# laitalaj/cvpce

Hardware: AMD Instinct MI355X
Metric: shelf images/sec end-to-end (detect+embed+match) (higher is better)
Workload: dtype bf16; 1 GPU; full production path: 8 shelf images/GPU of 3x2048x2048 (SKU-110K shape) -> GLN detect (800x800 internal, detections_per_img=200, conf>0.5) -> RoI crop 256x256 -> MAC-VGG16 embed -> cosine NN match, gallery=3200x1024 (BASELINE configs[2]/[4] per-GPU shape); images_per_gpu=8, global_images=8, gallery=3200, match_dtype=bf16, detector_precision=fp16, parallelism=dp1

## Files before the change

cvpce_amd/_lib.py:

```python
import ctypes
import os
from ctypes import c_int, c_float, c_void_p, c_size_t, c_longlong, POINTER

_HERE = os.path.dirname(os.path.abspath(__file__))
LIB_PATH = os.environ.get('CVPCE_LIB') or os.path.join(_HERE, 'libcvpce_hip.so')


class HipLibraryMissing(ImportError):
    pass


if not os.path.exists(LIB_PATH):
    raise HipLibraryMissing(
        f'{LIB_PATH} not found: the cvpce_amd hot path has no CPU fallback. '
        'Build the HIP library first (python -c "import __graft_entry__ as g; g.build()").')

lib = ctypes.CDLL(LIB_PATH)

_vp = c_void_p
_fp = c_void_p
_ip = c_void_p

SIGNATURES = {
    'cvpce_conv2d_nhwc_bf16': (c_int, [_vp, _vp, _fp, _vp, _vp] + [c_int] * 21 + [_vp]),
    'cvpce_conv2d_splitk_bf16': (c_int, [_vp, _vp, _fp, _vp, _vp] + [c_int] * 20 + [_vp, c_size_t, _vp]),
    'cvpce_conv2d_splitk_workspace_bytes': (c_size_t, [c_longlong, c_int, c_int]),
    'cvpce_set_persistent_workgroups': (c_int, [c_int]),
    'cvpce_conv1x1_nhwc_bf16': (c_int, [_vp, _vp, _fp, _vp, _vp] + [c_int] * 14 + [_vp]),
    'cvpce_vgg_stem_fused': (c_int, [_vp, c_int, _vp, _fp, _vp, _fp, _vp, c_int, c_int, c_int, _vp]),
    'cvpce_gln_stem_fused': (c_int, [_vp, _vp, _fp, _vp, c_int, c_int, c_int, _vp]),
    'cvpce_atlas_copy': (c_int, [POINTER(_vp), POINTER(c_int), POINTER(c_int), POINTER(c_int), POINTER(c_int), c_int, c_int, _vp, c_int, c_int, c_int, c_int, _vp]),
    'cvpce_conv3x3_halo': (c_int, [_vp, _vp, _fp, _vp] + [c_int] * 9 + [_vp]),
    'cvpce_conv3x3_halo_mac': (c_int, [_vp, _vp, _fp, _vp, _fp, c_int, c_int] + [c_int] * 8 + [_vp]),
    'cvpce_conv3x3_halo_wide': (c_int, [_vp, _vp, _fp, _vp] + [c_int] * 9 + [_vp]),
    'cvpce_conv3x3_halo_masked': (c_int, [_vp, _vp, _fp, _vp, _vp, c_int, _vp] + [c_int] * 8 + [_vp]),
    'cvpce_maxpool2d_nhwc_bf16': (c_int, [_vp, _vp] + [c_int] * 9 + [_vp]),
    'cvpce_relu_bf16': (c_int, [_vp, _vp, c_longlong, _vp]),
    'cvpce_pack_halo_weights': (c_int, [_vp, _vp, c_int, c_int]),
    'cvpce_conv3x3_thin_bf16': (c_int, [_vp, _vp, _fp, _vp] + [c_int] * 9 + [_vp]),
    'cvpce_gauss_tail_bf16': (c_int, [_vp, _vp, _fp, _vp, _fp, _fp, c_longlong, c_int, c_int, _vp]),
    'cvpce_gauss_subnet_bf16': (c_int, [_vp, _vp, _fp, _vp, _fp, _vp, _fp, _vp, _fp, c_int, _vp, _fp, c_int, _fp, c_int, c_int, c_int, c_int, _vp]),
    'cvpce_global_max_nhwc_bf16': (c_int, [_vp, _fp, c_int, c_int, c_int, c_int, c_int, _vp]),
    'cvpce_l2_normalize_f32': (c_int, [_fp, _fp, _vp, c_int, c_int, c_float, _vp]),
    'cvpce_gln_transform': (c_int, [_fp, _vp] + [c_int] * 6 + [POINTER(c_float), POINTER(c_float), _vp]),
    'cvpce_gln_transform_batch': (c_int, [POINTER(c_void_p), POINTER(c_int), POINTER(c_int), POINTER(c_int), POINTER(c_int), c_int, _vp, c_int, c_int,
                                          POINTER(c_float), POINTER(c_float), _vp]),
    'cvpce_crop_resize': (c_int, [_fp, _fp, _ip, c_int, _vp, c_int, c_int, c_int, c_int,
                                  POINTER(c_float), POINTER(c_float), _vp]),
    'cvpce_crop_resize_content': (c_int, [_fp, _fp, _ip, c_int, _vp, c_int, c_int, c_int, c_int,
                                          POINTER(c_float), POINTER(c_float), _ip, _vp]),
    'cvpce_pack_embed_input': (c_int, [_fp, _vp, c_int, c_int, c_int, POINTER(c_float), POINTER(c_float), _vp]),
    'cvpce_crop_extents': (c_int, [_fp, _ip, c_int, c_int, c_int, c_int, c_int, _ip, _vp]),
    'cvpce_pad_extents': (c_int, [_fp, c_int, c_int, c_float, _ip, _vp]),
    'cvpce_embed_worklists': (c_int, [_ip, c_int, c_int, ctypes.c_uint, _vp, c_int, _vp, c_longlong, _ip, _ip, _vp]),
    'cvpce_mac_init': (c_int, [_fp, c_int, c_int, c_int, c_int, _fp, _fp, c_int, c_int, _ip, _vp]),
    'cvpce_vgg_stem_fused_list': (c_int, [_vp, c_int, _vp, _vp, _fp, _vp, _fp, _vp, c_int, c_int, c_int, _vp, _ip, _vp]),
    'cvpce_bottleneck_fused_fm': (c_int, [_vp, _vp, _vp, _fp, _vp, _fp, _vp, _fp, _vp] + [c_int] * 5 + [_vp]),
    'cvpce_conv3x3_halo_thin_out': (c_int, [_vp, _vp, _fp, _fp] + [c_int] * 7 + [_vp]),
    'cvpce_conv3x3_halo_list': (c_int, [_vp, _vp, _fp, _vp, _fp, c_int, c_int] + [c_int] * 9 + [_vp, _ip, _vp]),
    'cvpce_conv3x3_halo_strips': (c_int, [_vp, _vp, _fp, _vp, _fp, c_int, c_int] + [c_int] * 9 + [_vp, _ip, _vp]),
    'cvpce_detect_workspace_bytes': (c_size_t, [c_int, c_int, c_int]),
    'cvpce_detect_postprocess': (c_int, [POINTER(c_void_p), POINTER(c_void_p), POINTER(c_int), POINTER(c_int),
                                         POINTER(c_int), POINTER(c_int), _fp, _ip, _fp,
                                         c_int, c_int, c_int, c_int, c_int, c_float, c_float, c_float, c_int, c_float,
                                         _vp, c_size_t, _fp, _fp, _vp, _ip, _ip, _vp]),
    'cvpce_row_norms': (c_int, [_vp, _fp, c_int, c_int, c_int, c_float, _vp]),
    'cvpce_match_workspace_bytes': (c_size_t, [c_int, c_int, c_int]),
    'cvpce_match_set_core': (c_int, [c_int, c_int, c_int]),
    'cvpce_probe_l2_stream': (c_int, [_vp, c_longlong, c_int, _fp, c_int, _vp]),
    'cvpce_probe_mfma_bf16': (c_int, [c_int, c_int, _vp, _fp, c_int, _vp]),
    'cvpce_match_topk': (c_int, [_vp, _vp, _fp, _fp, c_int, c_int, c_int, c_int, c_int, _vp, c_size_t, _vp, _fp, _vp]),
}
for _base, _twin in (('cvpce_conv2d_nhwc_bf16', 'cvpce_conv2d_nhwc_f16'), ('cvpce_conv2d_splitk_bf16', 'cvpce_conv2d_splitk_f16'), ('cvpce_conv1x1_nhwc_bf16', 'cvpce_conv1x1_nhwc_f16'),
                     ('cvpce_gln_stem_fused', 'cvpce_gln_stem_fused_f16'), ('cvpce_conv3x3_halo', 'cvpce_conv3x3_halo_f16'),
                     ('cvpce_conv3x3_halo_wide', 'cvpce_conv3x3_halo_wide_f16'), ('cvpce_conv3x3_halo_thin_out', 'cvpce_conv3x3_halo_thin_out_f16'), ('cvpce_conv3x3_halo_masked', 'cvpce_conv3x3_halo_masked_f16'),
                     ('cvpce_bottleneck_fused_fm', 'cvpce_bottleneck_fused_fm_f16'),
                     ('cvpce_maxpool2d_nhwc_bf16', 'cvpce_maxpool2d_nhwc_f16'), ('cvpce_relu_bf16', 'cvpce_relu_f16'), ('cvpce_gauss_tail_bf16', 'cvpce_gauss_tail_f16'), ('cvpce_gauss_subnet_bf16', 'cvpce_gauss_subnet_f16'), ('cvpce_conv3x3_thin_bf16', 'cvpce_conv3x3_thin_f16'),
                     ('cvpce_gln_transform', 'cvpce_gln_transform_f16'), ('cvpce_gln_transform_batch', 'cvpce_gln_transform_batch_f16')):
    SIGNATURES[_twin] = SIGNATURES[_base]

EVAL_SIGNATURES = {
    'cvpce_eval_match_detections': (c_int, [_fp, _ip, _ip, _ip, _fp, _ip, _ip, _fp] + [c_int] * 5 + [_ip, _vp, _vp]),
}

INPUT_SIGNATURES = {
    'cvpce_gln_transform_batch_u8': (c_int, [POINTER(c_void_p), POINTER(ctypes.c_ubyte), POINTER(c_int), POINTER(c_int), POINTER(c_int), POINTER(c_int), c_int,
                                             _vp, c_int, c_int, POINTER(c_float), POINTER(c_float), _fp, _vp]),
    'cvpce_crop_resize_u8': (c_int, [_vp, _fp, _fp, _ip, c_int, _vp, c_int, c_int, c_int, c_int, POINTER(c_float), POINTER(c_float), _vp]),
    'cvpce_crop_resize_content_u8': (c_int, [_vp, _fp, _fp, _ip, c_int, _vp, c_int, c_int, c_int, c_int, POINTER(c_float), POINTER(c_float), _ip, _vp]),
}
INPUT_SIGNATURES['cvpce_gln_transform_batch_u8_f16'] = INPUT_SIGNATURES['cvpce_gln_transform_batch_u8']

PLANOGRAM_SIGNATURES = {
    'cvpce_planogram_graphs': (c_int, [_fp, _ip, _fp] + [c_int] * 4 + [_ip, _fp, _ip, _vp]),
    'cvpce_planogram_match_workspace_bytes': (c_size_t, [c_longlong]),
    'cvpce_planogram_match': (c_int, [_ip] * 11 + [c_int] * 6 + [c_longlong, _vp, c_size_t, _ip, _ip, _vp]),
}

for _table in (SIGNATURES, EVAL_SIGNATURES, INPUT_SIGNATURES, PLANOGRAM_SIGNATURES):
    for _name, (_res, _args) in _table.items():
        _fn = getattr(lib, _name)
        _fn.restype = _res
        _fn.argtypes = _args

_ERR = {1: 'bad argument', 2: 'kernel launch failure'}


def check(rc, what):
    if rc != 0:
        raise RuntimeError(f'{what} failed: {_ERR.get(rc, rc)}')


class SkipLayer(ctypes.Structure):
    _fields_ = [(k, c_int) for k in ('H', 'W', 'tile_h', 'tile_w', 'out_ops', 'in_H', 'in_W', 'in_ops', 'skip')]


def float3(vals):
    return (c_float * 3)(*[float(v) for v in vals])
```

cvpce_amd/csrc/conv3x3_halo2.hip:

```cpp
#include "halo_common.h"
#include "../../include/cvpce_amd.h"

typedef __attribute__((address_space(3))) void lds_void;
typedef __attribute__((address_space(3))) char lds_char;

#ifndef CVPCE_DBG
#define CVPCE_DBG 0
#endif

#define G2_T 16
#define G2_P 18
#define G2_NPIX 324
#define G2_A_BYTES (328 * 128)
#define G2_NPIECE 41
#define G2_MAX_SEQ 512
#define G2_LTILE_OFF (3 * G2_A_BYTES)
#define G2_LROW_OFF (G2_LTILE_OFF + G2_MAX_SEQ * 4)
#define G2_SMEM_MASKED (G2_LROW_OFF + G2_MAX_SEQ * 32)
#define G2_LLIST_OFF (3 * G2_A_BYTES)
#define G2_SMEM_LIST (G2_LLIST_OFF + G2_MAX_SEQ * 8)

__device__ __forceinline__ int g2_swz0(int u) { return ((u & 3) << 1) | ((u >> 2) & 1); }
__device__ __forceinline__ int g2_swz(int py, int px) { return g2_swz0(px >> 1) ^ (py & 1); }

struct Halo2Args {
    const bf16_t* in;
    const bf16_t* wgt;
    const float* bias;
    const unsigned char* mask;
    bf16_t* out;
    const int* tile_map;
    int tiles_per_image;
    float* gmax;
    int gmax_stride, gmax_off;
    int N, H, W, Cin, Cout, K_pad, relu;
    int cgroups;
    int tiles_x, tiles_y, ptiles, ctiles, ntiles;
    unsigned in_bytes, wgt_bytes;
    const unsigned long long* list;
    const int* list_count;
};

#if CVPCE_DBG & 512
__device__ unsigned long long cvpce_halo2_clock[1024][2];
extern "C" int cvpce_debug_halo2_clock(unsigned long long* host_out) {
    return hipMemcpyFromSymbol(host_out, HIP_SYMBOL(cvpce_halo2_clock), sizeof(cvpce_halo2_clock)) == hipSuccess ? 0 : 2;
}
#endif

template <typename E, bool POOL, bool GMAX, bool LIST, bool STRIP = false, int NW = 8>
__global__ __launch_bounds__(64 * NW, NW == 8 ? 2 : 1) void conv3x3_halo2_kernel(Halo2Args a) {
    static_assert(!STRIP || LIST, "strips come from a work list");
    static_assert(NW == 8 || NW == 4, "cout waves");
    constexpr int TC = 32 * NW, NB = 16, NS = STRIP ? 3 : 1;

    extern __shared__ __attribute__((aligned(16))) unsigned char smem[];
    unsigned char* Ap = smem;

    const int tid = threadIdx.x, lane = tid & 63;
    const int wc = __builtin_amdgcn_readfirstlane(tid >> 6);
    const int l16 = lane & 15, lq = lane >> 4;

    const __amdgpu_buffer_rsrc_t srd_w = __builtin_amdgcn_make_buffer_rsrc((void*)a.wgt, 0, a.wgt_bytes, 0x00020000);
    const __amdgpu_buffer_rsrc_t srd_p = __builtin_amdgcn_make_buffer_rsrc((void*)a.in, 0, a.in_bytes, 0x00020000);

    const int nchunks = a.Cin >> 6;
    const int lbid = (CVPCE_DBG & 2) ? xcd_remap((int)blockIdx.x, (int)gridDim.x) : (int)blockIdx.x;
    int my_tiles, l_first = 0, l_entries = 0;
    if constexpr (LIST) {
        l_entries = __builtin_amdgcn_readfirstlane(*a.list_count);
        const int units = STRIP ? (l_entries + 2) / 3 : l_entries;
        const int groups = (int)gridDim.x / a.ctiles;
        const int per = (units + groups - 1) / groups;
        l_first = (lbid / a.ctiles) * per;
        my_tiles = units - l_first < per ? units - l_first : per;
    } else {
        my_tiles = halo_plain_tiles(a.ntiles, lbid, (int)gridDim.x);
    }
    if (my_tiles <= 0) return;
    const int total_chunks = my_tiles * nchunks;
    unsigned long long* llist = reinterpret_cast<unsigned long long*>(smem + G2_LLIST_OFF);
    if constexpr (LIST) {
        const int staged = my_tiles * NS < G2_MAX_SEQ ? my_tiles * NS : G2_MAX_SEQ;
        for (int idx = tid; idx < staged; idx += 64 * NW) {
            const int k = l_first * NS + idx;
            llist[idx] = a.list[k < l_entries ? k : l_entries - 1];
        }
        __syncthreads();
    }

    unsigned* ltile = reinterpret_cast<unsigned*>(smem + G2_LTILE_OFF);
    unsigned short* lrow = reinterpret_cast<unsigned short*>(smem + G2_LROW_OFF);
    if (a.mask) {
        for (int idx = tid; idx < my_tiles * 16; idx += 64 * NW) {
            const int sq = idx >> 4, y = idx & 15;
            const int r = ((lbid + sq * (int)gridDim.x) / a.ctiles) % a.tiles_per_image;
            int ty, tx;
            if (a.tile_map) {
                const int packed = a.tile_map[r];
                ty = packed >> 16;
                tx = packed & 0xFFFF;
            } else {
                ty = r / a.tiles_x;
                tx = r - ty * a.tiles_x;
            }
            const int oy = ty * G2_T + y;
            unsigned bits = 0;
            if (oy < a.H) {
#pragma unroll
                for (int c = 0; c < G2_T; ++c) {
                    const int ox = tx * G2_T + c;
                    if (ox < a.W && a.mask[oy * a.W + ox]) bits |= 1u << c;
                }
            }
            lrow[idx] = (unsigned short)bits;
            if (y == 0) ltile[sq] = (unsigned)((ty << 16) | tx);
        }
        __syncthreads();
    }

    auto tile_of = [&](int seq, int* n, int* ty, int* tx, int& ct, int* ext) {
        if constexpr (LIST) {
            ct = lbid % a.ctiles;
#pragma unroll
            for (int s = 0; s < NS; ++s) {
                const int k = seq * NS + s, g = l_first * NS + k;
                const unsigned long long e = k < G2_MAX_SEQ ? llist[k] : a.list[g < l_entries ? g : l_entries - 1];
                const int lo = __builtin_amdgcn_readfirstlane((int)wl_lo(e));
                ext[s] = __builtin_amdgcn_readfirstlane((int)wl_hi(e));
                n[s] = wl_image_signed(lo);
                ty[s] = wl_ty((unsigned)lo);
                tx[s] = wl_tx((unsigned)lo);
            }
            return;
        }
        ext[0] = 0;
        const int t = lbid + seq * (int)gridDim.x;
        ct = t % a.ctiles;
        const int p = t / a.ctiles;
        n[0] = p / a.tiles_per_image;
        const int r = p - n[0] * a.tiles_per_image;
        if (a.mask) {
            const int packed = __builtin_amdgcn_readfirstlane((int)ltile[seq]);
            ty[0] = packed >> 16;
            tx[0] = packed & 0xFFFF;
        } else {
            ty[0] = r / a.tiles_x;
            tx[0] = r - ty[0] * a.tiles_x;
        }
    };

    constexpr int NPP = (41 + NW - 1) / NW;
    const int npp = (41 - wc + NW - 1) / NW;
    auto issue_patch = [&](const int* n, const int* ty, const int* tx, int c, int buf, const int* ext) {
        const int ln = halo_lane_id();
#pragma unroll
        for (int i = 0; i < NPP; ++i) {
            if (i < npp) {
                const int j = wc + NW * i;
                const int pp = j * 8 + (ln >> 3);
                const int py = pp / G2_P, px = pp - py * G2_P;
                const int lchunk = (ln & 7) ^ g2_swz(py, px);
                int sn = n[0], sty = ty[0], stx = tx[0], sext = ext[0], ry = py;
                if constexpr (STRIP) {
                    const int st = py >= 12 ? 2 : (py >= 6 ? 1 : 0);
                    ry = py - 6 * st;
                    sn = st == 0 ? n[0] : (st == 1 ? n[1] : n[2]);
                    sty = st == 0 ? ty[0] : (st == 1 ? ty[1] : ty[2]);
                    stx = st == 0 ? tx[0] : (st == 1 ? tx[1] : tx[2]);
                    sext = st == 0 ? ext[0] : (st == 1 ? ext[1] : ext[2]);
                }
                const int ey = wl_ey((unsigned)sext), ex = wl_ex((unsigned)sext);
                const int y = sty * G2_T - 1 + ry, x = stx * G2_T - 1 + px;
                const bool ok = pp < G2_NPIX && (unsigned)y < (unsigned)a.H && (unsigned)x < (unsigned)a.W;
                int nn = sn;
                if constexpr (LIST) nn = (y >= ey || x >= ex) ? a.N - 1 : sn;
                const unsigned off = (unsigned)((((size_t)(nn * a.H + y) * a.W + x) * a.Cin + c * 64) * 2) + (unsigned)(lchunk * 16);
                __builtin_amdgcn_raw_ptr_buffer_load_lds(srd_p, (lds_void*)(Ap + buf * G2_A_BYTES + j * 1024), 16,
                                                         (int)(ok ? off : 0xFFFFFFF0u), 0, 0, 0);
            }
        }
    };
    int pi = 0, pi_seq = 0, pi_c = 0, pi_buf = 0, pi_n[NS], pi_ty[NS], pi_tx[NS], pi_ct, pi_ext[NS];
    tile_of(0, pi_n, pi_ty, pi_tx, pi_ct, pi_ext);
    auto issue_next_patch = [&]() {
        if (pi < total_chunks) {
            if (!(CVPCE_DBG & 4) || pi < 2) issue_patch(pi_n, pi_ty, pi_tx, pi_c, pi_buf, pi_ext);
            ++pi;
            if (++pi_buf == 3) pi_buf = 0;
            if (++pi_c == nchunks) {
                pi_c = 0;
                ++pi_seq;
                if (pi_seq < my_tiles) tile_of(pi_seq, pi_n, pi_ty, pi_tx, pi_ct, pi_ext);
            }
        }
    };

    const unsigned voff1 = (unsigned)(lane * 16);
    auto wbase = [&](int ct, int c) { return __builtin_amdgcn_readfirstlane((int)((unsigned)(c * a.cgroups + ct * (TC / 32) + wc) * 36864u)); };

    unsigned c3[3];
    {
        const int col = halo_col(l16);
#pragma unroll
        for (int kw = 0; kw < 3; ++kw) c3[kw] = (unsigned)(col * 128) ^ (unsigned)((lq ^ g2_swz0(((col + kw) >> 1) & 7)) << 4);
    }
    const unsigned lds_a = (unsigned)(size_t)(lds_char*)Ap;

    auto load_bias = [&](int ct, f32x4* b) {
#pragma unroll
        for (int mt = 0; mt < 2; ++mt) {
            const int co = ct * TC + wc * 32 + 8 * lq + 4 * mt;
            b[mt] = (a.bias && co < a.Cout) ? *reinterpret_cast<const f32x4*>(a.bias + co) : f32x4{0.f, 0.f, 0.f, 0.f};
        }
    };
    f32x4 acc[2][NB];
    {
        f32x4 b0[2];
        load_bias(pi_ct, b0);
#pragma unroll
        for (int i = 0; i < 2; ++i)
#pragma unroll
            for (int j = 0; j < NB; ++j) acc[i][j] = b0[i];
    }

    bf16x8 af[2][3][2];
    bf16x8 bfr[4];
    unsigned e0, e1;

#define G2_LOAD_A(T, SBASE)                                                                                    \
    if constexpr (!(CVPCE_DBG & 8)) {                                                                          \
        _Pragma("unroll") for (int kh_ = 0; kh_ < 3; ++kh_)                                                    \
            _Pragma("unroll") for (int mt_ = 0; mt_ < 2; ++mt_) {                                              \
                const u32x4 v_ = __builtin_amdgcn_raw_buffer_load_b128(srd_w, voff1, (SBASE) + (((T) * 3 + kh_) * 2 + mt_) * 1024, 0); \
                af[(T) & 1][kh_][mt_] = __builtin_bit_cast(bf16x8, v_);                                       \
            }                                                                                                  \
    }
#define G2_PREFETCH_A(T)                                                                                       \
    if constexpr ((T) < 5) { G2_LOAD_A((T) + 1, sb_cur) } else { G2_LOAD_A(0, sb_next) }
#define G2_SET_E(T, BUFB)                                                                                      \
    {                                                                                                          \
        const unsigned x_ = c3[(T) >> 1] ^ (unsigned)(((T) & 1) << 6);                                         \
        e0 = x_ + (BUFB);                                                                                      \
        e1 = (x_ ^ 16u) + (BUFB);                                                                              \
    }
#define G2_READ(T, P)                                                                                          \
    if constexpr (!(CVPCE_DBG & 32)) {                                                                         \
        if constexpr (((P) & 1) == 0)                                                                          \
            asm volatile("ds_read_b128 %0, %1 offset:%2" : "=v"(bfr[((P) + 2 * (T)) & 3]) : "v"(e0), "n"(((P) * G2_P + ((T) >> 1)) * 128)); \
        else                                                                                                   \
            asm volatile("ds_read_b128 %0, %1 offset:%2" : "=v"(bfr[((P) + 2 * (T)) & 3]) : "v"(e1), "n"(((P) * G2_P + ((T) >> 1)) * 128)); \
    }
#define G2_ROW_KH(T, P, KH)                                                                                    \
    {                                                                                                          \
        constexpr int j_ = STRIP ? (P) % 6 - (KH) : (P) - (KH);                                                \
        constexpr int r_ = STRIP ? 4 * ((P) / 6) + j_ : j_;                                                    \
        if constexpr (j_ >= 0 && j_ < (STRIP ? 4 : NB)) {                                                      \
            _Pragma("unroll") for (int mt_ = 0; mt_ < 2; ++mt_)                                                \
                acc[mt_][r_] = E::mfma16(af[(T) & 1][KH][mt_], bfr[((P) + 2 * (T)) & 3], acc[mt_][r_]);       \
        }                                                                                                      \
    }
#define G2_ROW(T, P)                                                                                           \
    {                                                                                                          \
        asm volatile("s_waitcnt lgkmcnt(2)" : "+v"(bfr[((P) + 2 * (T)) & 3]));                                 \
        G2_ROW_KH(T, P, 0) G2_ROW_KH(T, P, 1) G2_ROW_KH(T, P, 2)                                               \
        __builtin_amdgcn_sched_barrier(0);                                                                     \
    }
#define G2_RP(T, P) G2_READ(T, (P) + 2) G2_ROW(T, P)
#define G2_HANDOFF()                                                                                           \
    {                                                                                                          \
        asm volatile("s_waitcnt vmcnt(6)" ::: "memory");                                                       \
        if (!(CVPCE_DBG & 64)) __builtin_amdgcn_s_barrier();                                                   \
        issue_next_patch();                                                                                    \
    }
#define G2_ROWS_AND_TAIL(T, TN, BUFB_NEXT, BEFORE)                                                             \
    G2_RP(T, 0) G2_RP(T, 1) G2_RP(T, 2) G2_RP(T, 3) G2_RP(T, 4) G2_RP(T, 5)                                    \
    if (!LIST || STRIP || rows_ > 4) { G2_RP(T, 6) G2_RP(T, 7) G2_RP(T, 8) G2_RP(T, 9) }                       \
    if (!LIST || STRIP || rows_ > 8) { G2_RP(T, 10) G2_RP(T, 11) G2_RP(T, 12) G2_RP(T, 13) }                   \
    if (!LIST || STRIP || rows_ > 12) {                                                                        \
        G2_RP(T, 14) G2_RP(T, 15)                                                                              \
        BEFORE                                                                                                 \
        G2_SET_E(TN, BUFB_NEXT)                                                                                \
        G2_READ(TN, 0) G2_ROW(T, 16)                                                                           \
        G2_READ(TN, 1) G2_ROW(T, 17)                                                                           \
    } else {                                                                                                   \
        BEFORE                                                                                                 \
        G2_SET_E(TN, BUFB_NEXT)                                                                                \
        G2_READ(TN, 0)                                                                                         \
        G2_READ(TN, 1)                                                                                         \
    }
#define G2_STEP(T)                                                                                             \
    {                                                                                                          \
        G2_PREFETCH_A(T)                                                                                       \
        __builtin_amdgcn_sched_barrier(0);                                                                     \
        G2_ROWS_AND_TAIL(T, (T) + 1, bufb, )                                                                   \
    }

    int seq = 0, cchunk = 0, t_n[NS], t_ty[NS], t_tx[NS], t_ct, t_ext_[NS];
    tile_of(0, t_n, t_ty, t_tx, t_ct, t_ext_);
    int rows_ = (LIST && !STRIP) ? wl_rows((unsigned)t_ext_[0]) : NB;
    int n_ct = t_ct;
    auto next_ct = [&]() {
        if (cchunk + 1 < nchunks) return t_ct;
        if constexpr (LIST) return t_ct;
        if (seq + 1 < my_tiles) return (lbid + (seq + 1) * (int)gridDim.x) % a.ctiles;
        return t_ct;
    };
    issue_next_patch();
    issue_next_patch();
    int sb_cur = wbase(t_ct, 0);
    n_ct = next_ct();
    int sb_next = wbase(n_ct, (cchunk + 1 < nchunks) ? cchunk + 1 : 0);
    {
        constexpr int dbg8_ = CVPCE_DBG & 8;
        _Pragma("unroll") for (int kh_ = 0; kh_ < 3; ++kh_)
            _Pragma("unroll") for (int mt_ = 0; mt_ < 2; ++mt_) {
                const u32x4 v_ = __builtin_amdgcn_raw_buffer_load_b128(srd_w, voff1, sb_cur + (kh_ * 2 + mt_) * 1024, 0);
                af[0][kh_][mt_] = __builtin_bit_cast(bf16x8, v_);
                if (dbg8_) af[1][kh_][mt_] = af[0][kh_][mt_];
            }
    }
    asm volatile("s_waitcnt vmcnt(0)" ::: "memory");
    __builtin_amdgcn_s_barrier();
    unsigned bufb = lds_a;
    int bufi = 0;
    G2_SET_E(0, bufb)
    G2_READ(0, 0)
    G2_READ(0, 1)

    const int lp = lane & 15;
#if CVPCE_DBG & 512
    const unsigned long long ck0_ = __builtin_amdgcn_s_memtime(), rt0_ = __builtin_amdgcn_s_memrealtime();
#endif
    for (int cc = 0; cc < total_chunks; ++cc) {
        asm volatile("" : "+v"(c3[0]), "+v"(c3[1]), "+v"(c3[2]));
        G2_STEP(0) G2_STEP(1) G2_STEP(2) G2_STEP(3) G2_STEP(4)
        {
            G2_PREFETCH_A(5)
            __builtin_amdgcn_sched_barrier(0);
            const int nbufi = (bufi == 2) ? 0 : bufi + 1;
            const unsigned nbufb = lds_a + (unsigned)nbufi * G2_A_BYTES;
            G2_ROWS_AND_TAIL(5, 0, nbufb, G2_HANDOFF())
            bufb = nbufb;
            bufi = nbufi;
        }
        sb_cur = sb_next;

        if (cchunk + 1 == nchunks) {
            const int ct = t_ct;
            const int rows_t = STRIP ? 4 : rows_;
            auto e_n = [&](int nt) { return STRIP ? t_n[(nt >> 2) < NS ? (nt >> 2) : 0] : t_n[0]; };
            auto e_ty = [&](int nt) { return STRIP ? t_ty[(nt >> 2) < NS ? (nt >> 2) : 0] : t_ty[0]; };
            auto e_tx = [&](int nt) { return STRIP ? t_tx[(nt >> 2) < NS ? (nt >> 2) : 0] : t_tx[0]; };
            auto e_row = [&](int nt) { return STRIP ? (nt & 3) : nt; };
            auto e_live = [&](int nt) { return STRIP ? nt < 12 : (!LIST || nt < rows_t); };
            f32x4 nbias[2];
            load_bias(n_ct, nbias);
            const int col = halo_col(lp);
            const int co = ct * TC + wc * 32 + 8 * lq;
            if constexpr (GMAX) {
#pragma unroll
                for (int sg = 0; sg < NS; ++sg) {
                    unsigned m[8];
#pragma unroll
                    for (int j = 0; j < 8; ++j) m[j] = 0u;
                    const int n = t_n[sg], ty = t_ty[sg], tx = t_tx[sg];
                    if (tx * G2_T + col < a.W) {
#pragma unroll
                        for (int nt = STRIP ? 4 * sg : 0; nt < (STRIP ? 4 * sg + 4 : NB); ++nt)
                            if (ty * G2_T + e_row(nt) < a.H && e_live(nt)) {
#pragma unroll
                                for (int j = 0; j < 4; ++j) {
                                    m[j] = max(m[j], __float_as_uint(relu_bits(acc[0][nt][j])));
                                    m[4 + j] = max(m[4 + j], __float_as_uint(relu_bits(acc[1][nt][j])));
                                }
                            }
                    }
#pragma unroll
                    for (int j = 0; j < 8; ++j) {
                        unsigned v = m[j];
                        v = max(v, (unsigned)__builtin_amdgcn_update_dpp(0, (int)v, 0x128, 0xF, 0xF, false));
                        v = max(v, (unsigned)__builtin_amdgcn_update_dpp(0, (int)v, 0x124, 0xF, 0xF, false));
                        v = max(v, (unsigned)__builtin_amdgcn_update_dpp(0, (int)v, 0x122, 0xF, 0xF, false));
                        v = max(v, (unsigned)__builtin_amdgcn_update_dpp(0, (int)v, 0x121, 0xF, 0xF, false));
                        m[j] = v;
                    }
                    if (lp == 0) {
                        unsigned* g = reinterpret_cast<unsigned*>(a.gmax) + (size_t)n * a.gmax_stride + a.gmax_off + co;
#pragma unroll
                        for (int j = 0; j < 8; ++j)
                            if (co + j < a.Cout) atomicMax(g + j, __float_as_uint(E::widen(E::narrow(__uint_as_float(m[j])))));
                    }
                }
            }
            if (GMAX && a.out == nullptr) {
            } else if (POOL) {
#pragma unroll
                for (int i = 0; i < NB / 2; ++i) {
                    const int ox = e_tx(2 * i) * (G2_T / 2) + (col >> 1);
                    const bool lane_ok = (lp < 4 || lp >= 12) && ox < (a.W >> 1);
                    const int oy = e_ty(2 * i) * (G2_T / 2) + (e_row(2 * i) >> 1);
                    const size_t opix = (size_t)(e_n(2 * i) * (a.H >> 1) + oy) * (a.W >> 1) + ox;
                    float r[8];
#pragma unroll
                    for (int mt = 0; mt < 2; ++mt)
#pragma unroll
                        for (int j = 0; j < 4; ++j) r[4 * mt + j] = halo_pool2x2(acc[mt][2 * i][j], acc[mt][2 * i + 1][j], a.relu);
                    if (lane_ok && oy < (a.H >> 1) && co < a.Cout && e_live(2 * i) && (!(CVPCE_DBG & 16) || a.relu == 12345)) {
                        const uint2 l2 = __builtin_bit_cast(uint2, E::pack4(f32x4{r[0], r[1], r[2], r[3]}));
                        const uint2 h2 = __builtin_bit_cast(uint2, E::pack4(f32x4{r[4], r[5], r[6], r[7]}));
                        *reinterpret_cast<u32x4*>(a.out + opix * a.Cout + co) = u32x4{l2.x, l2.y, h2.x, h2.y};
                    }
                }
            } else {
#pragma unroll
                for (int nt = 0; nt < NB; ++nt) {
                    const int ox = e_tx(nt) * G2_T + col;
                    const int oy = e_ty(nt) * G2_T + e_row(nt);
                    const size_t opix = (size_t)(e_n(nt) * a.H + oy) * a.W + ox;
                    const bool store_lane = oy < a.H && ox < a.W && e_live(nt);
                    bool keep = true;
                    if (a.mask) keep = ((lrow[seq * 16 + nt] >> col) & 1u) != 0;
                    f32x4 r0 = acc[0][nt], r1 = acc[1][nt];
                    if (a.relu) {
#pragma unroll
                        for (int j = 0; j < 4; ++j) { r0[j] = relu_bits(r0[j]); r1[j] = relu_bits(r1[j]); }
                    }
                    if (store_lane && co < a.Cout && (!(CVPCE_DBG & 16) || a.relu == 12345)) {
                        const uint2 l2 = __builtin_bit_cast(uint2, E::pack4(r0)), h2 = __builtin_bit_cast(uint2, E::pack4(r1));
                        bf16_t* dst = a.out + opix * a.Cout + co;
                        *reinterpret_cast<u32x4*>(dst) = keep ? u32x4{l2.x, l2.y, h2.x, h2.y} : u32x4{0u, 0u, 0u, 0u};
                    }
                }
            }
#pragma unroll
            for (int mt = 0; mt < 2; ++mt)
#pragma unroll
                for (int nt = 0; nt < NB; ++nt) acc[mt][nt] = nbias[mt];
            cchunk = 0;
            ++seq;
            if (seq < my_tiles) {
                tile_of(seq, t_n, t_ty, t_tx, t_ct, t_ext_);
                if constexpr (LIST && !STRIP) rows_ = wl_rows((unsigned)t_ext_[0]);
            }
        } else {
            ++cchunk;
        }
        n_ct = next_ct();
        sb_next = wbase(n_ct, (cchunk + 1 < nchunks) ? cchunk + 1 : 0);
    }
    asm volatile("s_waitcnt lgkmcnt(0)" ::: "memory");
#if CVPCE_DBG & 512
    if (wc == 0 && lane == 0 && blockIdx.x < 1024) {
        cvpce_halo2_clock[blockIdx.x][0] = __builtin_amdgcn_s_memtime() - ck0_;
        cvpce_halo2_clock[blockIdx.x][1] = __builtin_amdgcn_s_memrealtime() - rt0_;
    }
#endif
#undef G2_STEP
#undef G2_HANDOFF
#undef G2_ROWS_AND_TAIL
#undef G2_RP
#undef G2_ROW
#undef G2_ROW_KH
#undef G2_READ
#undef G2_SET_E
#undef G2_PREFETCH_A
#undef G2_LOAD_A
}

template <typename E, bool POOL, bool GMAX, bool LIST = false, bool STRIP = false>
static int launch_halo2(Halo2Args a, hipStream_t stream) {
    a.ctiles = (a.Cout + 255) / 256;
    a.ntiles = a.ptiles * a.ctiles;
    if constexpr (!POOL && !GMAX && !LIST) {
        if (!a.mask && a.Cout % 128 == 0 && 2 * a.ntiles <= g_cvpce_persistent_wgs) {
            a.ctiles = a.Cout / 128;
            a.ntiles = a.ptiles * a.ctiles;
            return halo_launch<conv3x3_halo2_kernel<E, false, false, false, false, 4>>(a, a.ntiles, 256, 3 * G2_A_BYTES, stream);
        }
    }
    const int smem = a.mask ? G2_SMEM_MASKED : (LIST ? G2_SMEM_LIST : 3 * G2_A_BYTES);
    const int grid = halo_grid(a.ntiles, a.ctiles, LIST);
    if (a.mask && (a.ntiles + grid - 1) / grid > G2_MAX_SEQ) return CVPCE_ERR_ARG;
    return halo_launch<conv3x3_halo2_kernel<E, POOL, GMAX, LIST, STRIP>>(a, grid, 512, smem, stream, G2_SMEM_MASKED);
}

static Halo2Args halo2_args(const void* in, const void* wgt, const float* bias, void* out, float* gmax, int gmax_stride, int gmax_off,
                            const HaloShape& sh, int relu) {
    Halo2Args a;
    halo_fill(a, in, wgt, bias, out, sh, relu, G2_T, nullptr, nullptr);
    a.mask = nullptr; a.tile_map = nullptr; a.tiles_per_image = a.tiles_x * a.tiles_y;
    a.gmax = gmax; a.gmax_stride = gmax_stride; a.gmax_off = gmax_off;
    return a;
}
static bool halo2_gmax_ok(int relu, int Cout, int gmax_stride, int gmax_off) {
    return relu && Cout > 128 && gmax_off >= 0 && gmax_off + Cout <= gmax_stride;
}

static constexpr HaloRules G2_RULES = { G2_T,  256,  1LL << 30,  true,  0};

template <typename E>
static int halo2_dispatch(const void* in, const void* wgt, const float* bias, const unsigned char* mask, const int* tile_map,
                          int n_map, void* out, float* gmax,
                          int gmax_stride, int gmax_off, int N, int H, int W, int Cin, int Cout, int K_pad, int Cout_pad, int relu,
                          int fuse_pool2, void* stream) {
    if (N <= 0) return CVPCE_OK;
    if (!out && !gmax) return CVPCE_ERR_ARG;
    if (gmax && (mask || !halo2_gmax_ok(relu, Cout, gmax_stride, gmax_off))) return CVPCE_ERR_ARG;
    if (tile_map && (!mask || n_map <= 0)) return CVPCE_ERR_ARG;
    if (mask && fuse_pool2) return CVPCE_ERR_ARG;
    if (Cout <= 128 && !mask)
        return (E::kF16 ? cvpce_conv3x3_halo_wide_f16 : cvpce_conv3x3_halo_wide)(in, wgt, bias, out, N, H, W, Cin, Cout, K_pad, Cout_pad, relu, fuse_pool2, stream);
    const HaloShape sh{N, H, W, Cin, Cout, K_pad, Cout_pad};
    if (!halo_shape_ok(in, wgt, sh, fuse_pool2, tile_map ? n_map : 0, false, G2_RULES)) return CVPCE_ERR_ARG;
    Halo2Args a = halo2_args(in, wgt, bias, out, gmax, gmax_stride, gmax_off, sh, relu);
    hipStream_t s = (hipStream_t)stream;
    if (mask) {
        a.mask = mask;
        if (tile_map) { a.tile_map = tile_map; a.tiles_per_image = n_map; a.ptiles = N * n_map; }
        const long long per_image = (long long)a.tiles_per_image * ((Cout + 255) / 256);
        const long long cap = (long long)G2_MAX_SEQ * g_cvpce_persistent_wgs;
        if (per_image > cap) return CVPCE_ERR_ARG;
        const int n_per = (int)(cap / per_image);
        for (int n0 = 0; n0 < N; n0 += n_per) {
            Halo2Args b = a;
            b.N = (N - n0) < n_per ? (N - n0) : n_per;
            b.in = a.in + (size_t)n0 * H * W * Cin;
            b.out = a.out + (size_t)n0 * H * W * Cout;
            b.ptiles = b.N * a.tiles_per_image;
            b.in_bytes = (unsigned)((long long)b.N * H * W * Cin * 2);
            const int rc = launch_halo2<E, false, false>(b, s);
            if (rc != CVPCE_OK) return rc;
        }
        return CVPCE_OK;
    }
    return halo_pick([&](auto pool, auto mac) { return launch_halo2<E, decltype(pool)::value, decltype(mac)::value>(a, s); }, fuse_pool2 != 0, gmax != nullptr);
}

extern "C" int cvpce_conv3x3_halo(const void* in, const void* wgt, const float* bias, void* out, int N, int H, int W,
                                  int Cin, int Cout, int K_pad, int Cout_pad, int relu, int fuse_pool2, void* stream) {
    return halo2_dispatch<ElemBF16>(in, wgt, bias, nullptr, nullptr, 0, out, nullptr, 0, 0, N, H, W, Cin, Cout, K_pad, Cout_pad, relu, fuse_pool2, stream);
}

extern "C" int cvpce_conv3x3_halo_mac(const void* in, const void* wgt, const float* bias, void* out, float* mac, int mac_stride,
                                      int mac_off, int N, int H, int W, int Cin, int Cout, int K_pad, int Cout_pad,
                                      int fuse_pool2, void* stream) {
    if (!mac) return CVPCE_ERR_ARG;
    return halo2_dispatch<ElemBF16>(in, wgt, bias, nullptr, nullptr, 0, out, mac, mac_stride, mac_off, N, H, W, Cin, Cout, K_pad, Cout_pad, 1, fuse_pool2, stream);
}

extern "C" int cvpce_conv3x3_halo_masked(const void* in, const void* wgt, const float* bias, const unsigned char* mask,
                                         const int* tile_map, int n_tiles, void* out, int N, int H, int W, int Cin, int Cout,
                                         int K_pad, int Cout_pad, int relu, void* stream) {
    if (!mask) return CVPCE_ERR_ARG;
    return halo2_dispatch<ElemBF16>(in, wgt, bias, mask, tile_map, n_tiles, out, nullptr, 0, 0, N, H, W, Cin, Cout, K_pad, Cout_pad, relu, 0, stream);
}

extern "C" int cvpce_conv3x3_halo_f16(const void* in, const void* wgt, const float* bias, void* out, int N, int H, int W,
                                      int Cin, int Cout, int K_pad, int Cout_pad, int relu, int fuse_pool2, void* stream) {
    return halo2_dispatch<ElemF16>(in, wgt, bias, nullptr, nullptr, 0, out, nullptr, 0, 0, N, H, W, Cin, Cout, K_pad, Cout_pad, relu, fuse_pool2, stream);
}

extern "C" int cvpce_conv3x3_halo_masked_f16(const void* in, const void* wgt, const float* bias, const unsigned char* mask,
                                             const int* tile_map, int n_tiles, void* out, int N, int H, int W, int Cin, int Cout,
                                             int K_pad, int Cout_pad, int relu, void* stream) {
    if (!mask) return CVPCE_ERR_ARG;
    return halo2_dispatch<ElemF16>(in, wgt, bias, mask, tile_map, n_tiles, out, nullptr, 0, 0, N, H, W, Cin, Cout, K_pad, Cout_pad, relu, 0, stream);
}

int cvpce_conv3x3_halo_wide_list(const void* in, const void* wgt, const float* bias, void* out, int N, int H, int W, int Cin,
                                 int Cout, int K_pad, int Cout_pad, int relu, int fuse_pool2, const unsigned long long* list,
                                 const int* count_dev, void* stream);

static int halo_list_launch(const void* in, const void* wgt, const float* bias, void* out, float* mac, int mac_stride,
                            int mac_off, int N, int H, int W, int Cin, int Cout, int K_pad, int Cout_pad, int relu,
                            int fuse_pool2, const unsigned long long* list, const int* count_dev, bool strips, void* stream) {
    if (N <= 0) return CVPCE_OK;
    if ((!out && !mac) || !list || !count_dev) return CVPCE_ERR_ARG;
    if (mac && !halo2_gmax_ok(relu, Cout, mac_stride, mac_off)) return CVPCE_ERR_ARG;
    if (Cout <= 128) {
        if (strips) return CVPCE_ERR_ARG;
        return cvpce_conv3x3_halo_wide_list(in, wgt, bias, out, N, H, W, Cin, Cout, K_pad, Cout_pad, relu, fuse_pool2, list, count_dev, stream);
    }
    const HaloShape sh{N, H, W, Cin, Cout, K_pad, Cout_pad};
    if (!halo_shape_ok(in, wgt, sh, fuse_pool2, 0, true, G2_RULES)) return CVPCE_ERR_ARG;
    Halo2Args a = halo2_args(in, wgt, bias, out, mac, mac_stride, mac_off, sh, relu);
    a.list = list; a.list_count = count_dev;
    hipStream_t s = (hipStream_t)stream;
    return halo_pick([&](auto pool, auto gm, auto strip) { return launch_halo2<ElemBF16, decltype(pool)::value, decltype(gm)::value, true, decltype(strip)::value>(a, s); },
                     fuse_pool2 != 0, mac != nullptr, strips);
}

extern "C" int cvpce_conv3x3_halo_list(const void* in, const void* wgt, const float* bias, void* out, float* mac, int mac_stride,
                                       int mac_off, int N, int H, int W, int Cin, int Cout, int K_pad, int Cout_pad, int relu,
                                       int fuse_pool2, const unsigned long long* list, const int* count_dev, void* stream) {
    return halo_list_launch(in, wgt, bias, out, mac, mac_stride, mac_off, N, H, W, Cin, Cout, K_pad, Cout_pad, relu, fuse_pool2, list, count_dev, false, stream);
}

extern "C" int cvpce_conv3x3_halo_strips(const void* in, const void* wgt, const float* bias, void* out, float* mac, int mac_stride,
                                         int mac_off, int N, int H, int W, int Cin, int Cout, int K_pad, int Cout_pad, int relu,
                                         int fuse_pool2, const unsigned long long* strip_list, const int* count_dev, void* stream) {
    return halo_list_launch(in, wgt, bias, out, mac, mac_stride, mac_off, N, H, W, Cin, Cout, K_pad, Cout_pad, relu, fuse_pool2, strip_list, count_dev, true, stream);
}

extern "C" int cvpce_pack_halo_weights(const void* src_rowmajor, void* dst_halo, int Cout_pad, int Cin) {
    if (!src_rowmajor || !dst_halo || Cout_pad <= 0 || Cout_pad % 32 != 0 || Cin <= 0 || Cin % 64 != 0) return CVPCE_ERR_ARG;
    const unsigned short* src = (const unsigned short*)src_rowmajor;
    unsigned short* dst = (unsigned short*)dst_halo;
    const int nch = Cin / 64, groups = Cout_pad / 32;
    const size_t K_pad = (size_t)9 * Cin;
    size_t o = 0;
    for (int c = 0; c < nch; ++c)
        for (int g = 0; g < groups; ++g)
            for (int kw = 0; kw < 3; ++kw)
                for (int half = 0; half < 2; ++half)
                    for (int kh = 0; kh < 3; ++kh)
                        for (int mt = 0; mt < 2; ++mt)
                            for (int lane = 0; lane < 64; ++lane) {
                                const int m = lane & 15, q = lane >> 4;
                                const size_t row = (size_t)32 * g + 8 * (m >> 2) + 4 * mt + (m & 3);
                                const size_t k = (size_t)c * 576 + (kh * 3 + kw) * 64 + half * 32 + q * 8;
                                for (int e = 0; e < 8; ++e) dst[o++] = src[row * K_pad + k + e];
                            }
    return CVPCE_OK;
}
```

cvpce_amd/csrc/conv3x3_halo3.hip:

```cpp
#include "halo_common.h"
#include "../../include/cvpce_amd.h"

typedef __attribute__((address_space(3))) void lds_void;
typedef __attribute__((address_space(3))) char lds_char;

#ifndef CVPCE_DBG
#define CVPCE_DBG 0
#endif
#define G3_TH 16
#define G3_TW 32
#define G3_PW 34
#define G3_NPIX (18 * 34)
#define G3_NPIECE 39
#define G3_A_BYTES (G3_NPIECE * 1024)
#define G3_MAX_SEQ 512
#define G3_LLIST_OFF (3 * G3_A_BYTES)
#define G3_SMEM_LIST (G3_LLIST_OFF + G3_MAX_SEQ * 8)

struct Halo3Args {
    const bf16_t* in;
    const bf16_t* wgt;
    const float* bias;
    bf16_t* out;
    int N, H, W, Cin, Cout, K_pad, relu;
    int cgroups;
    int tiles_x, tiles_y, ptiles, ctiles, ntiles;
    unsigned in_bytes, wgt_bytes;
    const unsigned long long* list;
    const int* list_count;
};

#if CVPCE_DBG & 128
__device__ unsigned long long cvpce_halo3_stamps[2][6];
extern "C" int cvpce_debug_halo3_stamps(unsigned long long* host_out) {
    return hipMemcpyFromSymbol(host_out, HIP_SYMBOL(cvpce_halo3_stamps), sizeof(cvpce_halo3_stamps)) == hipSuccess ? 0 : 2;
}
#define G3_TIC() const unsigned long long tic_ = __builtin_amdgcn_s_memtime();
#define G3_TOC(I) st_[I] += __builtin_amdgcn_s_memtime() - tic_;
#define G3_STAMP_STEP() { G3_TIC() asm volatile("s_waitcnt vmcnt(0)" ::: "memory"); G3_TOC(0) st_[5] += 1; }
#else
#define G3_TIC()
#define G3_TOC(I)
#define G3_STAMP_STEP()
#endif

template <typename E, bool POOL, bool LIST, bool THIN = false>
__global__ __launch_bounds__(512, 2) void conv3x3_halo3_kernel(Halo3Args a) {
    static_assert(!THIN || (!POOL && !LIST), "thin-output form: plain launches only");
#if CVPCE_DBG & 128
    unsigned long long st_[6] = {0, 0, 0, 0, 0, 0};
#endif
    constexpr int TC = 128, NB = 16, NG = 4;

    extern __shared__ __attribute__((aligned(16))) unsigned char smem[];
    unsigned char* Ap = smem;

    const int tid = threadIdx.x, lane = tid & 63;
    const int wid = __builtin_amdgcn_readfirstlane(tid >> 6);
    const int wc = wid >> 1, wp = wid & 1;
    const int l16 = lane & 15, lq = lane >> 4;
    const bool active = THIN ? (wc * 32 < a.Cout) : true;

    const __amdgpu_buffer_rsrc_t srd_w = __builtin_amdgcn_make_buffer_rsrc((void*)a.wgt, 0, a.wgt_bytes, 0x00020000);
    const __amdgpu_buffer_rsrc_t srd_p = __builtin_amdgcn_make_buffer_rsrc((void*)a.in, 0, a.in_bytes, 0x00020000);

    const int nchunks = a.Cin >> 6;
    const int lbid = (CVPCE_DBG & 2) ? (int)blockIdx.x : xcd_remap((int)blockIdx.x, (int)gridDim.x);
    int my_tiles, l_first = 0;
    if constexpr (LIST) {
        my_tiles = halo_list_span(__builtin_amdgcn_readfirstlane(*a.list_count), (int)gridDim.x, a.ctiles, lbid, l_first);
    } else {
        my_tiles = halo_plain_tiles(a.ntiles, lbid, (int)gridDim.x);
    }
    if (my_tiles <= 0) return;
    const int total_chunks = my_tiles * nchunks;
    const int total_sub = 2 * total_chunks;
    unsigned long long* llist = reinterpret_cast<unsigned long long*>(smem + G3_LLIST_OFF);
    if constexpr (LIST) {
        const int staged = my_tiles < G3_MAX_SEQ ? my_tiles : G3_MAX_SEQ;
        for (int idx = tid; idx < staged; idx += 512) llist[idx] = a.list[l_first + idx];
        __syncthreads();
    }

    auto tile_of = [&](int seq, int& n, int& ty, int& tx, int& ct, int& ext) {
        if constexpr (LIST) {
            ct = lbid % a.ctiles;
            const unsigned long long e = seq < G3_MAX_SEQ ? llist[seq] : a.list[l_first + seq];
            const int lo = __builtin_amdgcn_readfirstlane((int)wl_lo(e));
            ext = __builtin_amdgcn_readfirstlane((int)wl_hi(e));
            n = wl_image_signed(lo);
            ty = wl_ty((unsigned)lo);
            tx = wl_tx((unsigned)lo);
            return;
        }
        ext = 0;
        const int t = lbid + seq * (int)gridDim.x;
        ct = t % a.ctiles;
        const int p = t / a.ctiles;
        n = p / (a.tiles_x * a.tiles_y);
        const int r = p - n * (a.tiles_x * a.tiles_y);
        ty = r / a.tiles_x;
        tx = r - ty * a.tiles_x;
    };

    const int npp = (wid < 7) ? 5 : 4;
    auto issue_patch = [&](int n, int ty, int tx, int c32, int buf, int ext) {
        const int y0 = ty * G3_TH - 1, x0 = tx * G3_TW - 1;
        const int ey = wl_ey((unsigned)ext), ex = wl_ex((unsigned)ext);
        const int ln = halo_lane_id();
#pragma unroll
        for (int i = 0; i < 5; ++i) {
            if (i < npp) {
                const int j = wid + 8 * i;
                const int pp = j * 16 + (ln >> 2);
                const int py = pp / G3_PW, px = pp - py * G3_PW;
                const int lchunk = (ln & 3) ^ ((px >> 2) & 3);
                const int y = y0 + py, x = x0 + px;
                const bool ok = pp < G3_NPIX && (unsigned)y < (unsigned)a.H && (unsigned)x < (unsigned)a.W;
                int nn = n;
                if constexpr (LIST) nn = (y >= ey || x >= ex) ? a.N - 1 : n;
                const unsigned off = (unsigned)((((size_t)(nn * a.H + y) * a.W + x) * a.Cin + c32 * 32) * 2) + (unsigned)(lchunk * 16);
                __builtin_amdgcn_raw_ptr_buffer_load_lds(srd_p, (lds_void*)(Ap + buf * G3_A_BYTES + j * 1024), 16,
                                                         (int)(ok ? off : 0xFFFFFFF0u), 0, 0, 0);
            }
        }
    };
    int pi = 0, pi_seq = 0, pi_c = 0, pi_buf = 0, pi_n, pi_ty, pi_tx, pi_ct, pi_ext;
    tile_of(0, pi_n, pi_ty, pi_tx, pi_ct, pi_ext);
    const int nsub = 2 * nchunks;
    auto issue_next_patch = [&]() {
        if (pi < total_sub) {
            if (!(CVPCE_DBG & 4) || pi < 2) issue_patch(pi_n, pi_ty, pi_tx, pi_c, pi_buf, pi_ext);
            ++pi;
            if (++pi_buf == 3) pi_buf = 0;
            if (++pi_c == nsub) {
                pi_c = 0;
                ++pi_seq;
                if (pi_seq < my_tiles) tile_of(pi_seq, pi_n, pi_ty, pi_tx, pi_ct, pi_ext);
            }
        }
    };

    const unsigned voff1 = (unsigned)(lane * 16);
    auto wbase = [&](int ct, int c) { return __builtin_amdgcn_readfirstlane((int)((unsigned)(c * a.cgroups + ct * (TC / 32) + wc) * 36864u)); };

    unsigned c3[3];
    {
        const int col = 16 * wp + halo_col(l16);
#pragma unroll
        for (int kw = 0; kw < 3; ++kw) c3[kw] = (unsigned)(col * 64 + ((lq ^ (((col + kw) >> 2) & 3)) << 4));
    }
    const unsigned lds_a = (unsigned)(size_t)(lds_char*)Ap;

    auto load_bias = [&](int ct, f32x4* b) {
#pragma unroll
        for (int mt = 0; mt < 2; ++mt) {
            const int co = ct * TC + wc * 32 + 8 * lq + 4 * mt;
            if constexpr (THIN) {
#pragma unroll
                for (int j = 0; j < 4; ++j) b[mt][j] = (a.bias && co + j < a.Cout) ? a.bias[co + j] : 0.f;
            } else {
                b[mt] = (a.bias && co < a.Cout) ? *reinterpret_cast<const f32x4*>(a.bias + co) : f32x4{0.f, 0.f, 0.f, 0.f};
            }
        }
    };
    f32x4 acc[2][NB];
    {
        f32x4 b0[2];
        load_bias(pi_ct, b0);
#pragma unroll
        for (int i = 0; i < 2; ++i)
#pragma unroll
            for (int j = 0; j < NB; ++j) acc[i][j] = b0[i];
    }

    bf16x8 af[2][3][2];
    bf16x8 bfr[4];
    unsigned e0;

#define G3_LOAD_A(T, SBASE)                                                                                    \
    if constexpr (!(CVPCE_DBG & 8)) if (active) {                                                              \
        _Pragma("unroll") for (int kh_ = 0; kh_ < 3; ++kh_)                                                    \
            _Pragma("unroll") for (int mt_ = 0; mt_ < 2; ++mt_) {                                              \
                const u32x4 v_ = __builtin_amdgcn_raw_buffer_load_b128(srd_w, voff1, (SBASE) + (((((T) % 3) * 2 + (T) / 3) * 3 + kh_) * 2 + mt_) * 1024, 0); \
                af[(T) & 1][kh_][mt_] = __builtin_bit_cast(bf16x8, v_);                                        \
            }                                                                                                  \
    }
#define G3_SET_E(T, BUFB) { e0 = c3[(T) % 3] + (BUFB); }
#define G3_READ(T, P)                                                                                          \
    if constexpr (!(CVPCE_DBG & 32)) if (active)                                                               \
    asm volatile("ds_read_b128 %0, %1 offset:%2" : "=v"(bfr[((P) + 2 * (T)) & 3]) : "v"(e0), "n"(((P) * G3_PW + (T) % 3) * 64));
#define G3_ROW(T, P)                                                                                           \
    if (active) {                                                                                              \
        if constexpr (!(CVPCE_DBG & 32)) asm volatile("s_waitcnt lgkmcnt(2)" : "+v"(bfr[((P) + 2 * (T)) & 3]));  \
        _Pragma("unroll") for (int kh_ = 0; kh_ < 3; ++kh_)                                                    \
            if ((P) - kh_ >= 0 && (P) - kh_ < NB) {                                                            \
                _Pragma("unroll") for (int mt_ = 0; mt_ < 2; ++mt_)                                            \
                    acc[mt_][(P) - kh_] = E::mfma16(af[(T) & 1][kh_][mt_], bfr[((P) + 2 * (T)) & 3], acc[mt_][(P) - kh_]); \
            }                                                                                                  \
        __builtin_amdgcn_sched_barrier(0);                                                                     \
    }
#define G3_RP(T, P) G3_READ(T, (P) + 2) G3_ROW(T, P)
#define G3_HANDOFF()                                                                                           \
    {                                                                                                          \
        { G3_TIC() if (!(CVPCE_DBG & 64)) asm volatile("s_waitcnt vmcnt(6)" ::: "memory"); G3_TOC(1) }         \
        { G3_TIC() if (!(CVPCE_DBG & 64)) __builtin_amdgcn_s_barrier(); G3_TOC(2) }      \
        issue_next_patch();                                                                                    \
    }
#define G3_ROWS_AND_TAIL(T, TN, BUFB_NEXT, BEFORE)                                                             \
    G3_RP(T, 0) G3_RP(T, 1) G3_RP(T, 2) G3_RP(T, 3) G3_RP(T, 4) G3_RP(T, 5)                                    \
    if (!LIST || rows_ > 4) { G3_RP(T, 6) G3_RP(T, 7) G3_RP(T, 8) G3_RP(T, 9) }                                \
    if (!LIST || rows_ > 8) { G3_RP(T, 10) G3_RP(T, 11) G3_RP(T, 12) G3_RP(T, 13) }                            \
    if (!LIST || rows_ > 12) {                                                                                 \
        G3_RP(T, 14) G3_RP(T, 15)                                                                              \
        BEFORE                                                                                                 \
        G3_SET_E(TN, BUFB_NEXT)                                                                                \
        G3_READ(TN, 0) G3_ROW(T, 16)                                                                           \
        G3_READ(TN, 1) G3_ROW(T, 17)                                                                           \
    } else {                                                                                                   \
        BEFORE                                                                                                 \
        G3_SET_E(TN, BUFB_NEXT)                                                                                \
        G3_READ(TN, 0)                                                                                         \
        G3_READ(TN, 1)                                                                                         \
    }
#define G3_STEP(T)                                                                                             \
    {                                                                                                          \
        G3_LOAD_A((T) + 1, sb_cur)                                                                             \
        __builtin_amdgcn_sched_barrier(0);                                                                     \
        G3_ROWS_AND_TAIL(T, (T) + 1, bufb, )                                                                   \
        G3_STAMP_STEP()                                                                                        \
    }
#define G3_STEP_HANDOFF(T, TN, SBN)                                                                            \
    {                                                                                                          \
        G3_LOAD_A(TN, SBN)                                                                                     \
        __builtin_amdgcn_sched_barrier(0);                                                                     \
        const int nbufi = (bufi == 2) ? 0 : bufi + 1;                                                          \
        const unsigned nbufb = lds_a + (unsigned)nbufi * G3_A_BYTES;                                           \
        G3_ROWS_AND_TAIL(T, TN, nbufb, G3_HANDOFF())                                                           \
        bufb = nbufb;                                                                                          \
        bufi = nbufi;                                                                                          \
    }

    int seq = 0, cchunk = 0, t_n, t_ty, t_tx, t_ct, t_ext_;
    tile_of(0, t_n, t_ty, t_tx, t_ct, t_ext_);
    int rows_ = LIST ? wl_rows((unsigned)t_ext_) : NB;
    int n_ct = t_ct;
    auto next_ct = [&]() {
        if (cchunk + 1 < nchunks) return t_ct;
        if constexpr (LIST) return t_ct;
        if (seq + 1 < my_tiles) return (lbid + (seq + 1) * (int)gridDim.x) % a.ctiles;
        return t_ct;
    };
    issue_next_patch();
    issue_next_patch();
    int sb_cur = wbase(t_ct, 0);
    n_ct = next_ct();
    int sb_next = wbase(n_ct, (cchunk + 1 < nchunks) ? cchunk + 1 : 0);
    G3_LOAD_A(0, sb_cur)
    asm volatile("s_waitcnt vmcnt(0)" ::: "memory");
    __builtin_amdgcn_s_barrier();
    unsigned bufb = lds_a;
    int bufi = 0;
    G3_SET_E(0, bufb)
    G3_READ(0, 0)
    G3_READ(0, 1)

    const int lp = lane & 15;
#if CVPCE_DBG & 128
    const unsigned long long loop0_ = __builtin_amdgcn_s_memtime();
#endif
    for (int cc = 0; cc < total_chunks; ++cc) {
        asm volatile("" : "+v"(c3[0]), "+v"(c3[1]), "+v"(c3[2]));
        G3_STEP(0) G3_STEP(1)
        G3_STEP_HANDOFF(2, 3, sb_cur)
        G3_STEP(3) G3_STEP(4)
        G3_STEP_HANDOFF(5, 0, sb_next)
        sb_cur = sb_next;

        if (cchunk + 1 == nchunks) {
            const int n = t_n, ty = t_ty, tx = t_tx, ct = t_ct;
            const int rows_t = rows_;
            G3_TIC()
            f32x4 nbias[2];
            load_bias(n_ct, nbias);
            const int col = halo_col(lp);
            if constexpr (THIN) {
                float* outf = reinterpret_cast<float*>(a.out);
                const int ox = tx * G3_TW + 16 * wp + col;
#pragma unroll
                for (int nt = 0; nt < NB; ++nt) {
                    const int oy = ty * G3_TH + nt;
                    if (active && oy < a.H && ox < a.W) {
                        float* po = outf + ((size_t)(n * a.H + oy) * a.W + ox) * a.Cout;
#pragma unroll
                        for (int mt = 0; mt < 2; ++mt) {
                            const int co = wc * 32 + 8 * lq + 4 * mt;
                            if ((a.Cout & 3) == 0) {
                                if (co < a.Cout) *reinterpret_cast<f32x4*>(po + co) = acc[mt][nt];
                            } else {
#pragma unroll
                                for (int j = 0; j < 4; ++j)
                                    if (co + j < a.Cout) po[co + j] = acc[mt][nt][j];
                            }
                        }
                    }
                }
            } else if (POOL) {
                const int ox = tx * (G3_TW / 2) + 8 * wp + (col >> 1);
                const bool lane_ok = (lp < 4 || lp >= 12) && ox < (a.W >> 1);
#pragma unroll
                for (int i = 0; i < NB / 2; ++i) {
                    const int oy = ty * (G3_TH / 2) + i;
                    const size_t opix = (size_t)(n * (a.H >> 1) + oy) * (a.W >> 1) + ox;
                    const int co = ct * TC + wc * 32 + 8 * lq;
                    float r[8];
#pragma unroll
                    for (int mt = 0; mt < 2; ++mt)
#pragma unroll
                        for (int j = 0; j < 4; ++j) r[4 * mt + j] = halo_pool2x2(acc[mt][2 * i][j], acc[mt][2 * i + 1][j], a.relu);
                    if (lane_ok && oy < (a.H >> 1) && co < a.Cout && (!LIST || 2 * i < rows_t) && (!(CVPCE_DBG & 16) || a.relu == 12345)) {
                        const uint2 l2 = __builtin_bit_cast(uint2, E::pack4(f32x4{r[0], r[1], r[2], r[3]}));
                        const uint2 h2 = __builtin_bit_cast(uint2, E::pack4(f32x4{r[4], r[5], r[6], r[7]}));
                        *reinterpret_cast<u32x4*>(a.out + opix * a.Cout + co) = u32x4{l2.x, l2.y, h2.x, h2.y};
                    }
                }
            } else {
                const int tp = lane >> 2, tq = lane & 3;
                const int src4 = (16 * tq + tp) * 4;
                const int ox = tx * G3_TW + 16 * wp + halo_col(tp);
                const int co = ct * TC + wc * 32 + 8 * tq;
#pragma unroll
                for (int nt = 0; nt < NB; ++nt) {
                    const int oy = ty * G3_TH + nt;
                    const size_t opix = (size_t)(n * a.H + oy) * a.W + ox;
                    const bool store_lane = oy < a.H && ox < a.W && (!LIST || nt < rows_t);
                    f32x4 r0 = acc[0][nt], r1 = acc[1][nt];
                    if (a.relu) {
#pragma unroll
                        for (int j = 0; j < 4; ++j) { r0[j] = relu_bits(r0[j]); r1[j] = relu_bits(r1[j]); }
                    }
                    const uint2 l2 = __builtin_bit_cast(uint2, E::pack4(r0)), h2 = __builtin_bit_cast(uint2, E::pack4(r1));
                    u32x4 v;
                    v[0] = (unsigned)__builtin_amdgcn_ds_bpermute(src4, (int)l2.x);
                    v[1] = (unsigned)__builtin_amdgcn_ds_bpermute(src4, (int)l2.y);
                    v[2] = (unsigned)__builtin_amdgcn_ds_bpermute(src4, (int)h2.x);
                    v[3] = (unsigned)__builtin_amdgcn_ds_bpermute(src4, (int)h2.y);
                    if (store_lane && co < a.Cout && (!(CVPCE_DBG & 16) || a.relu == 12345))
                        *reinterpret_cast<u32x4*>(a.out + opix * a.Cout + co) = v;
                }
            }
#pragma unroll
            for (int mt = 0; mt < 2; ++mt)
#pragma unroll
                for (int nt = 0; nt < NB; ++nt) acc[mt][nt] = nbias[mt];
            G3_TOC(3)
            cchunk = 0;
            ++seq;
            if (seq < my_tiles) {
                tile_of(seq, t_n, t_ty, t_tx, t_ct, t_ext_);
                if constexpr (LIST) rows_ = wl_rows((unsigned)t_ext_);
            }
        } else {
            ++cchunk;
        }
        n_ct = next_ct();
        sb_next = wbase(n_ct, (cchunk + 1 < nchunks) ? cchunk + 1 : 0);
    }
    asm volatile("s_waitcnt lgkmcnt(0)" ::: "memory");
#if CVPCE_DBG & 128
    st_[4] = __builtin_amdgcn_s_memtime() - loop0_;
    if (blockIdx.x == 3 && (wid == 0 || wid == 5) && lane == 0)
        for (int i = 0; i < 6; ++i) cvpce_halo3_stamps[wid ? 1 : 0][i] = st_[i];
#endif
#undef G3_STEP_HANDOFF
#undef G3_STEP
#undef G3_HANDOFF
#undef G3_ROWS_AND_TAIL
#undef G3_RP
#undef G3_ROW
#undef G3_READ
#undef G3_SET_E
#undef G3_LOAD_A
}

static constexpr HaloRules G3_RULES = { G3_TW,  128,  1LL << 29,  true,  0};
static constexpr HaloRules G3_THIN_RULES = { G3_TW,  0,  1LL << 29,  false,  128};

template <typename E>
static int halo3_dispatch(const void* in, const void* wgt, const float* bias, void* out, int N, int H, int W,
                          int Cin, int Cout, int K_pad, int Cout_pad, int relu, int fuse_pool2, void* stream,
                          const unsigned long long* list = nullptr, const int* count_dev = nullptr) {
    if (N <= 0) return CVPCE_OK;
    if (!out || (list && (E::kF16 || !count_dev))) return CVPCE_ERR_ARG;
    const HaloShape sh{N, H, W, Cin, Cout, K_pad, Cout_pad};
    if (!halo_shape_ok(in, wgt, sh, fuse_pool2, 0, list != nullptr, G3_RULES)) return CVPCE_ERR_ARG;
    Halo3Args a;
    halo_fill(a, in, wgt, bias, out, sh, relu, G3_TW, list, count_dev);
    a.ctiles = (Cout + 127) / 128;
    a.ntiles = a.ptiles * a.ctiles;
    return halo_pick([&](auto pool, auto lst) {
        constexpr bool LIST = decltype(lst)::value && !E::kF16;
        return halo_launch<conv3x3_halo3_kernel<E, decltype(pool)::value, LIST>>(a, halo_grid(a.ntiles, a.ctiles, LIST), 512,
                                                                                 LIST ? G3_SMEM_LIST : 3 * G3_A_BYTES, (hipStream_t)stream);
    }, fuse_pool2 != 0, list != nullptr);
}

template <typename E>
static int halo3_thin_dispatch(const void* in, const void* wgt, const float* bias, float* out, int N, int H, int W, int Cin, int Cout,
                               int K_pad, int Cout_pad, void* stream) {
    if (N <= 0) return CVPCE_OK;
    if (!out) return CVPCE_ERR_ARG;
    const HaloShape sh{N, H, W, Cin, Cout, K_pad, Cout_pad};
    if (!halo_shape_ok(in, wgt, sh, 0, 0, false, G3_THIN_RULES)) return CVPCE_ERR_ARG;
    Halo3Args a;
    halo_fill(a, in, wgt, bias, out, sh, 0, G3_TW, nullptr, nullptr);
    a.ctiles = 1; a.ntiles = a.ptiles;
    return halo_launch<conv3x3_halo3_kernel<E, false, false, true>>(a, halo_grid(a.ntiles, 1, false), 512, 3 * G3_A_BYTES, (hipStream_t)stream);
}
extern "C" int cvpce_conv3x3_halo_thin_out(const void* in, const void* wgt, const float* bias, float* out, int N, int H, int W,
                                           int Cin, int Cout, int K_pad, int Cout_pad, void* stream) {
    return halo3_thin_dispatch<ElemBF16>(in, wgt, bias, out, N, H, W, Cin, Cout, K_pad, Cout_pad, stream);
}
extern "C" int cvpce_conv3x3_halo_thin_out_f16(const void* in, const void* wgt, const float* bias, float* out, int N, int H, int W,
                                               int Cin, int Cout, int K_pad, int Cout_pad, void* stream) {
    return halo3_thin_dispatch<ElemF16>(in, wgt, bias, out, N, H, W, Cin, Cout, K_pad, Cout_pad, stream);
}

extern "C" int cvpce_conv3x3_halo_wide(const void* in, const void* wgt, const float* bias, void* out, int N, int H, int W,
                                       int Cin, int Cout, int K_pad, int Cout_pad, int relu, int fuse_pool2, void* stream) {
    return halo3_dispatch<ElemBF16>(in, wgt, bias, out, N, H, W, Cin, Cout, K_pad, Cout_pad, relu, fuse_pool2, stream);
}
extern "C" int cvpce_conv3x3_halo_wide_f16(const void* in, const void* wgt, const float* bias, void* out, int N, int H, int W,
                                           int Cin, int Cout, int K_pad, int Cout_pad, int relu, int fuse_pool2, void* stream) {
    return halo3_dispatch<ElemF16>(in, wgt, bias, out, N, H, W, Cin, Cout, K_pad, Cout_pad, relu, fuse_pool2, stream);
}

int cvpce_conv3x3_halo_wide_list(const void* in, const void* wgt, const float* bias, void* out, int N, int H, int W, int Cin,
                                 int Cout, int K_pad, int Cout_pad, int relu, int fuse_pool2, const unsigned long long* list,
                                 const int* count_dev, void* stream) {
    if (!list || !count_dev) return CVPCE_ERR_ARG;
    return halo3_dispatch<ElemBF16>(in, wgt, bias, out, N, H, W, Cin, Cout, K_pad, Cout_pad, relu, fuse_pool2, stream, list, count_dev);
}
```

cvpce_amd/csrc/skiplist.hip:

```cpp
#include "common.h"
#include "worklist.h"
#include "../../include/cvpce_amd.h"

#define SKL_MAX_LAYERS 16

struct WorklistArgs {
    const int* ext0;
    int n, S, nl;
    unsigned pool_mask;
    cvpce_skip_layer L[SKL_MAX_LAYERS];
    unsigned long long* lists;
    long long stride;
    int* counts;
    int* computed;
};

__device__ __forceinline__ int skl_extent(int e0, int S, unsigned pool_mask, int nops, int size) {
    if (e0 >= S) return size;
    int e = e0;
    for (int i = 0; i < nops; ++i) e = ((pool_mask >> i) & 1u) ? (e + 1) >> 1 : e + 1;
    return e < size ? e : size;
}

__global__ __launch_bounds__(1024) void embed_worklists_kernel(WorklistArgs a) {
    __shared__ int s_cnt[1024];
    __shared__ int s_end[1024], s_send[1024];
    __shared__ unsigned s_geo[1024], s_ext[1024];
    __shared__ int s_base, s_sbase, s_units;
    const cvpce_skip_layer L = a.L[blockIdx.x];
    const int tid = threadIdx.x;
    const int tiles_y = (L.H + L.tile_h - 1) / L.tile_h, tiles_x = (L.W + L.tile_w - 1) / L.tile_w;
    unsigned long long* list = a.lists + (long long)blockIdx.x * a.stride;
    unsigned long long* slist = a.lists + (long long)(a.nl + blockIdx.x) * a.stride;
    if (tid == 0) s_base = s_sbase = s_units = 0;
    __syncthreads();
    auto scan = [&](int v) {
        s_cnt[tid] = v;
        __syncthreads();
        for (int d = 1; d < 1024; d <<= 1) {
            const int t = tid >= d ? s_cnt[tid - d] : 0;
            __syncthreads();
            s_cnt[tid] += t;
            __syncthreads();
        }
    };
    for (int n0 = 0; n0 < a.n; n0 += 1024) {
        const int n = n0 + tid;
        int ny = 0, nx = 0, eiy = 0, eix = 0, last_rows = 16;
        if (n < a.n) {
            const bool is_const = n == a.n - 1;
            const int ey0 = is_const ? a.S : a.ext0[2 * n], ex0 = is_const ? a.S : a.ext0[2 * n + 1];
            ny = tiles_y; nx = tiles_x;
            if (L.skip) {
                const int eoy = skl_extent(ey0, a.S, a.pool_mask, L.out_ops, L.H), eox = skl_extent(ex0, a.S, a.pool_mask, L.out_ops, L.W);
                const int cy = (eoy + L.tile_h - 1) / L.tile_h, cx = (eox + L.tile_w - 1) / L.tile_w;
                ny = cy < tiles_y ? cy : tiles_y;
                nx = cx < tiles_x ? cx : tiles_x;
                if (L.skip >= 2 && ny > 0) {
                    const int left = eoy - (ny - 1) * L.tile_h;
                    const int act = left < L.tile_h ? left : L.tile_h;
                    last_rows = ((act * 16 + L.tile_h - 1) / L.tile_h + 3) & ~3;
                    if (last_rows > 16) last_rows = 16;
                }
            }
            eiy = skl_extent(ey0, a.S, a.pool_mask, L.in_ops, L.in_H);
            eix = skl_extent(ex0, a.S, a.pool_mask, L.in_ops, L.in_W);
        }
        if (nx == 0) ny = 0;
        const bool strips = L.skip >= 3 && ny > 0 && last_rows == 4;
        const int scnt = strips ? nx : 0, cnt = ny * nx - scnt;
        if (a.computed && n < a.n && blockIdx.y == 0) {
            a.computed[((long long)blockIdx.x * a.n + n) * 2] = ny > 0 ? (ny - 1) * 16 + last_rows : 0;
            a.computed[((long long)blockIdx.x * a.n + n) * 2 + 1] = nx;
        }
        if (ny > 0) atomicAdd(&s_units, nx * (16 * (ny - 1) + (strips ? 4 : (last_rows < 16 ? last_rows + 1 : 16))));
        s_geo[tid] = ((unsigned)ny << 16) | ((unsigned)nx << 8) | (unsigned)last_rows;
        s_ext[tid] = wl_pack_ext((unsigned)eiy, (unsigned)eix);
        const int base0 = s_base, sbase0 = s_sbase;
        scan(cnt);
        s_end[tid] = s_cnt[tid];
        const int total = s_cnt[1023];
        __syncthreads();
        scan(scnt);
        s_send[tid] = s_cnt[tid];
        const int stotal = s_cnt[1023];
        __syncthreads();
        auto crop_of = [&](const int* ends, int e) {
            int lo = 0, hi = 1023;
            while (lo < hi) {
                const int mid = (lo + hi) >> 1;
                if (ends[mid] > e) hi = mid; else lo = mid + 1;
            }
            return lo;
        };
        for (int e = (int)blockIdx.y * 1024 + tid; e < total; e += (int)gridDim.y * 1024) {
            const int c = crop_of(s_end, e);
            const unsigned geo = s_geo[c];
            const int cny = (int)(geo >> 16), cnx = (int)((geo >> 8) & 0xFF), j = e - (c ? s_end[c - 1] : 0);
            const int ty = j / cnx, tx = j - ty * cnx;
            const unsigned rows = (ty == cny - 1) ? (geo & 0xFF) : 16u;
            list[base0 + e] = wl_pack(rows, s_ext[c], (unsigned)(n0 + c), (unsigned)ty, (unsigned)tx);
        }
        for (int e = (int)blockIdx.y * 1024 + tid; e < stotal; e += (int)gridDim.y * 1024) {
            const int c = crop_of(s_send, e);
            const unsigned geo = s_geo[c];
            const int cny = (int)(geo >> 16), tx = e - (c ? s_send[c - 1] : 0);
            slist[sbase0 + e] = wl_pack(4u, s_ext[c], (unsigned)(n0 + c), (unsigned)(cny - 1), (unsigned)tx);
        }
        __syncthreads();
        if (tid == 0) { s_base = base0 + total; s_sbase = sbase0 + stotal; }
        __syncthreads();
    }
    if (tid == 0 && blockIdx.y == 0) {
        a.counts[blockIdx.x] = s_base;
        a.counts[a.nl + blockIdx.x] = s_units;
        a.counts[2 * a.nl + blockIdx.x] = s_sbase;
    }
}

extern "C" int cvpce_embed_worklists(const int* ext0, int n_images, int S, unsigned pool_mask, const cvpce_skip_layer* layers, int n_layers,
                                     unsigned long long* lists, long long list_stride, int* counts, int* computed, void* stream) {
    if (n_layers <= 0) return CVPCE_OK;
    if (!ext0 && n_images > 1) return CVPCE_ERR_ARG;
    if (!layers || !lists || !counts || n_layers > SKL_MAX_LAYERS || n_images <= 0 || n_images > WL_MAX_IMAGES || S <= 0 || S > 32767) return CVPCE_ERR_ARG;
    WorklistArgs a;
    a.ext0 = ext0; a.n = n_images; a.S = S; a.nl = n_layers; a.pool_mask = pool_mask; a.lists = lists; a.stride = list_stride; a.counts = counts; a.computed = computed;
    for (int i = 0; i < n_layers; ++i) {
        const cvpce_skip_layer& l = layers[i];
        if (l.H <= 0 || l.W <= 0 || l.tile_h <= 0 || l.tile_w <= 0 || l.in_H <= 0 || l.in_W <= 0 || l.in_H > WL_MAX_EXTENT || l.in_W > WL_MAX_EXTENT) return CVPCE_ERR_ARG;
        if (l.in_ops < 0 || l.out_ops < l.in_ops || l.out_ops > 32) return CVPCE_ERR_ARG;
        const long long ty = (l.H + l.tile_h - 1) / l.tile_h, tx = (l.W + l.tile_w - 1) / l.tile_w;
        if (ty > WL_MAX_TILES || tx > WL_MAX_TILES || ty * tx * n_images > list_stride) return CVPCE_ERR_ARG;
        a.L[i] = l;
    }
    const int split = n_images >= 64 ? 8 : 1;
    hipLaunchKernelGGL(embed_worklists_kernel, dim3(n_layers, split), dim3(1024), 0, (hipStream_t)stream, a);
    return cvpce_check_launch();
}


__global__ void mac_init_kernel(float* __restrict__ desc, int stride, int off, int C, const float* __restrict__ rtab, const float* __restrict__ ctab,
                                int Hc, int Wc, const int* __restrict__ computed) {
    const int n = blockIdx.y, c = blockIdx.x * blockDim.x + threadIdx.x;
    if (c >= C) return;
    int rc = computed[2 * n], cc = computed[2 * n + 1] * 16;
    rc = rc < Hc ? rc : Hc;
    cc = cc < Wc ? cc : Wc;
    desc[(size_t)n * stride + off + c] = fmaxf(rtab[(size_t)rc * C + c], ctab[(size_t)cc * C + c]);
}

extern "C" int cvpce_mac_init(float* desc, int n_images, int desc_stride, int desc_off, int C, const float* row_suffix_max,
                              const float* col_suffix_max, int Hc, int Wc, const int* computed, void* stream) {
    if (n_images <= 0) return CVPCE_OK;
    if (!desc || !row_suffix_max || !col_suffix_max || !computed || C <= 0 || Hc <= 0 || Wc <= 0 || desc_off < 0 || desc_off + C > desc_stride || n_images > 65535)
        return CVPCE_ERR_ARG;
    hipLaunchKernelGGL(mac_init_kernel, dim3((C + 255) / 256, n_images), dim3(256), 0, (hipStream_t)stream, desc, desc_stride, desc_off, C,
                       row_suffix_max, col_suffix_max, Hc, Wc, computed);
    return cvpce_check_launch();
}
```

cvpce_amd/models/classification.py:

```python
from collections import OrderedDict

import torch
from torch import nn

from .. import ops

VGG_CFGS = {'D': (64, 64, 'M', 128, 128, 'M', 256, 256, 256, 'M', 512, 512, 512, 'M', 512, 512, 512, 'M')}
IMAGENET_MEAN = (0.485, 0.456, 0.406)
IMAGENET_STD = (0.229, 0.224, 0.225)
TANH_MEAN = tuple(m * 2 - 1 for m in IMAGENET_MEAN)
TANH_STD = tuple(s * 2 for s in IMAGENET_STD)
INPUT_SIZE = 256
USE_FUSED_STEM = True
import os as _os
MAX_EMBED_BATCH = int(_os.environ.get('CVPCE_EMBED_BATCH', 256))
FUSED_EMBED_BATCH = int(_os.environ.get('CVPCE_EMBED_BATCH', 768))
FUSED_EMBED_MAX = int(_os.environ.get('CVPCE_EMBED_MAX', 960))
FUSED_EMBED_BATCH = min(FUSED_EMBED_BATCH, FUSED_EMBED_MAX)
SKIP_PADDING = _os.environ.get('CVPCE_SKIP_PADDING', '1') != '0'
LATE_EMBED_MAX = int(_os.environ.get('CVPCE_LATE_EMBED_MAX', 2000))
SKIP_ROWS = _os.environ.get('CVPCE_SKIP_ROWS', '1') != '0'
SKIP_MAC = _os.environ.get('CVPCE_SKIP_MAC', '1') != '0'
SKIP_STRIPS = _os.environ.get('CVPCE_SKIP_STRIPS', '1') != '0'


def _passes(n, step, longest):
    sizes = [step] * (n // step) + ([n % step] if n % step else [])
    if len(sizes) >= 2 and sizes[-1] + sizes[-2] <= longest:
        sizes[-2:] = [sizes[-1] + sizes[-2]]
    out, s = [], 0
    for z in sizes:
        out.append((s, s + z))
        s += z
    return out


def _vgg_features(cfg, batch_norm):
    layers, cin = [], 3
    for v in cfg:
        if v == 'M':
            layers.append(nn.MaxPool2d(kernel_size=2, stride=2))
        else:
            conv = nn.Conv2d(cin, v, kernel_size=3, padding=1)
            nn.init.kaiming_normal_(conv.weight, mode='fan_out', nonlinearity='relu')
            nn.init.constant_(conv.bias, 0)
            layers += [conv, nn.BatchNorm2d(v), nn.ReLU(inplace=True)] if batch_norm else [conv, nn.ReLU(inplace=True)]
            cin = v
    return layers


class MACVGGEngine:
    def __init__(self, model, device):
        self.plan = []
        mods = list(model.block1) + ['desc1'] + list(model.block2)
        i = 0
        while i < len(mods):
            m = mods[i]
            if isinstance(m, str):
                self.plan.append(('desc', None))
            elif isinstance(m, nn.MaxPool2d):
                if self.plan and self.plan[-1][0] == 'conv':
                    self.plan[-1] = ('conv_pool', self.plan[-1][1])
                else:
                    self.plan.append(('pool', None))
            elif isinstance(m, nn.Conv2d):
                scale = shift = None
                if i + 1 < len(mods) and isinstance(mods[i + 1], nn.BatchNorm2d):
                    bn = mods[i + 1]
                    scale = bn.weight * (bn.running_var + bn.eps).rsqrt()
                    shift = bn.bias - bn.running_mean * scale
                self.plan.append(('conv', ops.PackedConv(m.weight, m.bias, 1, 1, scale=scale, shift=shift, device=device)))
            i += 1
        self.stem = None
        if (USE_FUSED_STEM and len(self.plan) >= 2 and self.plan[0][0] == 'conv' and self.plan[1][0] == 'conv_pool'
                and self.plan[0][1].cin == 3 and self.plan[0][1].cout == 64 and self.plan[1][1].cout == 64):
            packed = []
            for i, m in enumerate(mods):
                if isinstance(m, nn.Conv2d) and len(packed) < 4:
                    w, b = m.weight.detach().float().cpu(), m.bias.detach().float().cpu()
                    if i + 1 < len(mods) and isinstance(mods[i + 1], nn.BatchNorm2d):
                        bn = mods[i + 1]
                        sc = (bn.weight * (bn.running_var + bn.eps).rsqrt()).detach().float().cpu()
                        w = w * sc[:, None, None, None]
                        b = b * sc + (bn.bias.detach().float().cpu() - bn.running_mean.detach().float().cpu() * sc)
                    packed += [w, b]
            self.stem = ops.PackedStem(*packed, device=device)
            self.plan = self.plan[2:]
        self.device = device
        self.embedding_size = model.embedding_size
        self._skip_plans = {}
        self._mac_tables = {}
        self._const_crops = {}

    def skip_plan(self, size):
        key = (size, SKIP_ROWS, SKIP_MAC, SKIP_STRIPS)
        if key in self._skip_plans:
            return self._skip_plans[key]
        steps, layers, chain = None, [], []
        if self.stem is not None and size % 16 == 0 and size <= 1024:
            steps = [('stem', None, True, False)]
            chain += [0, 0, 1]
            h = size // 2
            layers.append(ops.skip_layer(h, h, 8, 8, len(chain), size, size, 0, 1))
            plan = self.plan + [('desc', None)]
            i = 0
            while steps is not None and i < len(plan):
                kind, pc = plan[i]
                if kind not in ('conv', 'conv_pool') or not (pc.cin_pad % 64 == 0 and (pc.kh, pc.kw, pc.stride, pc.pad) == (3, 3, 1, 1)
                                                             and pc.cout % 8 == 0 and pc.cout > 64 and pc.dtype == ops.BF16):
                    steps = None
                    break
                mac = kind == 'conv' and i + 1 < len(plan) and plan[i + 1][0] == 'desc' and pc.cout > 128 and ops.USE_FUSED_MAC
                after = plan[i + 2][0] if i + 2 < len(plan) else None
                pool = kind == 'conv_pool' or (mac and after == 'pool' and h % 2 == 0)
                store = not mac or after is not None
                th, tw = (16, 32) if pc.cout <= 128 else (16, 16)
                in_ops, oh = len(chain), h
                chain.append(0)
                if pool:
                    chain.append(1)
                    th, tw, oh = th // 2, tw // 2, h // 2
                if not store:
                    oh, th, tw = h, 16, 16
                mode = 0 if (mac and not SKIP_MAC) else (1 if not SKIP_ROWS else (3 if (SKIP_STRIPS and pc.cout > 128) else 2))
                layers.append(ops.skip_layer(oh, oh, th, tw, len(chain), h, h, in_ops, mode))
                steps.append(('conv', pc, pool, mac, store))
                i += (3 if pool else 2) if mac else 1
                if not mac and i < len(plan) and plan[i][0] != 'conv' and plan[i][0] != 'conv_pool':
                    steps = None
                    break
                h = oh
                if h % 16 != 0 and i < len(plan):
                    steps = None
            if steps is not None and len(chain) > 32:
                steps = None
        pool_mask = sum(1 << i for i, p in enumerate(chain) if p)
        self._skip_plans[key] = None if steps is None else (steps, layers, pool_mask)
        return self._skip_plans[key]

    def const_crop(self, mean, std, channels, size):
        key = (tuple(float(v) for v in mean), tuple(float(v) for v in std), int(channels), int(size))
        if key not in self._const_crops:
            img = torch.zeros((3, 1, 1), dtype=torch.float32, device=self.device)
            box = torch.zeros((1, 4), dtype=torch.float32, device=self.device)
            self._const_crops[key] = ops.crop_resize(img, box, size, mode=2 if channels == 4 else 1, mean=mean, std=std)[0].contiguous()
        return self._const_crops[key]

    def mac_tables(self, const_in, sched):
        key = (const_in.data_ptr(), id(sched))
        if key in self._mac_tables:
            return self._mac_tables[key]
        steps = sched[0]
        t = ops.vgg_stem(const_in[None].contiguous(), self.stem)
        tables = {}
        for li, (kind, pc, pool, mac, store) in enumerate(steps[1:], start=1):
            if not mac:
                t = ops.conv2d(t, pc, act=1, pool=pool)
                continue
            full = ops.conv2d(t, pc, act=1)
            m = full[0].to(torch.float32)
            zero = torch.zeros((1, m.shape[2]), dtype=torch.float32, device=m.device)
            rows = torch.cat((torch.cummax(m.amax(dim=1).flip(0), 0).values.flip(0), zero)).contiguous()
            cols = torch.cat((torch.cummax(m.amax(dim=0).flip(0), 0).values.flip(0), zero)).contiguous()
            tables[li] = (rows, cols)
            if store:
                t = ops.maxpool2d(full, 2, 2) if pool else full
        self._mac_tables[key] = tables
        self._keep_const = getattr(self, '_keep_const', []) + [const_in]
        return tables

    def _embed_skip(self, x, ext, const_in, sched):
        steps, layers, pool_mask = sched
        N, S, nl = x.shape[0], x.shape[1], len(steps)
        early = 1 + sum(1 for st in steps[1:] if st[1].cout <= 128 and not st[3])
        if any(st[1].cout <= 128 for st in steps[early:]):
            early = nl
        dev = x.device
        mac_skips = any(st[3] and layers[i][-1] for i, st in enumerate(steps) if i)
        tables = self.mac_tables(const_in, sched) if mac_skips else None

        def run(t, ext_, first, last, n_img, out_last=None):
            sub = layers[first:last]
            k = last - first
            res = ops.embed_worklists(ext_, n_img, S, pool_mask, sub, (S // 16) ** 2 if first == 0 else max(1, (sub[0][5] // 16)) ** 2,
                                      want_computed=mac_skips)
            lists, counts = res[0], res[1]
            if mac_skips:
                o = sum(st[1].cout for st in steps[1:first] if st[3])
                for j in range(k):
                    if steps[first + j][3] if first + j else False:
                        ops.mac_init(desc, o, tables[first + j][0], tables[first + j][1], res[2][j])
                        o += steps[first + j][1].cout
            off = sum(st[1].cout for st in steps[1:first] if st[3])
            for j in range(k):
                li = first + j
                if li == 0:
                    t = ops.vgg_stem_list(t, const_in, self.stem, lists[0], counts[0:1])
                    continue
                kind, pc, pool, mac, store = steps[li]
                t = ops.conv2d_list(t, pc, lists[j], counts[j:j + 1], act=1, pool=pool, mac=desc if mac else None, mac_off=off, store=store,
                                    units=counts[k + j:k + j + 1], out=out_last if (j == k - 1 and store) else None,
                                    strips=(lists[k + j], counts[2 * k + j:2 * k + j + 1]) if layers[li][-1] == 3 else None)
                if mac:
                    off += pc.cout
            return t

        desc = (torch.empty if mac_skips else torch.zeros)((N + 1, self.embedding_size), dtype=torch.float32, device=dev)
        if early >= nl:
            outs = []
            for s_, e_ in _passes(N, FUSED_EMBED_BATCH, FUSED_EMBED_MAX - 1):
                desc = (torch.empty if mac_skips else torch.zeros)((e_ - s_ + 1, self.embedding_size), dtype=torch.float32, device=dev)
                run(x[s_:e_], ext[s_:e_], 0, nl, e_ - s_ + 1)
                outs.append(desc[:e_ - s_])
            return torch.cat(outs)
        eh, ec = layers[early - 1][0], steps[early - 1][1].cout if early > 1 else 64
        big = torch.empty((N + 1, eh, eh, ec), dtype=torch.bfloat16, device=dev)
        for s_, e_ in _passes(N, FUSED_EMBED_BATCH, FUSED_EMBED_MAX - 1):
            if early == 1:
                big[s_:e_ + 1].copy_(run(x[s_:e_], ext[s_:e_], 0, 1, e_ - s_ + 1))
            else:
                run(x[s_:e_], ext[s_:e_], 0, early, e_ - s_ + 1, out_last=big[s_:e_ + 1])
        run(big, ext, early, nl, N + 1)
        return desc[:N]

    def will_skip(self, size):
        return bool(SKIP_PADDING and self.stem is not None and size * size <= INPUT_SIZE * INPUT_SIZE and self.skip_plan(size) is not None)

    def embed_packed(self, x, eps=1e-8, want_bf16=False, batch=None, ext=None, const_in=None, partial=False):
        outs, outs_bf = [], []
        fused = batch is None and self.stem is not None and x.shape[1] * x.shape[2] <= INPUT_SIZE * INPUT_SIZE
        step = batch or (FUSED_EMBED_BATCH if fused else MAX_EMBED_BATCH)
        plan = self.plan + [('desc', None)]
        sched = self.skip_plan(x.shape[1]) if (SKIP_PADDING and ext is not None and const_in is not None and fused and x.shape[1] == x.shape[2]) else None
        if partial and sched is None:
            raise RuntimeError('embed_packed: crops that hold their content only (ops.crop_resize content_ext) need the work-list schedule')
        if sched is not None and x.shape[0]:
            for s, e in _passes(x.shape[0], LATE_EMBED_MAX, LATE_EMBED_MAX):
                r = ops.l2_normalize(self._embed_skip(x[s:e], ext[s:e], const_in, sched).contiguous(), eps, want_bf16)
                if want_bf16:
                    outs.append(r[0]); outs_bf.append(r[1])
                else:
                    outs.append(r)
            if want_bf16:
                return torch.cat(outs), torch.cat(outs_bf)
            return torch.cat(outs)
        for s, e in _passes(x.shape[0], step, FUSED_EMBED_MAX if fused else step):
            xb = x[s:e]
            desc = torch.zeros((xb.shape[0], self.embedding_size), dtype=torch.float32, device=x.device)
            off = 0
            if self.stem is not None:
                xb = ops.vgg_stem(xb, self.stem)
            i = 0
            while i < len(plan):
                kind, pc = plan[i]
                nxt = plan[i + 1][0] if i + 1 < len(plan) else None
                if kind == 'conv' and nxt == 'desc' and ops.can_fuse_mac(xb, pc):
                    after = plan[i + 2][0] if i + 2 < len(plan) else None
                    fuse_pool = after == 'pool' and xb.shape[1] % 2 == 0 and xb.shape[2] % 2 == 0
                    xb = ops.conv2d_relu_mac(xb, pc, desc, off, store=after is not None, pool=fuse_pool)
                    off += pc.cout
                    i += 3 if fuse_pool else 2
                    continue
                if kind == 'conv':
                    xb = ops.conv2d(xb, pc, act=1)
                elif kind == 'conv_pool':
                    xb = ops.conv2d(xb, pc, act=1, pool=True)
                elif kind == 'pool':
                    xb = ops.maxpool2d(xb, 2, 2)
                else:
                    ops.global_max_into(xb, desc, off)
                    off += xb.shape[3]
                i += 1
            r = ops.l2_normalize(desc, eps, want_bf16)
            if want_bf16:
                outs.append(r[0]); outs_bf.append(r[1])
            else:
                outs.append(r)
        if not outs:
            e = torch.empty((0, self.embedding_size), dtype=torch.float32, device=x.device)
            return (e, e.to(torch.bfloat16)) if want_bf16 else e
        if want_bf16:
            return torch.cat(outs), torch.cat(outs_bf)
        return torch.cat(outs)


class MACVGG(nn.Module):

    embedding_size = 512 * 2
    input_mean, input_std = TANH_MEAN, TANH_STD

    def __init__(self, config='D', convs_per_block=[2, 2, 3, 3, 3], batch_norm=True, vgg_state_dict=None):
        super().__init__()
        feats = _vgg_features(VGG_CFGS[config], batch_norm)
        if vgg_state_dict is not None:
            holder = nn.Module()
            holder.features = nn.Sequential(*feats)
            holder.load_state_dict({k: v for k, v in vgg_state_dict.items() if k.startswith('features.')}, strict=True)
        per_conv = 3 if batch_norm else 2
        per_block = [c * per_conv + 1 for c in convs_per_block]
        cut1, cut2 = sum(per_block[:-1]) - 1, sum(per_block) - 1
        named = [(str(i), m) for i, m in enumerate(feats)]
        self.block1 = nn.Sequential(OrderedDict(named[:cut1]))
        self.block2 = nn.Sequential(OrderedDict(named[cut1:cut2]))
        self._engine = None
        self.eval()

    def load_state_dict(self, *a, **k):
        self._engine = None
        return super().load_state_dict(*a, **k)

    def _apply(self, fn, *a, **k):
        self._engine = None
        return super()._apply(fn, *a, **k)

    def engine(self):
        dev = next(self.parameters()).device
        if dev.type != 'cuda':
            raise RuntimeError('MACVGG runs on an MI355X (HIP) device only: call .cuda() first (no CPU fallback).')
        if self._engine is None:
            self._engine = MACVGGEngine(self, dev)
        return self._engine

    @torch.no_grad()
    def forward(self, x, eps=1e-8):
        eng = self.engine()
        x = x.to(device=eng.device, dtype=torch.float32)
        packed = ops.pack_embed_input(x, False, TANH_MEAN, TANH_STD)
        return eng.embed_packed(packed, eps)


def distance(emb1, emb2, dim=1):
    return 1 - torch.nn.functional.cosine_similarity(emb1, emb2, dim=dim)


@torch.no_grad()
def nearest_neighbors(anchors, queries, k=1, dtype=torch.float32):
    if not anchors.is_cuda or not queries.is_cuda:
        raise RuntimeError('nearest_neighbors runs on an MI355X (HIP) device only (no CPU fallback)')
    if len(queries) == 0:
        return torch.empty((0, k), dtype=torch.int64, device=queries.device)
    a = ops.pad_features(anchors.to(dtype))
    q = ops.pad_features(queries.to(dtype))
    return ops.match_topk(q, a, k)


def macvgg_embedder(model='vgg16_bn', pretrained=True, progress=True):
    model_to_config = {'vgg16': ('D', False), 'vgg16_bn': ('D', True)}
    if model not in model_to_config:
        raise NotImplementedError(f'MACVGG not implemented for {model}')
    if pretrained:
        raise RuntimeError('pretrained VGG weights cannot be downloaded here; use pretrained=False and load_state_dict')
    config, batchnorm = model_to_config[model]
    return MACVGG(config, batch_norm=batchnorm)


class _ResBottleneck(nn.Module):
    expansion = 4

    def __init__(self, inplanes, planes, stride, downsample, norm_layer):
        super().__init__()
        self.conv1, self.bn1 = nn.Conv2d(inplanes, planes, 1, bias=False), norm_layer(planes)
        self.conv2, self.bn2 = nn.Conv2d(planes, planes, 3, stride, 1, bias=False), norm_layer(planes)
        self.conv3, self.bn3 = nn.Conv2d(planes, planes * 4, 1, bias=False), norm_layer(planes * 4)
        self.relu = nn.ReLU(inplace=True)
        self.downsample = (nn.Sequential(nn.Conv2d(inplanes, planes * 4, 1, stride, bias=False), norm_layer(planes * 4))
                           if downsample else None)
        self.stride = stride


class _ResNetSource(nn.Module):

    def __init__(self, layers=(3, 4, 6, 3), norm_layer=nn.BatchNorm2d, stem=64, planes=(64, 128, 256, 512)):
        super().__init__()
        self.conv1, self.bn1 = nn.Conv2d(3, stem, 7, 2, 3, bias=False), norm_layer(stem)
        self.relu, self.maxpool = nn.ReLU(inplace=True), nn.MaxPool2d(3, 2, 1)
        inpl = stem
        for li, (planes, blocks) in enumerate(zip(planes, layers)):
            seq = []
            for bi in range(blocks):
                seq.append(_ResBottleneck(inpl, planes, 2 if (bi == 0 and li > 0) else 1, bi == 0, norm_layer))
                inpl = planes * 4
            setattr(self, f'layer{li + 1}', nn.Sequential(*seq))
        for m in self.modules():
            if isinstance(m, nn.Conv2d):
                nn.init.kaiming_normal_(m.weight, mode='fan_out', nonlinearity='relu')


class MACResNetEngine:
    def __init__(self, model, device):
        def fold(conv, bn):
            scale = shift = None
            if isinstance(bn, nn.BatchNorm2d):
                scale = bn.weight * (bn.running_var + bn.eps).rsqrt()
                shift = bn.bias - bn.running_mean * scale
            return ops.PackedConv(conv.weight, conv.bias, conv.stride[0], conv.padding[0], scale=scale, shift=shift, device=device)

        self.blocks = []
        for block in model.blocks:
            stages = []
            for layer in block:
                if isinstance(layer[0], nn.Conv2d):
                    stages.append(('stem', fold(layer[0], layer[1])))
                else:
                    for b in layer:
                        stages.append(('bottleneck', (fold(b.conv1, b.bn1), fold(b.conv2, b.bn2), fold(b.conv3, b.bn3),
                                                      fold(b.downsample[0], b.downsample[1]) if b.downsample is not None else None)))
            self.blocks.append(stages)
        self.device = device
        self.embedding_size = sum((st[-1][1].cout if st[-1][0] == 'stem' else st[-1][1][2].cout) for st in self.blocks)

    def embed_packed(self, x, eps=1e-8, batch=None):
        outs = []
        step = batch or MAX_EMBED_BATCH
        for s in range(0, x.shape[0], step):
            xb = x[s:s + step]
            desc = torch.empty((xb.shape[0], self.embedding_size), dtype=torch.float32, device=x.device)
            off = 0
            for stages in self.blocks:
                for kind, p in stages:
                    if kind == 'stem':
                        xb = ops.maxpool2d(ops.conv2d(xb, p, act=1), 3, 2, 1)
                    else:
                        c1, c2, c3, ds = p
                        identity = ops.conv2d(xb, ds) if ds is not None else xb
                        y = ops.conv2d(ops.conv2d(xb, c1, act=1), c2, act=1)
                        xb = ops.conv2d(y, c3, act=1, residual=identity)
                ops.global_max_into(xb, desc, off)
                off += xb.shape[3]
            outs.append(ops.l2_normalize(desc, eps))
        return torch.cat(outs) if outs else torch.empty((0, self.embedding_size), dtype=torch.float32, device=x.device)


class MACResNet(nn.Module):
    layer_output_sizes = [64, 256, 512, 1024, 2048]
    input_mean, input_std = (0.0, 0.0, 0.0), (1.0, 1.0, 1.0)

    def __init__(self, source_resnet, descriptor_layers=[2, 3]):
        super().__init__()
        layers = [nn.Sequential(source_resnet.conv1, source_resnet.bn1, source_resnet.relu, source_resnet.maxpool),
                  source_resnet.layer1, source_resnet.layer2, source_resnet.layer3, source_resnet.layer4]
        prev = 0
        self.blocks = nn.ModuleList()
        for l in descriptor_layers:
            self.blocks.append(nn.Sequential(*layers[prev:l + 1]))
            prev = l + 1
        self.embedding_size = sum(self.layer_output_sizes[l] for l in descriptor_layers)
        self._engine = None
        self.eval()

    def load_state_dict(self, *a, **k):
        self._engine = None
        return super().load_state_dict(*a, **k)

    def _apply(self, fn, *a, **k):
        self._engine = None
        return super()._apply(fn, *a, **k)

    def engine(self):
        dev = next(self.parameters()).device
        if dev.type != 'cuda':
            raise RuntimeError('MACResNet runs on an MI355X (HIP) device only: call .cuda() first (no CPU fallback).')
        if self._engine is None:
            self._engine = MACResNetEngine(self, dev)
        return self._engine

    @torch.no_grad()
    def forward(self, x, eps=1e-8):
        eng = self.engine()
        x = x.to(device=eng.device, dtype=torch.float32)
        assert x.shape[2] == x.shape[3], 'square inputs (the reference feeds 256x256 crops)'
        return eng.embed_packed(ops.pack_embed_input(x, False, self.input_mean, self.input_std), eps)


def macresnet_encoder(model='resnet50', pretrained=True, progress=True, batch_norm=True, desc_layers=[2, 3]):
    if model != 'resnet50':
        raise NotImplementedError(f'MACResNet not implemented for {model}')
    if pretrained:
        raise RuntimeError('pretrained ResNet weights cannot be downloaded here; use pretrained=False and load_state_dict')
    return MACResNet(_ResNetSource((3, 4, 6, 3), nn.BatchNorm2d if batch_norm else nn.Identity), desc_layers)
```

cvpce_amd/ops.py:

```python
import os as _os

import torch

from ._lib import lib
from .torch_ops import T
from . import torch_ops_input

BF16 = torch.bfloat16
F16 = torch.float16
STORAGE_TYPES = {'bf16': BF16, 'fp16': F16}
DEFAULT_DETECTOR_PRECISION = 'fp16'
F16_MAX = 65504.0


def to_storage(t, dtype):
    return t.clamp(-F16_MAX, F16_MAX).to(F16) if dtype == F16 else t.to(dtype)


def _need_cuda(*ts):
    for t in ts:
        if t is not None and not t.is_cuda:
            raise RuntimeError('cvpce_amd ops run on the GPU only (HIP kernels); got a CPU tensor. '
                               'There is no CPU fallback in the product path.')


FORCE_GENERIC_CONV = False
USE_HALO_3X3 = True
HALO_RAGGED = bool(int(_os.environ.get('CVPCE_HALO_RAGGED', '0')))
USE_HALO_THIN_OUT = _os.environ.get('CVPCE_HALO_THIN_OUT', '1') != '0'
USE_THIN_3X3 = _os.environ.get('CVPCE_THIN_3X3', '1') != '0'
USE_CONV1X1 = True
CONV1X1_STRIDE1 = _os.environ.get('CVPCE_CONV1X1_STRIDE1', '1') != '0'
CONV1X1_MAX_CIN = int(_os.environ.get('CVPCE_CONV1X1_MAX_CIN', '256'))
CONV1X1_ANY_SHAPE = bool(int(_os.environ.get('CVPCE_CONV1X1_ANY', '0')))
CONV_SPLITK = _os.environ.get('CVPCE_CONV_SPLITK', '1') != '0'
USE_FUSED_BOTTLENECK = _os.environ.get('CVPCE_FUSED_BOTTLENECK', '1') != '0'
FUSED_BOTTLENECK_MAX_PLANES = int(_os.environ.get('CVPCE_FUSED_BOTTLENECK_MAXP', '128'))
USE_FUSED_MAC = True
USE_GAUSS_TAIL = _os.environ.get('CVPCE_GAUSS_TAIL', '1') != '0'
USE_GAUSS_SUBNET = _os.environ.get('CVPCE_GAUSS_SUBNET', '1') != '0'
ONE_OUTPUT_BLOCK = _os.environ.get('CVPCE_ONE_OUTPUT_BLOCK', '1') != '0'
U8_KERNELS = _os.environ.get('CVPCE_U8_KERNELS', '0') != '0'


class PackedConv:

    def __init__(self, weight, bias=None, stride=1, pad=0, scale=None, shift=None, device='cuda', dtype=BF16):
        assert dtype in (BF16, F16)
        self.dtype = dtype
        w = weight.detach().to(torch.float32).cpu()
        cout, cin, kh, kw = w.shape
        b = bias.detach().to(torch.float32).cpu() if bias is not None else None
        if scale is not None:
            scale = scale.detach().to(torch.float32).cpu()
            w = w * scale[:, None, None, None]
            b = b * scale if b is not None else None
        if shift is not None:
            shift = shift.detach().to(torch.float32).cpu()
            b = shift if b is None else b + shift
        self.cin = cin
        self.cin_pad = (cin + 7) // 8 * 8
        self.cout, self.kh, self.kw, self.stride, self.pad = cout, kh, kw, stride, pad
        k = kh * kw * self.cin_pad
        kq = 64 if self.cin_pad % 64 == 0 else 32
        self.k_pad = (k + kq - 1) // kq * kq
        self.cout_pad = (cout + 255) // 256 * 256
        wp = torch.zeros(self.cout_pad, kh, kw, self.cin_pad, dtype=torch.float32)
        wp[:cout, :, :, :cin] = w.permute(0, 2, 3, 1)
        if self.cin_pad % 64 == 0:
            wp = wp.reshape(self.cout_pad, kh, kw, self.cin_pad // 64, 64).permute(0, 3, 1, 2, 4)
        packed = torch.zeros(self.cout_pad, self.k_pad, dtype=torch.float32)
        packed[:, :k] = wp.reshape(self.cout_pad, k)
        w16 = to_storage(packed, dtype)
        self.weight = w16.to(device)
        self.bias = b.to(device) if b is not None else None
        self.weight_halo = (self._to_halo_layout(w16, self.cout_pad, self.cin_pad).to(device)
                            if (kh, kw) == (3, 3) and self.cin_pad % 64 == 0 else None)

    @staticmethod
    def _to_halo_layout(weight, cout_pad, cin_pad):
        nch = cin_pad // 64
        v = weight.view(torch.int16).reshape(cout_pad // 32, 4, 2, 4, nch, 3, 3, 2, 4, 8)
        return v.permute(4, 0, 6, 7, 5, 2, 8, 1, 3, 9).contiguous().view(weight.dtype).reshape(-1)

    def out_hw(self, h, w, in_up_shift=0):
        h, w = h << in_up_shift, w << in_up_shift
        return ((h + 2 * self.pad - self.kh) // self.stride + 1, (w + 2 * self.pad - self.kw) // self.stride + 1)


def igemm_tile(pc, m):
    bk64 = pc.cin_pad % 64 == 0
    tiles256 = (m + 255) // 256
    if bk64 and not FORCE_GENERIC_CONV:
        if pc.cout >= 192 and tiles256 * ((pc.cout + 255) // 256) >= 128:
            return 'conv_dma16_kernel', (256, 256, 2, 4, 2, 4)
        if 64 < pc.cout <= 128 and tiles256 >= 128:
            return 'conv_dma_kernel', (128, 128, 2, 2, 2)
        if 32 < pc.cout <= 64 and tiles256 >= 128:
            return 'conv_dma_kernel', (64, 128, 2, 2, 2)
    tc = 128 if pc.cout > 64 else (32 if (pc.cout <= 32 and bk64) else 64)
    return 'conv_igemm_kernel', (tc, 128, 64 if bk64 else 32, 1 if tc == 32 else 2, 4 if tc == 32 else 2)


class ConvProfile:

    class _Records(list):
        SPLIT = ('conv3x3_halo2_kernel', 'conv3x3_halo3_kernel')
        stage = None

        def append(self, rec):
            if self.stage == 'detect' and rec[0] in self.SPLIT:
                rec = (rec[0] + '[detector]',) + tuple(rec[1:])
            list.append(self, rec)

    def __init__(self):
        self.records = ConvProfile._Records()
        self.byte_records = []
        self.layer_records = []

    def layer(self, key, flops, nbytes, e0, e1):
        self.layer_records.append((key, float(flops), float(nbytes), e0, e1))

    def summary_layers(self):
        torch.cuda.synchronize()
        out = {}
        for key, flops, nbytes, e0, e1 in self.layer_records:
            d = out.setdefault(key, {'launches': 0, 'flops': 0.0, 'bytes': 0.0, 'ms': 0.0})
            d['launches'] += 1
            d['flops'] += flops
            d['bytes'] += nbytes
            d['ms'] += e0.elapsed_time(e1)
        return out

    @staticmethod
    def variant(pc, m):
        kernel, args = igemm_tile(pc, m)
        return f"{kernel}<{','.join(map(str, args))}>"

    def summary(self):
        torch.cuda.synchronize()
        out = {}
        for rec in self.records:
            name, flops, e0, e1 = rec[:4]
            d = out.setdefault(name, {'launches': 0, 'flops': 0.0, 'flops_executed': 0.0, 'ms': 0.0})
            d['launches'] += 1
            d['flops'] += flops
            d['flops_executed'] += (float(rec[4].item()) * rec[5] if rec[4] is not None else 0.0) if len(rec) > 4 else flops
            d['ms'] += e0.elapsed_time(e1)
        return out

    def summary_bytes(self):
        torch.cuda.synchronize()
        out = {}
        for name, nbytes, e0, e1 in self.byte_records:
            d = out.setdefault(name, {'launches': 0, 'bytes': 0.0, 'ms': 0.0})
            d['launches'] += 1
            d['bytes'] += float(nbytes)
            d['ms'] += e0.elapsed_time(e1)
        return out


PROFILE = None


class _Launch:

    def __init__(self, prof):
        self.prof = prof
        self.e0, self.e1 = None, self._mark()

    @staticmethod
    def _mark():
        e = torch.cuda.Event(enable_timing=True)
        e.record()
        return e

    def stop(self):
        self.e0, self.e1 = self.e1, self._mark()

    def file(self, kernel, flops=None, nbytes=None, layer=None, hbm=False, extras=()):
        if flops is not None:
            self.prof.records.append((kernel, flops, self.e0, self.e1) + extras)
        if hbm:
            self.prof.byte_records.append((kernel, nbytes, self.e0, self.e1))
        if layer is not None:
            self.prof.layer(layer, flops or 0.0, nbytes, self.e0, self.e1)


def _start():
    prof = PROFILE
    return None if prof is None else _Launch(prof)


def _nbytes(*ts):
    return sum(t.numel() * t.element_size() for t in ts if t is not None)


def splitk_factor(pc, ho, wo):
    if not CONV_SPLITK or pc.cin_pad % 64 != 0 or pc.cout <= 64 or pc.k_pad // 64 < 32:
        return 0
    return 4 if ho * wo <= 1024 else 0


def conv_route(pc, n, h, w, act, out_f32, has_residual, in_up_shift, pool):
    if FORCE_GENERIC_CONV:
        return 'igemm', 0
    cin = pc.cin_pad
    ho, wo = pc.out_hw(h, w, in_up_shift)
    is_3x3 = (pc.kh, pc.kw, pc.stride, pc.pad) == (3, 3, 1, 1)
    input_fits = n * h * w * cin * 2 < 2 ** 32
    if (USE_HALO_THIN_OUT and is_3x3 and cin % 64 == 0 and pc.cout <= 64 and out_f32 and act == 0 and not has_residual and not in_up_shift
            and not pool and min(h, w) >= 48 and input_fits):
        return 'halo_thin_out', 0
    if (USE_HALO_3X3 and is_3x3 and cin % 64 == 0 and pc.cout > 64 and pc.cout % 8 == 0 and not out_f32 and act in (0, 1) and not has_residual
            and not in_up_shift and (HALO_RAGGED or (h % 16 == 0 and w % 16 == 0) or min(h, w) >= 48) and input_fits):
        return 'halo', 0
    thin_shape = ((cin, pc.cin, pc.k_pad) == (32, 32, 288) and pc.cout in (16, 32) and not in_up_shift) or \
                 ((cin, pc.cin, pc.k_pad) == (64, 64, 576) and pc.cout == 32 and in_up_shift == 1)
    if (USE_THIN_3X3 and is_3x3 and thin_shape and not out_f32 and act in (0, 1) and not has_residual and not pool
            and n * ho * wo * 64 < 2 ** 32 - 65536):
        return 'thin3x3', 0
    if (USE_CONV1X1 and (pc.kh, pc.kw, pc.pad) == (1, 1, 0) and cin % 64 == 0 and pc.k_pad == cin and pc.cout % 64 == 0
            and (CONV1X1_ANY_SHAPE or (pc.stride == 1 and CONV1X1_STRIDE1) or (cin <= CONV1X1_MAX_CIN and pc.cout >= 4 * cin))
            and not out_f32 and act in (0, 1) and not in_up_shift and not pool and input_fits):
        return 'conv1x1', 0
    if not pool:
        kernel, tile = igemm_tile(pc, n * ho * wo)
        if kernel == 'conv_igemm_kernel' and tile[0] == 128:
            ks = splitk_factor(pc, ho, wo)
            if ks:
                return 'splitk', ks
    return 'igemm', 0


def _splitk_workspace(pc, n, ho, wo, ks, device):
    cache = pc.__dict__.setdefault('_splitk_ws', {})
    key = (n, ho, wo, ks, device)
    ws = cache.get(key)
    if ws is None:
        ws = cache[key] = torch.empty(int(lib.cvpce_conv2d_splitk_workspace_bytes(n * ho * wo, pc.cout, ks)), dtype=torch.uint8, device=device)
    return ws


def conv2d(x, pc, act=0, out_f32=False, residual=None, res_mode=0, in_up_shift=0, out=None, pool=False):
    _need_cuda(x, residual)
    assert x.dtype == pc.dtype and x.is_contiguous() and x.dim() == 4, (x.dtype, pc.dtype)
    n, h, w, cin = x.shape
    assert cin == pc.cin_pad, (cin, pc.cin_pad)
    ho, wo = pc.out_hw(h, w, in_up_shift)
    oshape = (n, ho // 2, wo // 2, pc.cout) if pool else (n, ho, wo, pc.cout)
    odtype = torch.float32 if out_f32 else x.dtype
    if out is None:
        out = torch.empty(oshape, dtype=odtype, device=x.device)
    else:
        assert tuple(out.shape) == oshape and out.dtype == odtype and out.is_contiguous(), (tuple(out.shape), oshape, out.dtype, odtype)
    if residual is not None:
        assert residual.dtype == x.dtype and residual.is_contiguous() and residual.shape[0] == n and residual.shape[3] == pc.cout
        if res_mode == 0:
            res_mode = 1 if tuple(residual.shape[1:3]) == (ho, wo) else 2
    route, ks = conv_route(pc, n, h, w, act, out_f32, residual is not None, in_up_shift, pool)
    t = _start()
    if route == 'halo_thin_out':
        T.conv3x3_halo_thin_out(x, pc.weight_halo, pc.bias, out, pc.cout, pc.k_pad, pc.cout_pad)
    elif route == 'halo':
        T.conv3x3_halo(x, pc.weight_halo, pc.bias, out, pc.cout, pc.k_pad, pc.cout_pad, int(act), int(pool))
    elif route == 'thin3x3':
        T.conv3x3_thin(x, pc.weight, pc.bias, out, pc.cout, pc.k_pad, pc.cout_pad, int(act), int(in_up_shift))
    elif route == 'conv1x1':
        T.conv1x1_nhwc(x, pc.weight, pc.bias, residual, out, pc.cout, pc.stride, ho, wo, pc.k_pad, pc.cout_pad, int(act), int(res_mode))
    elif route == 'splitk':
        T.conv2d_splitk(x, pc.weight, pc.bias, residual, out, pc.cout, pc.kh, pc.kw, pc.stride, pc.pad, ho, wo, pc.k_pad, pc.cout_pad,
                        int(act), int(out_f32), int(in_up_shift), int(res_mode), ks, _splitk_workspace(pc, n, ho, wo, ks, x.device))
    else:
        T.conv2d_nhwc(x, pc.weight, pc.bias, residual, out, pc.cout, pc.kh, pc.kw, pc.stride, pc.pad, ho, wo, pc.k_pad, pc.cout_pad,
                      int(act), int(out_f32), int(in_up_shift), int(res_mode), int(pool), int(FORCE_GENERIC_CONV))
    if t is not None:
        t.stop()
        flops = 2.0 * n * ho * wo * pc.cout * pc.kh * pc.kw * pc.cin
        nbytes = _nbytes(x, out, residual, pc.weight)
        shape = f'{pc.cin}->{pc.cout}'
        if route == 'halo_thin_out':
            t.file('conv3x3_halo3_kernel', flops, nbytes, f'conv3x3_halo3 thin out {ho}x{wo} {shape} f32 out')
        elif route == 'halo':
            halo = 'conv3x3_halo3' if pc.cout <= 128 else 'conv3x3_halo2'
            t.file(halo + '_kernel', flops, nbytes, f'{halo} {h}x{w} {shape}' + (' +pool' if pool else ''))
        elif route == 'thin3x3':
            t.file('thin3x3_kernel', flops, nbytes, f'thin3x3 {ho}x{wo} {shape}' + (' (2x upsampled input)' if in_up_shift else ''), hbm=True)
        elif route == 'conv1x1':
            nbytes = n * ho * wo * cin * x.element_size() + _nbytes(out, residual, pc.weight)
            t.file('conv1x1_kernel', flops, nbytes, f'conv1x1 {ho}x{wo} {shape} s{pc.stride}' + (' +res' if residual is not None else ''), hbm=True)
        else:
            variant = ConvProfile.variant(pc, n * ho * wo)
            t.file(variant, flops, nbytes, f"{variant.split('<')[0]} {ho}x{wo} {shape} k{pc.kh} s{pc.stride}" + (' f32 out' if out_f32 else '')
                   + (f' split-K {ks}' if ks else ''))
    return out


def can_fuse_bottleneck(x, c1, c2, c3, residual):
    p = c1.cout
    n, h, w, cin = x.shape
    if residual is not None and not torch.is_tensor(residual):
        residual = torch.empty(tuple(residual), device='meta')
    return (USE_FUSED_BOTTLENECK and not FORCE_GENERIC_CONV and p in (64, 128, 256) and p <= FUSED_BOTTLENECK_MAX_PLANES and cin % 64 == 0 and c1.cin_pad == cin
            and (c1.kh, c1.stride, c1.pad) == (1, 1, 0) and (c2.kh, c2.kw, c2.stride, c2.pad) == (3, 3, 1, 1) and c2.cin == p and c2.cout == p
            and (c3.kh, c3.stride, c3.pad) == (1, 1, 0) and c3.cin == p and c3.cout == 4 * p and c2.k_pad == 9 * p
            and all(c.bias is not None for c in (c1, c2, c3)) and residual is not None and tuple(residual.shape) == (n, h, w, 4 * p)
            and n * h * w * max(cin, 4 * p) * 2 < 2 ** 32)


def pack_bottleneck_weights(c1, c2, c3):
    cached = c1.__dict__.get('_bneck_fm')
    if cached is not None and cached[0] is c2 and cached[1] is c3:
        return cached[2]
    p, cin = c1.cout, c1.cin_pad
    dev = c1.weight.device
    l16, lq, e = torch.arange(16), torch.arange(4), torch.arange(8)
    pair = 8 * (l16 >> 2) + (l16 & 3)

    def gather(w, cout, k):
        return w.view(torch.int16)[cout.to(dev), k.to(dev)].contiguous().view(w.dtype).reshape(-1)

    ks, b = torch.arange(cin // 32), torch.arange(p // 16)
    cout1 = (32 * (b >> 1) + 4 * (b & 1))[None, :, None, None, None] + pair[None, None, None, :, None]
    k1 = (32 * ks)[:, None, None, None, None] + (8 * lq)[None, None, :, None, None] + e[None, None, None, None, :]
    w1f = gather(c1.weight, cout1.expand(len(ks), len(b), 4, 16, 8), k1.expand(len(ks), len(b), 4, 16, 8))
    cw = 16 if p == 64 else 32
    ncb, ncg, ns = cw // 16, p // cw, (p // 64) * 6
    cg, st, kh, hh = torch.arange(ncg), torch.arange(ns), torch.arange(3), torch.arange(ncb)
    c64, kw, hf = st // 6, (st % 6) >> 1, st & 1
    row = (pair[None, :] + 4 * hh[:, None]) if ncb == 2 else l16[None, :].expand(1, 16)
    cout2 = (cw * cg)[:, None, None, None, None, None, None] + row[None, None, None, :, None, :, None]
    k2 = (((3 * c64)[:, None] + kh[None, :]) * 3 + kw[:, None]) * 64 + (32 * hf)[:, None]
    k2 = k2[None, :, :, None, None, None, None] + (8 * lq)[None, None, None, None, :, None, None] + e[None, None, None, None, None, None, :]
    shape2 = (ncg, ns, 3, ncb, 4, 16, 8)
    w2f = gather(c2.weight, cout2.expand(shape2), k2.expand(shape2))
    g32, ks3, h2 = torch.arange(4 * p // 32), torch.arange(p // 32), torch.arange(2)
    cout3 = (32 * g32)[:, None, None, None, None, None] + (4 * h2)[None, None, :, None, None, None] + pair[None, None, None, None, :, None]
    k3 = (32 * ks3)[None, :, None, None, None, None] + (8 * lq)[None, None, None, :, None, None] + e[None, None, None, None, None, :]
    shape3 = (len(g32), len(ks3), 2, 4, 16, 8)
    w3f = gather(c3.weight, cout3.expand(shape3), k3.expand(shape3))
    c1.__dict__['_bneck_fm'] = (c2, c3, (w1f, w2f, w3f))
    return w1f, w2f, w3f


def bottleneck(x, c1, c2, c3, residual):
    _need_cuda(x, residual)
    assert can_fuse_bottleneck(x, c1, c2, c3, residual) and x.dtype == c1.dtype == c2.dtype == c3.dtype == residual.dtype
    assert x.is_contiguous() and residual.is_contiguous()
    n, h, w, cin = x.shape
    p = c1.cout
    out = torch.empty((n, h, w, 4 * p), dtype=x.dtype, device=x.device)
    w1f, w2f, w3f = pack_bottleneck_weights(c1, c2, c3)
    t = _start()
    T.bottleneck_fused_fm(x, residual, w1f, c1.bias, w2f, c2.bias, w3f, c3.bias, out, p)
    if t is not None:
        t.stop()
        nbytes = _nbytes(x, out, c1.weight, c2.weight, c3.weight) + (0 if residual.data_ptr() == x.data_ptr() else _nbytes(residual))
        t.file('bneck_kernel', 2.0 * n * h * w * (cin * p + 9 * p * p + 4 * p * p), nbytes, f'bneck {h}x{w} {cin}->{p}->{4 * p}')
    return out


def can_fuse_mac(x, pc):
    n, h, w, _ = x.shape
    return (USE_FUSED_MAC and USE_HALO_3X3 and not FORCE_GENERIC_CONV and pc.cin_pad % 64 == 0 and pc.kh == 3 and pc.kw == 3 and pc.stride == 1
            and pc.pad == 1 and pc.cout % 8 == 0 and pc.cout > 128 and n * h * w * pc.cin_pad * 2 < 2 ** 32)


def conv2d_relu_mac(x, pc, mac, mac_off, store=True, pool=False):
    _need_cuda(x, mac)
    assert x.dtype == BF16 and pc.dtype == BF16 and x.is_contiguous() and x.dim() == 4 and mac.dtype == torch.float32 and mac.is_contiguous()
    assert can_fuse_mac(x, pc) and mac.shape[0] == x.shape[0] and mac_off + pc.cout <= mac.shape[1]
    n, h, w, cin = x.shape
    out = None
    if store:
        out = torch.empty((n, h // 2, w // 2, pc.cout) if pool else (n, h, w, pc.cout), dtype=BF16, device=x.device)
    t = _start()
    T.conv3x3_halo_mac(x, pc.weight_halo, pc.bias, out, mac, int(mac_off), pc.cout, pc.k_pad, pc.cout_pad, int(pool and store))
    if t is not None:
        t.stop()
        t.file('conv3x3_halo2_kernel', 2.0 * n * h * w * pc.cout * 9 * pc.cin)
    return out


class PackedStem:

    def __init__(self, w1, b1, w2, b2, device='cuda'):
        w1 = w1.detach().to(torch.float32).cpu()
        w2 = w2.detach().to(torch.float32).cpu()
        assert tuple(w1.shape) == (64, 3, 3, 3) and tuple(w2.shape) == (64, 64, 3, 3)
        p1 = torch.zeros(64, 3, 4, 4)
        p1[:, :, :3, :3] = w1.permute(0, 2, 3, 1)
        self.w1 = p1.reshape(64, 48).to(BF16).to(device)
        self.w2 = w2.permute(2, 3, 0, 1).reshape(9, 64, 64).contiguous().to(BF16).to(device)
        self.b1 = b1.detach().to(torch.float32).to(device)
        self.b2 = b2.detach().to(torch.float32).to(device)
        self.flops_per_pixel = 2.0 * 64 * (27 + 576)


class PackedGlnStem:

    def __init__(self, weight, scale, shift, device='cuda', dtype=BF16):
        self.dtype = dtype
        w = weight.detach().to(torch.float32).cpu() * scale.detach().to(torch.float32).cpu()[:, None, None, None]
        assert tuple(w.shape) == (64, 3, 7, 7)
        slots = torch.zeros(64, 7, 8, 4)
        slots[:, :, :7, :3] = w.permute(0, 2, 3, 1)
        f = slots.reshape(2, 32, 7, 2, 2, 2, 4).permute(0, 2, 3, 4, 1, 5, 6)
        self.w_frag = to_storage(f.reshape(2, 14, 64, 8).contiguous(), dtype).to(device)
        self.bias = shift.detach().to(torch.float32).to(device)


def gln_stem(x, ps):
    _need_cuda(x)
    assert x.dtype == ps.dtype and x.is_contiguous() and x.shape[3] == 8
    n, h, w, _ = x.shape
    hc, wc = (h - 1) // 2 + 1, (w - 1) // 2 + 1
    out = torch.empty((n, (hc - 1) // 2 + 1, (wc - 1) // 2 + 1, 64), dtype=x.dtype, device=x.device)
    t = _start()
    T.gln_stem_fused(x, ps.w_frag, ps.bias, out)
    if t is not None:
        t.stop()
        t.file('gln_stem_kernel', 2.0 * n * hc * wc * 64 * 147, _nbytes(x, out), f'gln_stem {h}x{w} 3->64 k7 s2 +pool')
    return out


def atlas_tile_map(mask, tile=16):
    m = mask.cpu().bool()
    h, w = m.shape
    tiles = [(ty << 16) | tx for ty in range((h + tile - 1) // tile) for tx in range((w + tile - 1) // tile)
             if bool(m[ty * tile:(ty + 1) * tile, tx * tile:(tx + 1) * tile].any())]
    return torch.tensor(tiles, dtype=torch.int32).to(mask.device)


def conv3x3_atlas(x, pc, mask, act=1, tile_map=None, out=None, mask_pixels=None):
    _need_cuda(x, mask, tile_map, out)
    assert x.dtype == pc.dtype and x.is_contiguous() and x.dim() == 4 and mask.dtype == torch.uint8 and mask.is_contiguous()
    n, h, w, cin = x.shape
    assert tuple(mask.shape) == (h, w) and cin == pc.cin_pad and pc.kh == 3 and pc.kw == 3 and pc.stride == 1 and pc.pad == 1
    assert pc.cin_pad % 64 == 0 and pc.cout % 8 == 0 and pc.cout > 128 and act in (0, 1)
    if tile_map is not None:
        assert out is not None and tile_map.dtype == torch.int32 and tile_map.is_contiguous()
    if out is None:
        out = torch.empty((n, h, w, pc.cout), dtype=x.dtype, device=x.device)
    assert tuple(out.shape) == (n, h, w, pc.cout) and out.dtype == x.dtype and out.is_contiguous()
    t = _start()
    T.conv3x3_halo_masked(x, pc.weight_halo, pc.bias, mask, tile_map, out, pc.cout, pc.k_pad, pc.cout_pad, int(act))
    if t is not None:
        t.stop()
        npix = float(mask.sum().item()) if mask_pixels is None else float(mask_pixels)
        t.file('conv3x3_halo2_kernel', 2.0 * npix * n * pc.cout * 9 * pc.cin, 2 * npix * n * (pc.cin + pc.cout) * x.element_size() + _nbytes(pc.weight),
               f'conv3x3_halo2 atlas {pc.cin}->{pc.cout} (head tower)')
    return out


def atlas_pack(levels, atlas, offs):
    _need_cuda(atlas, *levels)
    assert atlas.is_contiguous()
    T.atlas_pack(list(levels), atlas, [int(o[0]) for o in offs], [int(o[1]) for o in offs])


def atlas_unpack(atlas, shapes, offs):
    _need_cuda(atlas)
    assert atlas.is_contiguous()
    n, _, _, c = atlas.shape
    levels = [torch.empty((n, h, w, c), dtype=atlas.dtype, device=atlas.device) for (h, w) in shapes]
    T.atlas_unpack(atlas, levels, [int(o[0]) for o in offs], [int(o[1]) for o in offs])
    return levels


def vgg_stem(x, ps):
    _need_cuda(x)
    assert x.dtype == BF16 and x.is_contiguous() and x.shape[3] in (4, 8)
    n, h, w, c = x.shape
    out = torch.empty((n, h // 2, w // 2, 64), dtype=BF16, device=x.device)
    t = _start()
    T.vgg_stem_fused(x, ps.w1, ps.b1, ps.w2, ps.b2, out)
    if t is not None:
        t.stop()
        t.file('vgg_stem2_kernel', ps.flops_per_pixel * n * h * w)
    return out


def crop_extents(boxes, count, h0, w0, size=256, out=None, per_image=0):
    _need_cuda(boxes, count)
    boxes = boxes.to(torch.float32).contiguous()
    if out is None:
        out = torch.empty((boxes.shape[0], 2), dtype=torch.int32, device=boxes.device)
    T.crop_extents(boxes, count, int(per_image), int(h0), int(w0), int(size), out)
    return out


def pad_extents(images, pad=0.5):
    _need_cuda(images)
    ext = torch.empty((images.shape[0], 2), dtype=torch.int32, device=images.device)
    T.pad_extents(images, float(pad), ext)
    return ext


def skip_layer(h, w, tile_h, tile_w, out_ops, in_h, in_w, in_ops, skip):
    return [int(v) for v in (h, w, tile_h, tile_w, out_ops, in_h, in_w, in_ops, skip)]


def embed_worklists(ext0, n_images, size, pool_mask, layers, max_tiles, want_computed=False):
    _need_cuda(ext0)
    dev = ext0.device if ext0 is not None else torch.device('cuda', torch.cuda.current_device())
    lists = torch.empty((2 * len(layers), n_images * max_tiles), dtype=torch.int64, device=dev)
    counts = torch.empty((3 * len(layers),), dtype=torch.int32, device=dev)
    computed = torch.empty((len(layers), n_images, 2), dtype=torch.int32, device=dev) if want_computed else None
    T.embed_worklists(ext0, int(n_images), int(size), int(pool_mask), [v for l in layers for v in l], lists, counts, computed)
    return (lists, counts, computed) if want_computed else (lists, counts)


def mac_init(desc, off, row_suffix_max, col_suffix_max, computed):
    _need_cuda(desc, row_suffix_max, col_suffix_max, computed)
    T.mac_init(desc, int(off), row_suffix_max, col_suffix_max, computed)


def vgg_stem_list(x, const_in, ps, work, count):
    _need_cuda(x, const_in, work, count)
    assert x.dtype == BF16 and x.is_contiguous() and x.shape[3] in (4, 8) and const_in.is_contiguous()
    n1, h, w, c = x.shape
    out = torch.empty((n1 + 1, h // 2, w // 2, 64), dtype=BF16, device=x.device)
    t = _start()
    T.vgg_stem_fused_list(x, const_in, ps.w1, ps.b1, ps.w2, ps.b2, out, work, count)
    if t is not None:
        t.stop()
        t.file('vgg_stem2_kernel', ps.flops_per_pixel * n1 * h * w, extras=(count, ps.flops_per_pixel * 256, f'stem@{h}'))
    return out


def conv2d_list(x, pc, work, count, act=1, pool=False, mac=None, mac_off=0, store=True, units=None, strips=None, out=None):
    _need_cuda(x, work, count, mac)
    assert x.dtype == BF16 and pc.dtype == BF16 and x.is_contiguous() and x.dim() == 4
    assert pc.cin_pad % 64 == 0 and (pc.kh, pc.kw, pc.stride, pc.pad) == (3, 3, 1, 1) and pc.cout % 8 == 0 and pc.cout > 64
    n, h, w, cin = x.shape
    oshape = (n, h // 2, w // 2, pc.cout) if pool else (n, h, w, pc.cout)
    if not store:
        out = None
    elif out is None:
        out = torch.empty(oshape, dtype=BF16, device=x.device)
    else:
        assert tuple(out.shape) == oshape and out.dtype == BF16 and out.is_contiguous()
    t = _start()
    T.conv3x3_halo_list(x, pc.weight_halo, pc.bias, out, mac, int(mac_off), pc.cout, pc.k_pad, pc.cout_pad, int(act), int(pool and store), work, count)
    if t is not None:
        t.stop()
        wide = pc.cout <= 128
        tile_flops = 2.0 * 16 * (32 if wide else 16) * pc.cout * 9 * pc.cin
        tag = f'{pc.cin}->{pc.cout}@{h}' + ('mac' if mac is not None else '')
        lunits = (units - 4 * strips[1]) if (units is not None and strips is not None) else units
        t.file('conv3x3_halo3_kernel' if wide else 'conv3x3_halo2_kernel', 2.0 * (n - 1) * h * w * pc.cout * 9 * pc.cin,
               extras=((lunits, tile_flops / 16) if units is not None else (count, tile_flops)) + (tag,))
    if strips is not None:
        assert pc.cout > 128
        T.conv3x3_halo_strips(x, pc.weight_halo, pc.bias, out, mac, int(mac_off), pc.cout, pc.k_pad, pc.cout_pad, int(act), int(pool and store), strips[0], strips[1])
        if t is not None:
            t.stop()
            t.file('conv3x3_halo2_kernel[strips]', 0.0, extras=(strips[1], tile_flops / 4, tag))
    return out


def maxpool2d(x, k, stride, pad=0):
    _need_cuda(x)
    n, h, w, c = x.shape
    ho, wo = (h + 2 * pad - k) // stride + 1, (w + 2 * pad - k) // stride + 1
    out = torch.empty((n, ho, wo, c), dtype=x.dtype, device=x.device)
    T.maxpool2d_nhwc(x, out, k, stride, pad)
    return out


def relu(x):
    _need_cuda(x)
    out = torch.empty_like(x)
    T.relu(x, out)
    return out


def can_fuse_gauss_tail(x, c4, c5):
    return (USE_GAUSS_TAIL and not FORCE_GENERIC_CONV and x.shape[-1] == 16 and c4.dtype == c5.dtype == x.dtype
            and (c4.cin, c4.cin_pad, c4.cout, c4.kh, c4.kw, c4.stride, c4.pad) == (16, 16, 16, 1, 1, 1, 0)
            and (c5.cin, c5.cin_pad, c5.cout, c5.kh, c5.kw, c5.stride, c5.pad) == (16, 16, 1, 1, 1, 1, 0))


def gauss_tail(x, c4, c5, act):
    _need_cuda(x)
    assert can_fuse_gauss_tail(x, c4, c5) and x.is_contiguous() and act in (0, 1, 2)
    out = torch.empty(x.shape[:3] + (1,), dtype=torch.float32, device=x.device)
    t = _start()
    T.gauss_tail(x, c4.weight, c4.bias, c5.weight, c5.bias, out, c4.k_pad, int(act))
    if t is not None:
        t.stop()
        t.file('gauss_tail_kernel', 2.0 * x.shape[0] * x.shape[1] * x.shape[2] * (16 * 16 + 16), _nbytes(x, out),
               f'gauss_tail {x.shape[1]}x{x.shape[2]} 16->16->1', hbm=True)
    return out


def can_fuse_gauss_subnet(x, convs):
    if not (USE_GAUSS_SUBNET and not FORCE_GENERIC_CONV and len(convs) == 5 and x.dim() == 4 and x.shape[-1] == 64):
        return False
    c1, c2, c3, c4, c5 = convs
    shape = lambda c: (c.cin, c.cin_pad, c.cout, c.kh, c.kw, c.stride, c.pad, c.k_pad)
    return (all(c.dtype == x.dtype for c in convs) and shape(c1) == (64, 64, 32, 3, 3, 1, 1, 576) and shape(c2) == (32, 32, 32, 3, 3, 1, 1, 288)
            and shape(c3) == (32, 32, 16, 3, 3, 1, 1, 288) and shape(c4)[:7] == (16, 16, 16, 1, 1, 1, 0) and shape(c5)[:7] == (16, 16, 1, 1, 1, 1, 0)
            and c4.k_pad % 4 == 0 and x.numel() * 2 < 2 ** 32 - 65536)


def gauss_subnet(x, convs, act):
    _need_cuda(x)
    assert can_fuse_gauss_subnet(x, convs) and x.is_contiguous() and act in (0, 1, 2)
    c1, c2, c3, c4, c5 = convs
    n, hs, ws, _ = x.shape
    out = torch.empty((n, 2 * hs, 2 * ws, 1), dtype=torch.float32, device=x.device)
    t = _start()
    T.gauss_subnet(x, c1.weight, c1.bias, c2.weight, c2.bias, c3.weight, c3.bias, c4.weight, c4.bias, c4.k_pad, c5.weight, c5.bias, c5.k_pad, out, int(act))
    if t is not None:
        t.stop()
        t.file('gauss_subnet_kernel', 2.0 * n * 4 * hs * ws * (9 * 64 * 32 + 9 * 32 * 32 + 9 * 32 * 16 + 16 * 16 + 16), _nbytes(x, out),
               f'gauss_subnet {2 * hs}x{2 * ws} 64->32->32->16->16->1 (2x upsampled input)')
    return out


def global_max_into(x, out, out_off):
    _need_cuda(x, out)
    T.global_max_nhwc(x, out, out_off)


def l2_normalize(desc, eps=1e-8, want_bf16=False):
    _need_cuda(desc)
    out = torch.empty_like(desc)
    out_bf = torch.empty(desc.shape, dtype=BF16, device=desc.device) if want_bf16 else None
    T.l2_normalize(desc, out, out_bf, float(eps))
    return (out, out_bf) if want_bf16 else out


IMAGE_FORMS = 'float (3,H,W) in [0,1] or uint8 (H,W,3)'
_UINT8_TABLES = {}


def uint8_table(device=None):
    key = None if device is None else str(torch.device(device))
    t = _UINT8_TABLES.get(key)
    if t is None:
        t = torch.arange(256, dtype=torch.float32) / 255.0
        if key is not None and torch.device(device).type != 'cpu':
            t = t.to(device)
        _UINT8_TABLES[key] = t
    return t


def is_uint8_image(img):
    return torch.is_tensor(img) and img.dtype == torch.uint8


def check_image_form(img):
    if not torch.is_tensor(img):
        raise TypeError(f'an image is a tensor, {IMAGE_FORMS}; got {type(img).__name__}')
    if img.dtype == torch.uint8 and (img.dim() != 3 or img.shape[2] != 3):
        raise TypeError(f'an image is {IMAGE_FORMS}; got uint8 {tuple(img.shape)}')
    return img


def uint8_to_float(u):
    check_image_form(u)
    h, w, _ = u.shape
    idx = u.permute(2, 0, 1).to(torch.int32, memory_format=torch.contiguous_format).reshape(-1)
    return uint8_table(u.device).index_select(0, idx).view(3, h, w)


def device_image(img, device):
    check_image_form(img)
    if img.dtype != torch.uint8:
        return img.to(device=device, dtype=torch.float32).contiguous()
    if not img.is_cuda:
        img = img.to(device, non_blocking=img.is_pinned())
    return uint8_to_float(img)


def device_bytes(img, device):
    check_image_form(img)
    if img.dtype != torch.uint8:
        return img.to(device=device, dtype=torch.float32).contiguous()
    if not img.is_cuda:
        img = img.to(device, non_blocking=img.is_pinned())
    return img.contiguous()


def input_image(img, device):
    return device_bytes(img, device) if U8_KERNELS else device_image(img, device)


def gln_transform_into(img, batch, index, h, w, mean, std):
    _need_cuda(img, batch)
    assert img.dtype == torch.float32 and img.is_contiguous()
    _, hp, wp, c8 = batch.shape
    assert c8 == 8
    T.gln_transform(img, batch, index, h, w, [float(v) for v in mean], [float(v) for v in std])


def gln_transform_batch(images, batch, sizes, mean, std):
    _need_cuda(batch, *images)
    assert batch.shape[0] == len(images) == len(sizes) and batch.shape[3] == 8 and batch.is_contiguous()
    for i in images:
        check_image_form(i)
    has_bytes = any(i.dtype == torch.uint8 for i in images)
    if has_bytes and not U8_KERNELS:
        images, has_bytes = [uint8_to_float(i) if i.dtype == torch.uint8 else i for i in images], False
    t = _start()
    if has_bytes:
        T.gln_transform_batch_u8([i.contiguous() for i in images], uint8_table(batch.device), batch, [int(s[0]) for s in sizes],
                                 [int(s[1]) for s in sizes], [float(v) for v in mean], [float(v) for v in std])
    else:
        T.gln_transform_batch([i.contiguous() for i in images], batch, [int(s[0]) for s in sizes], [int(s[1]) for s in sizes],
                              [float(v) for v in mean], [float(v) for v in std])
    if t is not None:
        t.stop()
        t.file('gln_transform_batch_kernel', None, _nbytes(batch, *images), 'gln_transform_batch', hbm=True)


MAX_CROPS_PER_LAUNCH = 65528


def crop_resize(img, boxes, size=256, mode=0, mean=None, std=None, count=None, out=None, content_ext=None):
    _need_cuda(img, boxes)
    check_image_form(img)
    from_bytes = img.dtype == torch.uint8
    if from_bytes and not U8_KERNELS:
        img, from_bytes = uint8_to_float(img), False
    assert (from_bytes or img.dtype == torch.float32) and img.is_contiguous()
    table = uint8_table(img.device) if from_bytes else None
    boxes = boxes.to(torch.float32).contiguous()
    p = boxes.shape[0]
    if out is None:
        out = (torch.empty((p, 3, size, size), dtype=torch.float32, device=img.device) if mode == 0
               else torch.empty((p, size, size, 8 if mode == 1 else 4), dtype=BF16, device=img.device))
    assert out.shape[-1] == {0: size, 1: 8, 2: 4}[mode]
    m = [float(v) for v in mean] if mean is not None else None
    s = [float(v) for v in std] if std is not None else None
    prof = PROFILE
    for start in range(0, p, MAX_CROPS_PER_LAUNCH):
        nb = min(MAX_CROPS_PER_LAUNCH, p - start)
        cnt = None
        if count is not None:
            assert start == 0 and p <= MAX_CROPS_PER_LAUNCH
            cnt = count
        t = None if prof is None else _Launch(prof)
        if content_ext is not None:
            assert mode in (1, 2) and size % 2 == 0
            if from_bytes:
                T.crop_resize_content_u8(img, table, boxes[start:start + nb], cnt, out[start:start + nb], size, mode, m, s, content_ext[start:start + nb])
            else:
                T.crop_resize_content(img, boxes[start:start + nb], cnt, out[start:start + nb], size, mode, m, s, content_ext[start:start + nb])
        elif from_bytes:
            T.crop_resize_u8(img, table, boxes[start:start + nb], cnt, out[start:start + nb], size, mode, m, s)
        else:
            T.crop_resize(img, boxes[start:start + nb], cnt, out[start:start + nb], size, mode, m, s)
        if t is not None:
            t.stop()
            v = nb if cnt is None else int(cnt.reshape(-1)[0])
            b = boxes[start:start + v].to(torch.long)
            area = int(((b[:, 2] - b[:, 0]).clamp(min=0) * (b[:, 3] - b[:, 1]).clamp(min=0)).sum())
            if content_ext is not None:
                e = content_ext[start:start + v].to(torch.long)
                written = int((e[:, 0] * e[:, 1]).sum()) * out.shape[-1] * out.element_size()
            else:
                written = v * out[0].numel() * out.element_size()
            t.file('crop_resize_kernel', None, area * 3 * (1 if from_bytes else 4) + written, hbm=True)
    return out


def pack_embed_input(images, to_tanh, mean, std):
    _need_cuda(images)
    images = images.to(torch.float32).contiguous()
    b, _, s, s2 = images.shape
    assert s == s2
    out = torch.empty((b, s, s, 8), dtype=BF16, device=images.device)
    T.pack_embed_input(images, out, int(to_tanh), [float(v) for v in mean], [float(v) for v in std])
    return out


def detect_postprocess(logits, regs, grids, strides, base_anchors, image_hw, ratios, num_anchors, num_classes,
                       topk, score_thresh, nms_thresh, xform_clip, detections_per_img, conf_thresh):
    _need_cuda(*logits, *regs, base_anchors, image_hw, ratios)
    L, n = len(logits), logits[0].shape[0]
    dev = logits[0].device
    ws_bytes = lib.cvpce_detect_workspace_bytes(n, L, topk)
    ws = torch.empty(ws_bytes, dtype=torch.uint8, device=dev)
    nd = n * detections_per_img
    if ONE_OUTPUT_BLOCK:
        zero = torch.zeros(nd * 28 + n * 8, dtype=torch.uint8, device=dev)
        labels = zero[:nd * 8].view(torch.int64).view(n, detections_per_img)
        boxes = zero[nd * 8:nd * 24].view(torch.float32).view(n, detections_per_img, 4)
        scores = zero[nd * 24:nd * 28].view(torch.float32).view(n, detections_per_img)
        count = zero[nd * 28:nd * 28 + n * 4].view(torch.int32)
        conf = zero[nd * 28 + n * 4:].view(torch.int32)
    else:
        boxes = torch.zeros((n, detections_per_img, 4), dtype=torch.float32, device=dev)
        scores = torch.zeros((n, detections_per_img), dtype=torch.float32, device=dev)
        labels = torch.zeros((n, detections_per_img), dtype=torch.int64, device=dev)
        count = torch.zeros((n,), dtype=torch.int32, device=dev)
        conf = torch.zeros((n,), dtype=torch.int32, device=dev)
    for t in list(logits) + list(regs):
        assert t.dtype == torch.float32 and t.is_contiguous()
    t = _start()
    T.detect_postprocess(list(logits), list(regs), [int(g[0]) for g in grids], [int(g[1]) for g in grids], [int(s[0]) for s in strides],
                         [int(s[1]) for s in strides], base_anchors, image_hw, ratios, num_anchors, num_classes, topk, float(score_thresh),
                         float(nms_thresh), float(xform_clip), detections_per_img, float(conf_thresh), ws, boxes, scores, labels, count, conf)
    if t is not None:
        t.stop()
        t.file(None, None, _nbytes(*logits, *regs, boxes, scores, labels), f'detect_postprocess (top-k {topk}, NMS, dpi {detections_per_img}: 5 launches)')
    return boxes, scores, labels, count, conf


def clone_views(tensors):
    blocks, out = {}, []
    for t in tensors:
        st = t.untyped_storage()
        key = st.data_ptr()
        if key not in blocks:
            whole = torch.empty(0, dtype=torch.uint8, device=t.device).set_(st, 0, (st.nbytes(),), (1,))
            blocks[key] = whole.clone().untyped_storage()
        out.append(torch.empty(0, dtype=t.dtype, device=t.device).set_(blocks[key], t.storage_offset(), t.size(), t.stride()))
    return tuple(out)


def row_norms(x, eps=1e-8):
    _need_cuda(x)
    assert x.is_contiguous() and x.dtype in (BF16, torch.float32)
    out = torch.empty((x.shape[0],), dtype=torch.float32, device=x.device)
    T.row_norms(x, out, float(eps))
    return out


def match_topk(queries, gallery, k=1, q_norms=None, g_norms=None, return_distance=False):
    _need_cuda(queries, gallery)
    assert queries.dtype == gallery.dtype and queries.dtype in (BF16, torch.float32)
    assert queries.is_contiguous() and gallery.is_contiguous() and queries.shape[1] == gallery.shape[1]
    qn, d = queries.shape
    gn = gallery.shape[0]
    k = min(int(k), gn)
    if k == 0 or qn == 0:
        idx = torch.empty((qn, k), dtype=torch.int64, device=queries.device)
        return (idx, torch.empty((qn, k), dtype=torch.float32, device=queries.device)) if return_distance else idx
    if q_norms is None:
        q_norms = row_norms(queries)
    if g_norms is None:
        g_norms = row_norms(gallery)
    idx = torch.empty((qn, k), dtype=torch.int64, device=queries.device)
    dist = torch.empty((qn, k), dtype=torch.float32, device=queries.device) if return_distance else None
    ws_bytes = lib.cvpce_match_workspace_bytes(qn, gn, k)
    ws = torch.empty(ws_bytes, dtype=torch.uint8, device=queries.device)
    T.match_topk(queries, gallery, q_norms, g_norms, k, ws, idx, dist)
    return (idx, dist) if return_distance else idx


def match_set_core(core=0, nq=0, mg=0):
    return int(lib.cvpce_match_set_core(int(core), int(nq), int(mg)))


def pad_features(x, multiple=64):
    d = x.shape[1]
    dp = (d + multiple - 1) // multiple * multiple
    if dp == d:
        return x.contiguous()
    out = torch.zeros((x.shape[0], dp), dtype=x.dtype, device=x.device)
    out[:, :d] = x
    return out


def probe_mfma_bf16(shape, seconds=2.0, iters=20000, workgroups=256):
    import time
    dev = torch.device('cuda', torch.cuda.current_device())
    operands = torch.randn(1 << 16, device=dev).to(BF16)
    sink = torch.empty(workgroups * 256, dtype=torch.float32, device=dev)
    flop = workgroups * 4 * iters * 16 * (32768 if shape == 0 else 16384)
    launch = lambda: T.probe_mfma_bf16(int(shape), int(iters), operands, sink, int(workgroups))
    launch()
    torch.cuda.synchronize()
    t0, last = time.perf_counter(), 0.0
    while True:
        e0, e1 = torch.cuda.Event(enable_timing=True), torch.cuda.Event(enable_timing=True)
        e0.record()
        for _ in range(4):
            launch()
        e1.record()
        torch.cuda.synchronize()
        last = 4 * flop / (e0.elapsed_time(e1) * 1e-3) / 1e12
        if time.perf_counter() - t0 >= seconds:
            break
    return last


def probe_l2_stream(mib=2, seconds=1.0, workgroups=512, iters=64):
    import time
    dev = torch.device('cuda', torch.cuda.current_device())
    buf = torch.randint(0, 1 << 30, (mib << 18,), dtype=torch.int32, device=dev)
    sink = torch.empty(workgroups * 512, dtype=torch.float32, device=dev)
    T.probe_l2_stream(buf, 2, sink, workgroups)
    torch.cuda.synchronize()
    t0, last = time.perf_counter(), 0.0
    while True:
        e0, e1 = torch.cuda.Event(enable_timing=True), torch.cuda.Event(enable_timing=True)
        e0.record()
        T.probe_l2_stream(buf, iters, sink, workgroups)
        e1.record()
        torch.cuda.synchronize()
        last = workgroups * iters * (mib << 20) / (e0.elapsed_time(e1) * 1e-3) / 1e12
        if time.perf_counter() - t0 >= seconds:
            break
    return last
```

cvpce_amd/torch_ops.py:

```python
import ctypes

import torch

from . import _lib
from ._lib import lib, check

_L = torch.library.Library('cvpce_amd', 'DEF')
NAMES = []


def _stream():
    return ctypes.c_void_p(torch.cuda.current_stream().cuda_stream)


def _p(t):
    return ctypes.c_void_p(t.data_ptr()) if t is not None else ctypes.c_void_p(0)


def _by_dtype(x, bf16_name, f16_name, *same):
    if x.dtype not in (torch.bfloat16, torch.float16):
        raise RuntimeError(f'{bf16_name}: activations must be bfloat16 or float16, got {x.dtype}')
    for t in same:
        if t is not None and t.dtype != x.dtype:
            raise RuntimeError(f'{bf16_name}: operand of type {t.dtype} with {x.dtype} activations')
    return getattr(lib, f16_name if x.dtype == torch.float16 else bf16_name)


def _op(schema):
    def deco(fn):
        name = schema.split('(')[0]
        _L.define(schema)
        _L.impl(name, fn, 'CUDA')
        NAMES.append(name)
        return fn
    return deco


@_op('conv2d_nhwc(Tensor x, Tensor weight, Tensor? bias, Tensor? residual, Tensor(a!) out, int cout, int kh, int kw, int stride, '
     'int pad, int ho, int wo, int k_pad, int cout_pad, int act, int out_f32, int in_up_shift, int res_mode, int pool, '
     'int force_generic) -> ()')
def _conv2d_nhwc(x, weight, bias, residual, out, cout, kh, kw, stride, pad, ho, wo, k_pad, cout_pad, act, out_f32, in_up_shift,
                 res_mode, pool, force_generic):
    n, h, w, cin = x.shape
    hr, wr = (residual.shape[1], residual.shape[2]) if residual is not None else (0, 0)
    fn = _by_dtype(x, 'cvpce_conv2d_nhwc_bf16', 'cvpce_conv2d_nhwc_f16', weight, residual, None if out_f32 else out)
    check(fn(_p(x), _p(weight), _p(bias), _p(residual), _p(out), n, h, w, cin, cout, kh, kw, stride, pad, ho, wo,
             k_pad, cout_pad, act, out_f32, in_up_shift, res_mode if residual is not None else 0, hr, wr, pool,
             force_generic, _stream()), 'cvpce_conv2d_nhwc')


@_op('conv2d_splitk(Tensor x, Tensor weight, Tensor? bias, Tensor? residual, Tensor(a!) out, int cout, int kh, int kw, int stride, '
     'int pad, int ho, int wo, int k_pad, int cout_pad, int act, int out_f32, int in_up_shift, int res_mode, int ksplit, '
     'Tensor(b!) workspace) -> ()')
def _conv2d_splitk(x, weight, bias, residual, out, cout, kh, kw, stride, pad, ho, wo, k_pad, cout_pad, act, out_f32, in_up_shift,
                   res_mode, ksplit, workspace):
    n, h, w, cin = x.shape
    hr, wr = (residual.shape[1], residual.shape[2]) if residual is not None else (0, 0)
    fn = _by_dtype(x, 'cvpce_conv2d_splitk_bf16', 'cvpce_conv2d_splitk_f16', weight, residual, None if out_f32 else out)
    check(fn(_p(x), _p(weight), _p(bias), _p(residual), _p(out), n, h, w, cin, cout, kh, kw, stride, pad, ho, wo,
             k_pad, cout_pad, act, out_f32, in_up_shift, res_mode if residual is not None else 0, hr, wr, ksplit,
             _p(workspace), workspace.numel() * workspace.element_size(), _stream()), 'cvpce_conv2d_splitk')


@_op('conv1x1_nhwc(Tensor x, Tensor weight, Tensor? bias, Tensor? residual, Tensor(a!) out, int cout, int stride, int ho, int wo, '
     'int k_pad, int cout_pad, int relu, int res_mode) -> ()')
def _conv1x1_nhwc(x, weight, bias, residual, out, cout, stride, ho, wo, k_pad, cout_pad, relu, res_mode):
    n, h, w, cin = x.shape
    hr, wr = (residual.shape[1], residual.shape[2]) if residual is not None else (0, 0)
    fn = _by_dtype(x, 'cvpce_conv1x1_nhwc_bf16', 'cvpce_conv1x1_nhwc_f16', weight, residual, out)
    check(fn(_p(x), _p(weight), _p(bias), _p(residual), _p(out), n, h, w, cin, cout, stride, ho, wo, k_pad,
             cout_pad, relu, res_mode if residual is not None else 0, hr, wr, _stream()), 'cvpce_conv1x1_nhwc')


@_op('conv3x3_halo(Tensor x, Tensor weight, Tensor? bias, Tensor(a!) out, int cout, int k_pad, int cout_pad, int relu, int pool) -> ()')
def _conv3x3_halo(x, weight, bias, out, cout, k_pad, cout_pad, relu, pool):
    n, h, w, cin = x.shape
    fn = _by_dtype(x, 'cvpce_conv3x3_halo', 'cvpce_conv3x3_halo_f16', weight, out)
    check(fn(_p(x), _p(weight), _p(bias), _p(out), n, h, w, cin, cout, k_pad, cout_pad, relu, pool, _stream()), 'cvpce_conv3x3_halo')


@_op('conv3x3_halo_thin_out(Tensor x, Tensor weight, Tensor? bias, Tensor(a!) out, int cout, int k_pad, int cout_pad) -> ()')
def _conv3x3_halo_thin_out(x, weight, bias, out, cout, k_pad, cout_pad):
    n, h, w, cin = x.shape
    if out.dtype != torch.float32:
        raise RuntimeError('cvpce_conv3x3_halo_thin_out: the output is float32')
    fn = _by_dtype(x, 'cvpce_conv3x3_halo_thin_out', 'cvpce_conv3x3_halo_thin_out_f16', weight)
    check(fn(_p(x), _p(weight), _p(bias), _p(out), n, h, w, cin, cout, k_pad, cout_pad, _stream()), 'cvpce_conv3x3_halo_thin_out')


@_op('conv3x3_halo_mac(Tensor x, Tensor weight, Tensor? bias, Tensor(a!)? out, Tensor(b!) mac, int mac_off, int cout, int k_pad, '
     'int cout_pad, int pool) -> ()')
def _conv3x3_halo_mac(x, weight, bias, out, mac, mac_off, cout, k_pad, cout_pad, pool):
    n, h, w, cin = x.shape
    if x.dtype != torch.bfloat16 or weight.dtype != torch.bfloat16:
        raise RuntimeError('cvpce_conv3x3_halo_mac: bf16 only (the embedder has no fp16 mode)')
    check(lib.cvpce_conv3x3_halo_mac(_p(x), _p(weight), _p(bias), _p(out), _p(mac), mac.shape[1], mac_off, n, h, w, cin, cout, k_pad,
                                     cout_pad, pool, _stream()), 'cvpce_conv3x3_halo_mac')


@_op('conv3x3_halo_masked(Tensor x, Tensor weight, Tensor? bias, Tensor mask, Tensor? tile_map, Tensor(a!) out, int cout, int k_pad, '
     'int cout_pad, int relu) -> ()')
def _conv3x3_halo_masked(x, weight, bias, mask, tile_map, out, cout, k_pad, cout_pad, relu):
    n, h, w, cin = x.shape
    fn = _by_dtype(x, 'cvpce_conv3x3_halo_masked', 'cvpce_conv3x3_halo_masked_f16', weight, out)
    check(fn(_p(x), _p(weight), _p(bias), _p(mask), _p(tile_map), tile_map.numel() if tile_map is not None else 0,
             _p(out), n, h, w, cin, cout, k_pad, cout_pad, relu, _stream()), 'cvpce_conv3x3_halo_masked')


@_op('bottleneck_fused_fm(Tensor x, Tensor res, Tensor w1f, Tensor b1, Tensor w2f, Tensor b2, Tensor w3f, Tensor b3, Tensor(a!) out, int planes) -> ()')
def _bottleneck_fused_fm(x, res, w1f, b1, w2f, b2, w3f, b3, out, planes):
    n, h, w, cin = x.shape
    if w1f.numel() != planes * cin or w2f.numel() != 9 * planes * planes or w3f.numel() != 4 * planes * planes:
        raise RuntimeError('cvpce_bottleneck_fused_fm: fragment-major weights of the wrong size')
    fn = _by_dtype(x, 'cvpce_bottleneck_fused_fm', 'cvpce_bottleneck_fused_fm_f16', res, w1f, w2f, w3f, out)
    check(fn(_p(x), _p(res), _p(w1f), _p(b1), _p(w2f), _p(b2), _p(w3f), _p(b3), _p(out), n, h, w, cin, planes, _stream()), 'cvpce_bottleneck_fused_fm')


@_op('vgg_stem_fused(Tensor x, Tensor w1, Tensor b1, Tensor w2, Tensor b2, Tensor(a!) out) -> ()')
def _vgg_stem_fused(x, w1, b1, w2, b2, out):
    n, h, w, c = x.shape
    if x.dtype != torch.bfloat16 or w1.dtype != torch.bfloat16 or w2.dtype != torch.bfloat16:
        raise RuntimeError('cvpce_vgg_stem_fused: bf16 only (the embedder has no fp16 mode)')
    check(lib.cvpce_vgg_stem_fused(_p(x), c, _p(w1), _p(b1), _p(w2), _p(b2), _p(out), n, h, w, _stream()), 'cvpce_vgg_stem_fused')


@_op('gln_stem_fused(Tensor x, Tensor w_frag, Tensor bias, Tensor(a!) out) -> ()')
def _gln_stem_fused(x, w_frag, bias, out):
    n, h, w, c = x.shape
    fn = _by_dtype(x, 'cvpce_gln_stem_fused', 'cvpce_gln_stem_fused_f16', w_frag, out)
    check(fn(_p(x), _p(w_frag), _p(bias), _p(out), n, h, w, _stream()), 'cvpce_gln_stem_fused')


@_op('maxpool2d_nhwc(Tensor x, Tensor(a!) out, int k, int stride, int pad) -> ()')
def _maxpool2d_nhwc(x, out, k, stride, pad):
    n, h, w, c = x.shape
    fn = _by_dtype(x, 'cvpce_maxpool2d_nhwc_bf16', 'cvpce_maxpool2d_nhwc_f16', out)
    check(fn(_p(x), _p(out), n, h, w, c, k, stride, pad, out.shape[1], out.shape[2], _stream()), 'maxpool')


@_op('relu(Tensor x, Tensor(a!) out) -> ()')
def _relu(x, out):
    check(_by_dtype(x, 'cvpce_relu_bf16', 'cvpce_relu_f16', out)(_p(x), _p(out), x.numel(), _stream()), 'relu')


@_op('conv3x3_thin(Tensor x, Tensor weight, Tensor? bias, Tensor(a!) out, int cout, int k_pad, int cout_pad, int relu, int in_up_shift) -> ()')
def _conv3x3_thin(x, weight, bias, out, cout, k_pad, cout_pad, relu, in_up_shift):
    n, h, w, cin = x.shape
    fn = _by_dtype(x, 'cvpce_conv3x3_thin_bf16', 'cvpce_conv3x3_thin_f16', weight, out)
    check(fn(_p(x), _p(weight), _p(bias), _p(out), n, h << in_up_shift, w << in_up_shift, cin, cout, k_pad, cout_pad, relu, in_up_shift, _stream()),
          'cvpce_conv3x3_thin')


@_op('gauss_tail(Tensor x, Tensor w2, Tensor? b2, Tensor w3, Tensor? b3, Tensor(a!) out, int k2_pad, int act) -> ()')
def _gauss_tail(x, w2, b2, w3, b3, out, k2_pad, act):
    assert x.shape[-1] == 16 and out.dtype == torch.float32 and out.numel() == x.numel() // 16
    check(_by_dtype(x, 'cvpce_gauss_tail_bf16', 'cvpce_gauss_tail_f16', w2, w3)(_p(x), _p(w2), _p(b2), _p(w3), _p(b3), _p(out), x.numel() // 16,
                                                                               k2_pad, act, _stream()), 'gauss_tail')


@_op('gauss_subnet(Tensor x, Tensor w1, Tensor? b1, Tensor w2, Tensor? b2, Tensor w3, Tensor? b3, Tensor w4, Tensor? b4, int k4_pad, '
     'Tensor w5, Tensor? b5, int k5_pad, Tensor(a!) out, int act) -> ()')
def _gauss_subnet(x, w1, b1, w2, b2, w3, b3, w4, b4, k4_pad, w5, b5, k5_pad, out, act):
    n, hs, ws, c = x.shape
    assert c == 64 and out.dtype == torch.float32 and tuple(out.shape[:3]) == (n, 2 * hs, 2 * ws) and out.numel() == n * 4 * hs * ws
    fn = _by_dtype(x, 'cvpce_gauss_subnet_bf16', 'cvpce_gauss_subnet_f16', w1, w2, w3, w4, w5)
    check(fn(_p(x), _p(w1), _p(b1), _p(w2), _p(b2), _p(w3), _p(b3), _p(w4), _p(b4), k4_pad, _p(w5), _p(b5), k5_pad, _p(out), n, 2 * hs, 2 * ws, act,
             _stream()), 'gauss_subnet')


@_op('global_max_nhwc(Tensor x, Tensor(a!) out, int out_off) -> ()')
def _global_max_nhwc(x, out, out_off):
    n, h, w, c = x.shape
    check(lib.cvpce_global_max_nhwc_bf16(_p(x), _p(out), n, h * w, c, out.shape[1], out_off, _stream()), 'global_max')


@_op('l2_normalize(Tensor x, Tensor(a!) out, Tensor(b!)? out_bf16, float eps) -> ()')
def _l2_normalize(x, out, out_bf16, eps):
    check(lib.cvpce_l2_normalize_f32(_p(x), _p(out), _p(out_bf16), x.shape[0], x.shape[1], eps, _stream()), 'l2norm')


@_op('gln_transform(Tensor img, Tensor(a!) batch, int index, int h, int w, float[] mean, float[] std) -> ()')
def _gln_transform(img, batch, index, h, w, mean, std):
    _, hp, wp, _ = batch.shape
    fn = _by_dtype(batch, 'cvpce_gln_transform', 'cvpce_gln_transform_f16')
    check(fn(_p(img), ctypes.c_void_p(batch[index].data_ptr()), img.shape[1], img.shape[2], h, w, hp, wp,
             _lib.float3(mean), _lib.float3(std), _stream()), 'gln_transform')


@_op('gln_transform_batch(Tensor[] imgs, Tensor(a!) batch, int[] h, int[] w, float[] mean, float[] std) -> ()')
def _gln_transform_batch(imgs, batch, h, w, mean, std):
    n, hp, wp, _ = batch.shape
    if len(imgs) != n or len(h) != n or len(w) != n:
        raise RuntimeError('gln_transform_batch: one image and one resized size per batch slot')
    for t in imgs:
        if t.dtype != torch.float32 or not t.is_contiguous() or t.dim() != 3 or t.shape[0] != 3:
            raise RuntimeError('gln_transform_batch: images must be contiguous (3,H,W) float32 tensors')
    ci = lambda v: (ctypes.c_int * n)(*[int(x) for x in v])
    ptrs = (ctypes.c_void_p * n)(*[t.data_ptr() for t in imgs])
    fn = _by_dtype(batch, 'cvpce_gln_transform_batch', 'cvpce_gln_transform_batch_f16')
    check(fn(ptrs, ci([t.shape[1] for t in imgs]), ci([t.shape[2] for t in imgs]), ci(h), ci(w), n, _p(batch), hp, wp,
             _lib.float3(mean), _lib.float3(std), _stream()), 'gln_transform_batch')


@_op('crop_resize(Tensor img, Tensor boxes, Tensor? count, Tensor(a!) out, int size, int mode, float[]? mean, float[]? std) -> ()')
def _crop_resize(img, boxes, count, out, size, mode, mean, std):
    check(lib.cvpce_crop_resize(_p(img), _p(boxes), _p(count), boxes.shape[0], _p(out), img.shape[1], img.shape[2], size, mode,
                                _lib.float3(mean) if mean is not None else None, _lib.float3(std) if std is not None else None,
                                _stream()), 'crop_resize')


@_op('crop_resize_content(Tensor img, Tensor boxes, Tensor? count, Tensor(a!) out, int size, int mode, float[] mean, float[] std, Tensor ext) -> ()')
def _crop_resize_content(img, boxes, count, out, size, mode, mean, std, ext):
    if ext.dtype != torch.int32 or not ext.is_contiguous() or ext.shape != (boxes.shape[0], 2):
        raise RuntimeError('crop_resize_content: ext must be a contiguous (P,2) int32 tensor')
    check(lib.cvpce_crop_resize_content(_p(img), _p(boxes), _p(count), boxes.shape[0], _p(out), img.shape[1], img.shape[2], size, mode,
                                        _lib.float3(mean), _lib.float3(std), _p(ext), _stream()), 'crop_resize_content')


@_op('crop_extents(Tensor boxes, Tensor? count, int per_image, int h0, int w0, int size, Tensor(a!) ext) -> ()')
def _crop_extents(boxes, count, per_image, h0, w0, size, ext):
    if boxes.dtype != torch.float32 or not boxes.is_contiguous() or ext.dtype != torch.int32 or not ext.is_contiguous() or ext.numel() < 2 * boxes.shape[0] \
            or (per_image > 0 and (count is None or count.numel() * per_image < boxes.shape[0])):
        raise RuntimeError('crop_extents: boxes (P,4) float32, ext (P,2) int32, both contiguous; per_image > 0 needs one count per image')
    check(lib.cvpce_crop_extents(_p(boxes), _p(count), boxes.shape[0], per_image, h0, w0, size, _p(ext), _stream()), 'cvpce_crop_extents')


@_op('pad_extents(Tensor images, float pad, Tensor(a!) ext) -> ()')
def _pad_extents(images, pad, ext):
    if images.dtype != torch.float32 or not images.is_contiguous() or images.dim() != 4 or images.shape[1] != 3 or images.shape[2] != images.shape[3] \
            or ext.dtype != torch.int32 or not ext.is_contiguous() or ext.numel() < 2 * images.shape[0]:
        raise RuntimeError('pad_extents: images (B,3,S,S) float32 contiguous, ext (B,2) int32')
    check(lib.cvpce_pad_extents(_p(images), images.shape[0], images.shape[2], pad, _p(ext), _stream()), 'cvpce_pad_extents')


@_op('mac_init(Tensor(a!) desc, int off, Tensor row_suffix_max, Tensor col_suffix_max, Tensor computed) -> ()')
def _mac_init(desc, off, row_suffix_max, col_suffix_max, computed):
    c = row_suffix_max.shape[1]
    if desc.dtype != torch.float32 or not desc.is_contiguous() or row_suffix_max.dtype != torch.float32 or col_suffix_max.dtype != torch.float32 \
            or not row_suffix_max.is_contiguous() or not col_suffix_max.is_contiguous() or col_suffix_max.shape[1] != c \
            or computed.dtype != torch.int32 or not computed.is_contiguous() or computed.numel() < 2 * desc.shape[0]:
        raise RuntimeError('mac_init: bad argument shapes / types')
    check(lib.cvpce_mac_init(_p(desc), desc.shape[0], desc.shape[1], off, c, _p(row_suffix_max), _p(col_suffix_max), row_suffix_max.shape[0] - 1,
                             col_suffix_max.shape[0] - 1, _p(computed), _stream()), 'cvpce_mac_init')


@_op('embed_worklists(Tensor? ext0, int n_images, int size, int pool_mask, int[] layers, Tensor(a!) lists, Tensor(b!) counts, '
     'Tensor(c!)? computed) -> ()')
def _embed_worklists(ext0, n_images, size, pool_mask, layers, lists, counts, computed):
    nf = len(_lib.SkipLayer._fields_)
    nl = len(layers) // nf
    if len(layers) != nl * nf or lists.dtype != torch.int64 or not lists.is_contiguous() or lists.shape[0] != 2 * nl or counts.dtype != torch.int32 \
            or counts.numel() != 3 * nl or (ext0 is not None and (ext0.dtype != torch.int32 or not ext0.is_contiguous() or ext0.numel() < 2 * (n_images - 1))):
        raise RuntimeError('embed_worklists: bad argument shapes / types')
    arr = (_lib.SkipLayer * nl)(*[_lib.SkipLayer(*[int(v) for v in layers[i * nf:(i + 1) * nf]]) for i in range(nl)])
    if computed is not None and (computed.dtype != torch.int32 or not computed.is_contiguous() or computed.numel() < 2 * nl * n_images):
        raise RuntimeError('embed_worklists: computed must be a contiguous int32 tensor of (n_layers, n_images, 2)')
    check(lib.cvpce_embed_worklists(_p(ext0), n_images, size, pool_mask, ctypes.cast(arr, ctypes.c_void_p), nl, _p(lists), lists.shape[1], _p(counts),
                                    _p(computed), _stream()), 'cvpce_embed_worklists')


@_op('vgg_stem_fused_list(Tensor x, Tensor const_in, Tensor w1, Tensor b1, Tensor w2, Tensor b2, Tensor(a!) out, Tensor work, Tensor count) -> ()')
def _vgg_stem_fused_list(x, const_in, w1, b1, w2, b2, out, work, count):
    n1, h, w, c = x.shape
    if x.dtype != torch.bfloat16 or const_in.dtype != torch.bfloat16 or tuple(const_in.shape[-3:]) != (h, w, c) or out.shape[0] != n1 + 1 \
            or work.dtype != torch.int64 or count.dtype != torch.int32:
        raise RuntimeError('cvpce_vgg_stem_fused_list: bad argument shapes / types')
    check(lib.cvpce_vgg_stem_fused_list(_p(x), c, _p(const_in), _p(w1), _p(b1), _p(w2), _p(b2), _p(out), n1 + 1, h, w, _p(work), _p(count),
                                        _stream()), 'cvpce_vgg_stem_fused_list')


def _halo_list(fn, what, x, weight, bias, out, mac, mac_off, cout, k_pad, cout_pad, relu, pool, work, count):
    n, h, w, cin = x.shape
    if x.dtype != torch.bfloat16 or weight.dtype != torch.bfloat16 or work.dtype != torch.int64 or count.dtype != torch.int32:
        raise RuntimeError(f'{what}: bf16 activations, int64 work list, int32 count')
    check(fn(_p(x), _p(weight), _p(bias), _p(out), _p(mac), mac.shape[1] if mac is not None else 0, mac_off, n, h, w,
             cin, cout, k_pad, cout_pad, relu, pool, _p(work), _p(count), _stream()), what)


@_op('conv3x3_halo_list(Tensor x, Tensor weight, Tensor? bias, Tensor(a!)? out, Tensor(b!)? mac, int mac_off, int cout, int k_pad, '
     'int cout_pad, int relu, int pool, Tensor work, Tensor count) -> ()')
def _conv3x3_halo_list(x, weight, bias, out, mac, mac_off, cout, k_pad, cout_pad, relu, pool, work, count):
    _halo_list(lib.cvpce_conv3x3_halo_list, 'cvpce_conv3x3_halo_list', x, weight, bias, out, mac, mac_off, cout, k_pad, cout_pad, relu, pool, work, count)


@_op('conv3x3_halo_strips(Tensor x, Tensor weight, Tensor? bias, Tensor(a!)? out, Tensor(b!)? mac, int mac_off, int cout, int k_pad, '
     'int cout_pad, int relu, int pool, Tensor work, Tensor count) -> ()')
def _conv3x3_halo_strips(x, weight, bias, out, mac, mac_off, cout, k_pad, cout_pad, relu, pool, work, count):
    _halo_list(lib.cvpce_conv3x3_halo_strips, 'cvpce_conv3x3_halo_strips', x, weight, bias, out, mac, mac_off, cout, k_pad, cout_pad, relu, pool, work, count)


@_op('pack_embed_input(Tensor images, Tensor(a!) out, int to_tanh, float[] mean, float[] std) -> ()')
def _pack_embed_input(images, out, to_tanh, mean, std):
    check(lib.cvpce_pack_embed_input(_p(images), _p(out), images.shape[0], images.shape[2], to_tanh, _lib.float3(mean), _lib.float3(std),
                                     _stream()), 'pack_embed_input')


@_op('detect_postprocess(Tensor[] logits, Tensor[] regs, int[] gh, int[] gw, int[] sh, int[] sw, Tensor base_anchors, Tensor image_hw, '
     'Tensor ratios, int num_anchors, int num_classes, int topk, float score_thresh, float nms_thresh, float xform_clip, '
     'int detections_per_img, float conf_thresh, Tensor(a!) workspace, Tensor(b!) boxes, Tensor(c!) scores, Tensor(d!) labels, '
     'Tensor(e!) count, Tensor(f!) conf) -> ()')
def _detect_postprocess(logits, regs, gh, gw, sh, sw, base_anchors, image_hw, ratios, num_anchors, num_classes, topk, score_thresh,
                        nms_thresh, xform_clip, detections_per_img, conf_thresh, workspace, boxes, scores, labels, count, conf):
    L, n = len(logits), logits[0].shape[0]
    lp = (ctypes.c_void_p * L)(*[t.data_ptr() for t in logits])
    rp = (ctypes.c_void_p * L)(*[t.data_ptr() for t in regs])
    ci = lambda v: (ctypes.c_int * L)(*[int(x) for x in v])
    check(lib.cvpce_detect_postprocess(lp, rp, ci(gh), ci(gw), ci(sh), ci(sw), _p(base_anchors), _p(image_hw), _p(ratios), L, n,
                                       num_anchors, num_classes, topk, score_thresh, nms_thresh, xform_clip, detections_per_img,
                                       conf_thresh, _p(workspace), workspace.numel(), _p(boxes), _p(scores), _p(labels), _p(count),
                                       _p(conf), _stream()), 'cvpce_detect_postprocess')


def _atlas_copy(levels, atlas, oy, ox, to_atlas):
    L = len(levels)
    n, hc, wc, c = atlas.shape
    lp = (ctypes.c_void_p * L)(*[t.data_ptr() for t in levels])
    ci = lambda v: (ctypes.c_int * L)(*[int(x) for x in v])
    for t in levels:
        if t.dtype != atlas.dtype or t.shape[0] != n or t.shape[3] != c or not t.is_contiguous():
            raise RuntimeError('atlas_copy: levels must be contiguous (N,h,w,C) tensors of the atlas dtype / batch / channels')
    check(lib.cvpce_atlas_copy(lp, ci([t.shape[1] for t in levels]), ci([t.shape[2] for t in levels]), ci(oy), ci(ox), L, n, _p(atlas),
                               hc, wc, c * atlas.element_size(), int(to_atlas), _stream()), 'cvpce_atlas_copy')


@_op('atlas_pack(Tensor[] levels, Tensor(a!) atlas, int[] oy, int[] ox) -> ()')
def _atlas_pack(levels, atlas, oy, ox):
    _atlas_copy(levels, atlas, oy, ox, True)


@_op('atlas_unpack(Tensor atlas, Tensor(a!)[] levels, int[] oy, int[] ox) -> ()')
def _atlas_unpack(atlas, levels, oy, ox):
    _atlas_copy(levels, atlas, oy, ox, False)


@_op('row_norms(Tensor x, Tensor(a!) out, float eps) -> ()')
def _row_norms(x, out, eps):
    check(lib.cvpce_row_norms(_p(x), _p(out), x.shape[0], x.shape[1], int(x.dtype == torch.float32), eps, _stream()), 'row_norms')


@_op('match_topk(Tensor queries, Tensor gallery, Tensor q_norms, Tensor g_norms, int k, Tensor(a!) workspace, Tensor(b!) idx, '
     'Tensor(c!)? dist) -> ()')
def _match_topk(queries, gallery, q_norms, g_norms, k, workspace, idx, dist):
    check(lib.cvpce_match_topk(_p(queries), _p(gallery), _p(q_norms), _p(g_norms), queries.shape[0], gallery.shape[0], queries.shape[1], k,
                               int(queries.dtype == torch.float32), _p(workspace), workspace.numel(), _p(idx), _p(dist), _stream()),
          'cvpce_match_topk')


@_op('probe_mfma_bf16(int shape, int iters, Tensor operands, Tensor(a!) sink, int workgroups) -> ()')
def _probe_mfma_bf16(shape, iters, operands, sink, workgroups):
    check(lib.cvpce_probe_mfma_bf16(shape, iters, _p(operands), _p(sink), workgroups, _stream()), 'probe')


@_op('probe_l2_stream(Tensor buf, int iters, Tensor(a!) sink, int workgroups) -> ()')
def _probe_l2_stream(buf, iters, sink, workgroups):
    check(lib.cvpce_probe_l2_stream(_p(buf), buf.numel() * buf.element_size(), iters, _p(sink), workgroups, _stream()), 'probe_l2_stream')


T = torch.ops.cvpce_amd
```

Before: 278.4 images/s.

## Add 2-row strip work lists to skip finer empty regions in embed convs

Adds a finer-grained skip mode in which wide halo conv layers process 2-row strips (four per workgroup) in addition to 4-row strips, using a third work list produced by the worklist builder. The kernel template gains a strip-height parameter, with adjusted LDS read scheduling, waitcnt values and row predication, and a new strips2 entry point is exposed through ctypes and torch ops. The goal is to avoid MFMA work on rows that fall outside crop content in the VGG embed. In exchange it adds an extra kernel launch per layer and partially filled workgroups, and it makes the mode selection more complex. It is on by default through environment flags.

```diff
diff --git a/cvpce_amd/_lib.py b/cvpce_amd/_lib.py
--- a/cvpce_amd/_lib.py
+++ b/cvpce_amd/_lib.py
@@ -97,7 +97,11 @@
     'cvpce_planogram_match': (c_int, [_ip] * 11 + [c_int] * 6 + [c_longlong, _vp, c_size_t, _ip, _ip, _vp]),
 }
 
-for _table in (SIGNATURES, EVAL_SIGNATURES, INPUT_SIGNATURES, PLANOGRAM_SIGNATURES):
+LISTS_SIGNATURES = {
+    'cvpce_conv3x3_halo_strips2': SIGNATURES['cvpce_conv3x3_halo_strips'],
+}
+
+for _table in (SIGNATURES, EVAL_SIGNATURES, INPUT_SIGNATURES, PLANOGRAM_SIGNATURES, LISTS_SIGNATURES):
     for _name, (_res, _args) in _table.items():
         _fn = getattr(lib, _name)
         _fn.restype = _res
diff --git a/cvpce_amd/csrc/conv3x3_halo2.hip b/cvpce_amd/csrc/conv3x3_halo2.hip
--- a/cvpce_amd/csrc/conv3x3_halo2.hip
+++ b/cvpce_amd/csrc/conv3x3_halo2.hip
@@ -1,5 +1,6 @@
 #include "halo_common.h"
 #include "../../include/cvpce_amd.h"
+#include "../../include/cvpce_amd_lists.h"
 
 typedef __attribute__((address_space(3))) void lds_void;
 typedef __attribute__((address_space(3))) char lds_char;
@@ -48,11 +49,14 @@
 }
 #endif
 
-template <typename E, bool POOL, bool GMAX, bool LIST, bool STRIP = false, int NW = 8>
+template <typename E, bool POOL, bool GMAX, bool LIST, int SH = 0, int NW = 8>
 __global__ __launch_bounds__(64 * NW, NW == 8 ? 2 : 1) void conv3x3_halo2_kernel(Halo2Args a) {
+    constexpr bool STRIP = SH != 0;
+    static_assert(SH == 0 || SH == 2 || SH == 4, "strip height");
     static_assert(!STRIP || LIST, "strips come from a work list");
     static_assert(NW == 8 || NW == 4, "cout waves");
-    constexpr int TC = 32 * NW, NB = 16, NS = STRIP ? 3 : 1;
+    constexpr int TC = 32 * NW, NB = 16, NS = SH == 4 ? 3 : (SH == 2 ? 4 : 1);
+    constexpr int SHD = STRIP ? SH : 1, PR = SH + 2;
 
     extern __shared__ __attribute__((aligned(16))) unsigned char smem[];
     unsigned char* Ap = smem;
@@ -69,7 +73,7 @@
     int my_tiles, l_first = 0, l_entries = 0;
     if constexpr (LIST) {
         l_entries = __builtin_amdgcn_readfirstlane(*a.list_count);
-        const int units = STRIP ? (l_entries + 2) / 3 : l_entries;
+        const int units = STRIP ? (l_entries + NS - 1) / NS : l_entries;
         const int groups = (int)gridDim.x / a.ctiles;
         const int per = (units + groups - 1) / groups;
         l_first = (lbid / a.ctiles) * per;
@@ -162,17 +166,26 @@
                 const int py = pp / G2_P, px = pp - py * G2_P;
                 const int lchunk = (ln & 7) ^ g2_swz(py, px);
                 int sn = n[0], sty = ty[0], stx = tx[0], sext = ext[0], ry = py;
-                if constexpr (STRIP) {
+                bool in_strip = true;
+                if constexpr (SH == 4) {
                     const int st = py >= 12 ? 2 : (py >= 6 ? 1 : 0);
                     ry = py - 6 * st;
                     sn = st == 0 ? n[0] : (st == 1 ? n[1] : n[2]);
                     sty = st == 0 ? ty[0] : (st == 1 ? ty[1] : ty[2]);
                     stx = st == 0 ? tx[0] : (st == 1 ? tx[1] : tx[2]);
                     sext = st == 0 ? ext[0] : (st == 1 ? ext[1] : ext[2]);
+                } else if constexpr (SH == 2) {
+                    const int st = py >> 2;
+                    in_strip = st < NS;
+                    ry = py & 3;
+                    sn = st == 0 ? n[0] : (st == 1 ? n[1] : (st == 2 ? n[2] : n[3]));
+                    sty = st == 0 ? ty[0] : (st == 1 ? ty[1] : (st == 2 ? ty[2] : ty[3]));
+                    stx = st == 0 ? tx[0] : (st == 1 ? tx[1] : (st == 2 ? tx[2] : tx[3]));
+                    sext = st == 0 ? ext[0] : (st == 1 ? ext[1] : (st == 2 ? ext[2] : ext[3]));
                 }
                 const int ey = wl_ey((unsigned)sext), ex = wl_ex((unsigned)sext);
                 const int y = sty * G2_T - 1 + ry, x = stx * G2_T - 1 + px;
-                const bool ok = pp < G2_NPIX && (unsigned)y < (unsigned)a.H && (unsigned)x < (unsigned)a.W;
+                const bool ok = pp < G2_NPIX && (unsigned)y < (unsigned)a.H && (unsigned)x < (unsigned)a.W && in_strip;
                 int nn = sn;
                 if constexpr (LIST) nn = (y >= ey || x >= ex) ? a.N - 1 : sn;
                 const unsigned off = (unsigned)((((size_t)(nn * a.H + y) * a.W + x) * a.Cin + c * 64) * 2) + (unsigned)(lchunk * 16);
@@ -245,7 +258,7 @@
         e1 = (x_ ^ 16u) + (BUFB);                                                                              \
     }
 #define G2_READ(T, P)                                                                                          \
-    if constexpr (!(CVPCE_DBG & 32)) {                                                                         \
+    if constexpr (!(CVPCE_DBG & 32) && !(SH == 2 && (P) >= 16)) {                                              \
         if constexpr (((P) & 1) == 0)                                                                          \
             asm volatile("ds_read_b128 %0, %1 offset:%2" : "=v"(bfr[((P) + 2 * (T)) & 3]) : "v"(e0), "n"(((P) * G2_P + ((T) >> 1)) * 128)); \
         else                                                                                                   \
@@ -253,16 +266,16 @@
     }
 #define G2_ROW_KH(T, P, KH)                                                                                    \
     {                                                                                                          \
-        constexpr int j_ = STRIP ? (P) % 6 - (KH) : (P) - (KH);                                                \
-        constexpr int r_ = STRIP ? 4 * ((P) / 6) + j_ : j_;                                                    \
-        if constexpr (j_ >= 0 && j_ < (STRIP ? 4 : NB)) {                                                      \
+        constexpr int j_ = STRIP ? (P) % PR - (KH) : (P) - (KH);                                               \
+        constexpr int r_ = STRIP ? SH * ((P) / PR) + j_ : j_;                                                  \
+        if constexpr (j_ >= 0 && j_ < (STRIP ? SH : NB) && (!STRIP || (P) / PR < NS)) {                        \
             _Pragma("unroll") for (int mt_ = 0; mt_ < 2; ++mt_)                                                \
                 acc[mt_][r_] = E::mfma16(af[(T) & 1][KH][mt_], bfr[((P) + 2 * (T)) & 3], acc[mt_][r_]);       \
         }                                                                                                      \
     }
 #define G2_ROW(T, P)                                                                                           \
     {                                                                                                          \
-        asm volatile("s_waitcnt lgkmcnt(2)" : "+v"(bfr[((P) + 2 * (T)) & 3]));                                 \
+        asm volatile("s_waitcnt lgkmcnt(%1)" : "+v"(bfr[((P) + 2 * (T)) & 3]) : "n"(SH == 2 && ((P) == 14 || (P) == 15) ? 15 - (P) : 2)); \
         G2_ROW_KH(T, P, 0) G2_ROW_KH(T, P, 1) G2_ROW_KH(T, P, 2)                                               \
         __builtin_amdgcn_sched_barrier(0);                                                                     \
     }
@@ -273,17 +286,27 @@
         if (!(CVPCE_DBG & 64)) __builtin_amdgcn_s_barrier();                                                   \
         issue_next_patch();                                                                                    \
     }
+#define G2_MORE(R) (!LIST || SH == 4 || (SH == 2 ? (R) < 14 : rows_ > (R)))
+#define G2_STALE_LANDED()                                                                                      \
+    {                                                                                                          \
+        asm volatile("s_waitcnt lgkmcnt(0)" ::: "memory");                                                     \
+        __builtin_amdgcn_sched_barrier(0);                                                                     \
+    }
 #define G2_ROWS_AND_TAIL(T, TN, BUFB_NEXT, BEFORE)                                                             \
-    G2_RP(T, 0) G2_RP(T, 1) G2_RP(T, 2) G2_RP(T, 3) G2_RP(T, 4) G2_RP(T, 5)                                    \
-    if (!LIST || STRIP || rows_ > 4) { G2_RP(T, 6) G2_RP(T, 7) G2_RP(T, 8) G2_RP(T, 9) }                       \
-    if (!LIST || STRIP || rows_ > 8) { G2_RP(T, 10) G2_RP(T, 11) G2_RP(T, 12) G2_RP(T, 13) }                   \
-    if (!LIST || STRIP || rows_ > 12) {                                                                        \
-        G2_RP(T, 14) G2_RP(T, 15)                                                                              \
+    G2_RP(T, 0) G2_RP(T, 1) G2_RP(T, 2) G2_RP(T, 3)                                                            \
+    if (G2_MORE(2)) { G2_RP(T, 4) G2_RP(T, 5) }                                                                \
+    if (G2_MORE(4)) { G2_RP(T, 6) G2_RP(T, 7) }                                                                \
+    if (G2_MORE(6)) { G2_RP(T, 8) G2_RP(T, 9) }                                                                \
+    if (G2_MORE(8)) { G2_RP(T, 10) G2_RP(T, 11) }                                                              \
+    if (G2_MORE(10)) { G2_RP(T, 12) G2_RP(T, 13) }                                                             \
+    if (G2_MORE(12)) { G2_RP(T, 14) G2_RP(T, 15) }                                                             \
+    if (G2_MORE(14)) {                                                                                         \
         BEFORE                                                                                                 \
         G2_SET_E(TN, BUFB_NEXT)                                                                                \
         G2_READ(TN, 0) G2_ROW(T, 16)                                                                           \
         G2_READ(TN, 1) G2_ROW(T, 17)                                                                           \
     } else {                                                                                                   \
+        G2_STALE_LANDED()                                                                                      \
         BEFORE                                                                                                 \
         G2_SET_E(TN, BUFB_NEXT)                                                                                \
         G2_READ(TN, 0)                                                                                         \
@@ -298,7 +321,7 @@
 
     int seq = 0, cchunk = 0, t_n[NS], t_ty[NS], t_tx[NS], t_ct, t_ext_[NS];
     tile_of(0, t_n, t_ty, t_tx, t_ct, t_ext_);
-    int rows_ = (LIST && !STRIP) ? wl_rows((unsigned)t_ext_[0]) : NB;
+    int rows_ = (LIST && !STRIP) ? wl_rows((unsigned)t_ext_[0]) : (SH == 2 ? 14 : NB);
     int n_ct = t_ct;
     auto next_ct = [&]() {
         if (cchunk + 1 < nchunks) return t_ct;
@@ -348,12 +371,12 @@
 
         if (cchunk + 1 == nchunks) {
             const int ct = t_ct;
-            const int rows_t = STRIP ? 4 : rows_;
-            auto e_n = [&](int nt) { return STRIP ? t_n[(nt >> 2) < NS ? (nt >> 2) : 0] : t_n[0]; };
-            auto e_ty = [&](int nt) { return STRIP ? t_ty[(nt >> 2) < NS ? (nt >> 2) : 0] : t_ty[0]; };
-            auto e_tx = [&](int nt) { return STRIP ? t_tx[(nt >> 2) < NS ? (nt >> 2) : 0] : t_tx[0]; };
-            auto e_row = [&](int nt) { return STRIP ? (nt & 3) : nt; };
-            auto e_live = [&](int nt) { return STRIP ? nt < 12 : (!LIST || nt < rows_t); };
+            const int rows_t = STRIP ? SH : rows_;
+            auto e_n = [&](int nt) { return STRIP ? t_n[(nt / SHD) < NS ? (nt / SHD) : 0] : t_n[0]; };
+            auto e_ty = [&](int nt) { return STRIP ? t_ty[(nt / SHD) < NS ? (nt / SHD) : 0] : t_ty[0]; };
+            auto e_tx = [&](int nt) { return STRIP ? t_tx[(nt / SHD) < NS ? (nt / SHD) : 0] : t_tx[0]; };
+            auto e_row = [&](int nt) { return STRIP ? (nt % SHD) : nt; };
+            auto e_live = [&](int nt) { return STRIP ? nt < NS * SH : (!LIST || nt < rows_t); };
             f32x4 nbias[2];
             load_bias(n_ct, nbias);
             const int col = halo_col(lp);
@@ -367,7 +390,7 @@
                     const int n = t_n[sg], ty = t_ty[sg], tx = t_tx[sg];
                     if (tx * G2_T + col < a.W) {
 #pragma unroll
-                        for (int nt = STRIP ? 4 * sg : 0; nt < (STRIP ? 4 * sg + 4 : NB); ++nt)
+                        for (int nt = STRIP ? SH * sg : 0; nt < (STRIP ? SH * sg + SH : NB); ++nt)
                             if (ty * G2_T + e_row(nt) < a.H && e_live(nt)) {
 #pragma unroll
                                 for (int j = 0; j < 4; ++j) {
@@ -459,6 +482,8 @@
 #undef G2_STEP
 #undef G2_HANDOFF
 #undef G2_ROWS_AND_TAIL
+#undef G2_MORE
+#undef G2_STALE_LANDED
 #undef G2_RP
 #undef G2_ROW
 #undef G2_ROW_KH
@@ -468,7 +493,7 @@
 #undef G2_LOAD_A
 }
 
-template <typename E, bool POOL, bool GMAX, bool LIST = false, bool STRIP = false>
+template <typename E, bool POOL, bool GMAX, bool LIST = false, int SH = 0>
 static int launch_halo2(Halo2Args a, hipStream_t stream) {
     a.ctiles = (a.Cout + 255) / 256;
     a.ntiles = a.ptiles * a.ctiles;
@@ -476,13 +501,13 @@
         if (!a.mask && a.Cout % 128 == 0 && 2 * a.ntiles <= g_cvpce_persistent_wgs) {
             a.ctiles = a.Cout / 128;
             a.ntiles = a.ptiles * a.ctiles;
-            return halo_launch<conv3x3_halo2_kernel<E, false, false, false, false, 4>>(a, a.ntiles, 256, 3 * G2_A_BYTES, stream);
+            return halo_launch<conv3x3_halo2_kernel<E, false, false, false, 0, 4>>(a, a.ntiles, 256, 3 * G2_A_BYTES, stream);
         }
     }
     const int smem = a.mask ? G2_SMEM_MASKED : (LIST ? G2_SMEM_LIST : 3 * G2_A_BYTES);
     const int grid = halo_grid(a.ntiles, a.ctiles, LIST);
     if (a.mask && (a.ntiles + grid - 1) / grid > G2_MAX_SEQ) return CVPCE_ERR_ARG;
-    return halo_launch<conv3x3_halo2_kernel<E, POOL, GMAX, LIST, STRIP>>(a, grid, 512, smem, stream, G2_SMEM_MASKED);
+    return halo_launch<conv3x3_halo2_kernel<E, POOL, GMAX, LIST, SH>>(a, grid, 512, smem, stream, G2_SMEM_MASKED);
 }
 
 static Halo2Args halo2_args(const void* in, const void* wgt, const float* bias, void* out, float* gmax, int gmax_stride, int gmax_off,
@@ -574,12 +599,12 @@
 
 static int halo_list_launch(const void* in, const void* wgt, const float* bias, void* out, float* mac, int mac_stride,
                             int mac_off, int N, int H, int W, int Cin, int Cout, int K_pad, int Cout_pad, int relu,
-                            int fuse_pool2, const unsigned long long* list, const int* count_dev, bool strips, void* stream) {
+                            int fuse_pool2, const unsigned long long* list, const int* count_dev, int strip_h, void* stream) {
     if (N <= 0) return CVPCE_OK;
     if ((!out && !mac) || !list || !count_dev) return CVPCE_ERR_ARG;
     if (mac && !halo2_gmax_ok(relu, Cout, mac_stride, mac_off)) return CVPCE_ERR_ARG;
     if (Cout <= 128) {
-        if (strips) return CVPCE_ERR_ARG;
+        if (strip_h) return CVPCE_ERR_ARG;
         return cvpce_conv3x3_halo_wide_list(in, wgt, bias, out, N, H, W, Cin, Cout, K_pad, Cout_pad, relu, fuse_pool2, list, count_dev, stream);
     }
     const HaloShape sh{N, H, W, Cin, Cout, K_pad, Cout_pad};
@@ -587,20 +612,27 @@
     Halo2Args a = halo2_args(in, wgt, bias, out, mac, mac_stride, mac_off, sh, relu);
     a.list = list; a.list_count = count_dev;
     hipStream_t s = (hipStream_t)stream;
-    return halo_pick([&](auto pool, auto gm, auto strip) { return launch_halo2<ElemBF16, decltype(pool)::value, decltype(gm)::value, true, decltype(strip)::value>(a, s); },
-                     fuse_pool2 != 0, mac != nullptr, strips);
+    return halo_pick([&](auto pool, auto gm, auto strip, auto thin) {
+        return launch_halo2<ElemBF16, decltype(pool)::value, decltype(gm)::value, true, decltype(strip)::value ? (decltype(thin)::value ? 2 : 4) : 0>(a, s);
+    }, fuse_pool2 != 0, mac != nullptr, strip_h != 0, strip_h == 2);
 }
 
 extern "C" int cvpce_conv3x3_halo_list(const void* in, const void* wgt, const float* bias, void* out, float* mac, int mac_stride,
                                        int mac_off, int N, int H, int W, int Cin, int Cout, int K_pad, int Cout_pad, int relu,
                                        int fuse_pool2, const unsigned long long* list, const int* count_dev, void* stream) {
-    return halo_list_launch(in, wgt, bias, out, mac, mac_stride, mac_off, N, H, W, Cin, Cout, K_pad, Cout_pad, relu, fuse_pool2, list, count_dev, false, stream);
+    return halo_list_launch(in, wgt, bias, out, mac, mac_stride, mac_off, N, H, W, Cin, Cout, K_pad, Cout_pad, relu, fuse_pool2, list, count_dev, 0, stream);
 }
 
 extern "C" int cvpce_conv3x3_halo_strips(const void* in, const void* wgt, const float* bias, void* out, float* mac, int mac_stride,
                                          int mac_off, int N, int H, int W, int Cin, int Cout, int K_pad, int Cout_pad, int relu,
                                          int fuse_pool2, const unsigned long long* strip_list, const int* count_dev, void* stream) {
-    return halo_list_launch(in, wgt, bias, out, mac, mac_stride, mac_off, N, H, W, Cin, Cout, K_pad, Cout_pad, relu, fuse_pool2, strip_list, count_dev, true, stream);
+    return halo_list_launch(in, wgt, bias, out, mac, mac_stride, mac_off, N, H, W, Cin, Cout, K_pad, Cout_pad, relu, fuse_pool2, strip_list, count_dev, 4, stream);
+}
+
+extern "C" int cvpce_conv3x3_halo_strips2(const void* in, const void* wgt, const float* bias, void* out, float* mac, int mac_stride,
+                                          int mac_off, int N, int H, int W, int Cin, int Cout, int K_pad, int Cout_pad, int relu,
+                                          int fuse_pool2, const unsigned long long* thin_list, const int* count_dev, void* stream) {
+    return halo_list_launch(in, wgt, bias, out, mac, mac_stride, mac_off, N, H, W, Cin, Cout, K_pad, Cout_pad, relu, fuse_pool2, thin_list, count_dev, 2, stream);
 }
 
 extern "C" int cvpce_pack_halo_weights(const void* src_rowmajor, void* dst_halo, int Cout_pad, int Cin) {
diff --git a/cvpce_amd/csrc/conv3x3_halo3.hip b/cvpce_amd/csrc/conv3x3_halo3.hip
--- a/cvpce_amd/csrc/conv3x3_halo3.hip
+++ b/cvpce_amd/csrc/conv3x3_halo3.hip
@@ -207,17 +207,24 @@
         { G3_TIC() if (!(CVPCE_DBG & 64)) __builtin_amdgcn_s_barrier(); G3_TOC(2) }      \
         issue_next_patch();                                                                                    \
     }
+#define G3_MORE(R) (!LIST || rows_ > (R))
 #define G3_ROWS_AND_TAIL(T, TN, BUFB_NEXT, BEFORE)                                                             \
-    G3_RP(T, 0) G3_RP(T, 1) G3_RP(T, 2) G3_RP(T, 3) G3_RP(T, 4) G3_RP(T, 5)                                    \
-    if (!LIST || rows_ > 4) { G3_RP(T, 6) G3_RP(T, 7) G3_RP(T, 8) G3_RP(T, 9) }                                \
-    if (!LIST || rows_ > 8) { G3_RP(T, 10) G3_RP(T, 11) G3_RP(T, 12) G3_RP(T, 13) }                            \
-    if (!LIST || rows_ > 12) {                                                                                 \
-        G3_RP(T, 14) G3_RP(T, 15)                                                                              \
+    G3_RP(T, 0) G3_RP(T, 1) G3_RP(T, 2) G3_RP(T, 3)                                                            \
+    if (G3_MORE(2)) { G3_RP(T, 4) G3_RP(T, 5) }                                                                \
+    if (G3_MORE(4)) { G3_RP(T, 6) G3_RP(T, 7) }                                                                \
+    if (G3_MORE(6)) { G3_RP(T, 8) G3_RP(T, 9) }                                                                \
+    if (G3_MORE(8)) { G3_RP(T, 10) G3_RP(T, 11) }                                                              \
+    if (G3_MORE(10)) { G3_RP(T, 12) G3_RP(T, 13) }                                                             \
+    if (G3_MORE(12)) { G3_RP(T, 14) G3_RP(T, 15) }                                                             \
+    if (G3_MORE(14)) {                                                                                         \
         BEFORE                                                                                                 \
         G3_SET_E(TN, BUFB_NEXT)                                                                                \
         G3_READ(TN, 0) G3_ROW(T, 16)                                                                           \
         G3_READ(TN, 1) G3_ROW(T, 17)                                                                           \
     } else {                                                                                                   \
+                        \
+        asm volatile("s_waitcnt lgkmcnt(0)" ::: "memory");                                                     \
+        __builtin_amdgcn_sched_barrier(0);                                                                     \
         BEFORE                                                                                                 \
         G3_SET_E(TN, BUFB_NEXT)                                                                                \
         G3_READ(TN, 0)                                                                                         \
@@ -376,6 +383,7 @@
 #undef G3_STEP
 #undef G3_HANDOFF
 #undef G3_ROWS_AND_TAIL
+#undef G3_MORE
 #undef G3_RP
 #undef G3_ROW
 #undef G3_READ
diff --git a/cvpce_amd/csrc/skiplist.hip b/cvpce_amd/csrc/skiplist.hip
--- a/cvpce_amd/csrc/skiplist.hip
+++ b/cvpce_amd/csrc/skiplist.hip
@@ -12,6 +12,7 @@
     unsigned long long* lists;
     long long stride;
     int* counts;
+    int thin;
     int* computed;
 };
 
@@ -24,15 +25,18 @@
 
 __global__ __launch_bounds__(1024) void embed_worklists_kernel(WorklistArgs a) {
     __shared__ int s_cnt[1024];
-    __shared__ int s_end[1024], s_send[1024];
+    __shared__ int s_end[1024], s_send[1024], s_tend[1024];
     __shared__ unsigned s_geo[1024], s_ext[1024];
-    __shared__ int s_base, s_sbase, s_units;
+    __shared__ int s_base, s_sbase, s_tbase, s_units;
     const cvpce_skip_layer L = a.L[blockIdx.x];
     const int tid = threadIdx.x;
     const int tiles_y = (L.H + L.tile_h - 1) / L.tile_h, tiles_x = (L.W + L.tile_w - 1) / L.tile_w;
     unsigned long long* list = a.lists + (long long)blockIdx.x * a.stride;
     unsigned long long* slist = a.lists + (long long)(a.nl + blockIdx.x) * a.stride;
-    if (tid == 0) s_base = s_sbase = s_units = 0;
+    unsigned long long* tlist = a.lists + (long long)(2 * a.nl + blockIdx.x) * a.stride;
+    const bool has_strips = L.skip == 3 || L.skip == 5, has_thin = L.skip == 5;
+    const int rnd = L.skip >= 4 ? 1 : 3;
+    if (tid == 0) s_base = s_sbase = s_tbase = s_units = 0;
     __syncthreads();
     auto scan = [&](int v) {
         s_cnt[tid] = v;
@@ -59,7 +63,7 @@
                 if (L.skip >= 2 && ny > 0) {
                     const int left = eoy - (ny - 1) * L.tile_h;
                     const int act = left < L.tile_h ? left : L.tile_h;
-                    last_rows = ((act * 16 + L.tile_h - 1) / L.tile_h + 3) & ~3;
+                    last_rows = ((act * 16 + L.tile_h - 1) / L.tile_h + rnd) & ~rnd;
                     if (last_rows > 16) last_rows = 16;
                 }
             }
@@ -67,16 +71,16 @@
             eix = skl_extent(ex0, a.S, a.pool_mask, L.in_ops, L.in_W);
         }
         if (nx == 0) ny = 0;
-        const bool strips = L.skip >= 3 && ny > 0 && last_rows == 4;
-        const int scnt = strips ? nx : 0, cnt = ny * nx - scnt;
+        const bool strips = has_strips && ny > 0 && last_rows == 4, thin = has_thin && ny > 0 && last_rows == 2;
+        const int scnt = strips ? nx : 0, tcnt = thin ? nx : 0, cnt = ny * nx - scnt - tcnt;
         if (a.computed && n < a.n && blockIdx.y == 0) {
             a.computed[((long long)blockIdx.x * a.n + n) * 2] = ny > 0 ? (ny - 1) * 16 + last_rows : 0;
             a.computed[((long long)blockIdx.x * a.n + n) * 2 + 1] = nx;
         }
-        if (ny > 0) atomicAdd(&s_units, nx * (16 * (ny - 1) + (strips ? 4 : (last_rows < 16 ? last_rows + 1 : 16))));
+        if (ny > 0) atomicAdd(&s_units, nx * (16 * (ny - 1) + (strips ? 4 : (thin ? 2 : (last_rows < 16 ? last_rows + 1 : 16)))));
         s_geo[tid] = ((unsigned)ny << 16) | ((unsigned)nx << 8) | (unsigned)last_rows;
         s_ext[tid] = wl_pack_ext((unsigned)eiy, (unsigned)eix);
-        const int base0 = s_base, sbase0 = s_sbase;
+        const int base0 = s_base, sbase0 = s_sbase, tbase0 = s_tbase;
         scan(cnt);
         s_end[tid] = s_cnt[tid];
         const int total = s_cnt[1023];
@@ -85,6 +89,13 @@
         s_send[tid] = s_cnt[tid];
         const int stotal = s_cnt[1023];
         __syncthreads();
+        int ttotal = 0;
+        if (has_thin) {
+            scan(tcnt);
+            s_tend[tid] = s_cnt[tid];
+            ttotal = s_cnt[1023];
+            __syncthreads();
+        }
         auto crop_of = [&](const int* ends, int e) {
             int lo = 0, hi = 1023;
             while (lo < hi) {
@@ -107,14 +118,21 @@
             const int cny = (int)(geo >> 16), tx = e - (c ? s_send[c - 1] : 0);
             slist[sbase0 + e] = wl_pack(4u, s_ext[c], (unsigned)(n0 + c), (unsigned)(cny - 1), (unsigned)tx);
         }
+        for (int e = (int)blockIdx.y * 1024 + tid; e < ttotal; e += (int)gridDim.y * 1024) {
+            const int c = crop_of(s_tend, e);
+            const unsigned geo = s_geo[c];
+            const int cny = (int)(geo >> 16), tx = e - (c ? s_tend[c - 1] : 0);
+            tlist[tbase0 + e] = wl_pack(2u, s_ext[c], (unsigned)(n0 + c), (unsigned)(cny - 1), (unsigned)tx);
+        }
         __syncthreads();
-        if (tid == 0) { s_base = base0 + total; s_sbase = sbase0 + stotal; }
+        if (tid == 0) { s_base = base0 + total; s_sbase = sbase0 + stotal; s_tbase = tbase0 + ttotal; }
         __syncthreads();
     }
     if (tid == 0 && blockIdx.y == 0) {
         a.counts[blockIdx.x] = s_base;
         a.counts[a.nl + blockIdx.x] = s_units;
         a.counts[2 * a.nl + blockIdx.x] = s_sbase;
+        if (a.thin) a.counts[3 * a.nl + blockIdx.x] = s_tbase;
     }
 }
 
@@ -124,11 +142,13 @@
     if (!ext0 && n_images > 1) return CVPCE_ERR_ARG;
     if (!layers || !lists || !counts || n_layers > SKL_MAX_LAYERS || n_images <= 0 || n_images > WL_MAX_IMAGES || S <= 0 || S > 32767) return CVPCE_ERR_ARG;
     WorklistArgs a;
+    a.thin = 0;
     a.ext0 = ext0; a.n = n_images; a.S = S; a.nl = n_layers; a.pool_mask = pool_mask; a.lists = lists; a.stride = list_stride; a.counts = counts; a.computed = computed;
     for (int i = 0; i < n_layers; ++i) {
         const cvpce_skip_layer& l = layers[i];
         if (l.H <= 0 || l.W <= 0 || l.tile_h <= 0 || l.tile_w <= 0 || l.in_H <= 0 || l.in_W <= 0 || l.in_H > WL_MAX_EXTENT || l.in_W > WL_MAX_EXTENT) return CVPCE_ERR_ARG;
         if (l.in_ops < 0 || l.out_ops < l.in_ops || l.out_ops > 32) return CVPCE_ERR_ARG;
+        if (l.skip == 5) a.thin = 1;
         const long long ty = (l.H + l.tile_h - 1) / l.tile_h, tx = (l.W + l.tile_w - 1) / l.tile_w;
         if (ty > WL_MAX_TILES || tx > WL_MAX_TILES || ty * tx * n_images > list_stride) return CVPCE_ERR_ARG;
         a.L[i] = l;
diff --git a/cvpce_amd/models/classification.py b/cvpce_amd/models/classification.py
--- a/cvpce_amd/models/classification.py
+++ b/cvpce_amd/models/classification.py
@@ -22,6 +22,18 @@
 SKIP_ROWS = _os.environ.get('CVPCE_SKIP_ROWS', '1') != '0'
 SKIP_MAC = _os.environ.get('CVPCE_SKIP_MAC', '1') != '0'
 SKIP_STRIPS = _os.environ.get('CVPCE_SKIP_STRIPS', '1') != '0'
+SKIP_FINE = _os.environ.get('CVPCE_SKIP_FINE', '1') != '0'
+SKIP_FINE_PARTS = tuple(p for p in _os.environ.get('CVPCE_SKIP_FINE_PARTS', 'halo2,thin').split(',') if p)
+
+
+def _fine_mode(mode, cout):
+    if not SKIP_FINE or mode not in (2, 3):
+        return mode
+    if cout <= 128:
+        return 4 if (mode == 2 and 'halo3' in SKIP_FINE_PARTS) else mode
+    if 'halo2' not in SKIP_FINE_PARTS:
+        return mode
+    return 4 if mode == 2 else (5 if 'thin' in SKIP_FINE_PARTS else mode)
 
 
 def _passes(n, step, longest):
@@ -172,6 +184,7 @@
     def _embed_skip(self, x, ext, const_in, sched):
         steps, layers, pool_mask = sched
         N, S, nl = x.shape[0], x.shape[1], len(steps)
+        layers = [l if i == 0 else l[:-1] + [_fine_mode(l[-1], steps[i][1].cout)] for i, l in enumerate(layers)]
         early = 1 + sum(1 for st in steps[1:] if st[1].cout <= 128 and not st[3])
         if any(st[1].cout <= 128 for st in steps[early:]):
             early = nl
@@ -185,6 +198,7 @@
             res = ops.embed_worklists(ext_, n_img, S, pool_mask, sub, (S // 16) ** 2 if first == 0 else max(1, (sub[0][5] // 16)) ** 2,
                                       want_computed=mac_skips)
             lists, counts = res[0], res[1]
+            has_thin = any(l[-1] == 5 for l in sub)
             if mac_skips:
                 o = sum(st[1].cout for st in steps[1:first] if st[3])
                 for j in range(k):
@@ -200,7 +214,8 @@
                 kind, pc, pool, mac, store = steps[li]
                 t = ops.conv2d_list(t, pc, lists[j], counts[j:j + 1], act=1, pool=pool, mac=desc if mac else None, mac_off=off, store=store,
                                     units=counts[k + j:k + j + 1], out=out_last if (j == k - 1 and store) else None,
-                                    strips=(lists[k + j], counts[2 * k + j:2 * k + j + 1]) if layers[li][-1] == 3 else None)
+                                    strips=(lists[k + j], counts[2 * k + j:2 * k + j + 1]) if layers[li][-1] in (3, 5) else None,
+                                    thin=(lists[2 * k + j], counts[3 * k + j:3 * k + j + 1]) if (has_thin and layers[li][-1] == 5) else None)
                 if mac:
                     off += pc.cout
             return t
diff --git a/cvpce_amd/ops.py b/cvpce_amd/ops.py
--- a/cvpce_amd/ops.py
+++ b/cvpce_amd/ops.py
@@ -5,6 +5,7 @@
 from ._lib import lib
 from .torch_ops import T
 from . import torch_ops_input
+from . import torch_ops_lists
 
 BF16 = torch.bfloat16
 F16 = torch.float16
@@ -504,8 +505,9 @@
 def embed_worklists(ext0, n_images, size, pool_mask, layers, max_tiles, want_computed=False):
     _need_cuda(ext0)
     dev = ext0.device if ext0 is not None else torch.device('cuda', torch.cuda.current_device())
-    lists = torch.empty((2 * len(layers), n_images * max_tiles), dtype=torch.int64, device=dev)
-    counts = torch.empty((3 * len(layers),), dtype=torch.int32, device=dev)
+    thin = any(l[-1] == 5 for l in layers)
+    lists = torch.empty(((3 if thin else 2) * len(layers), n_images * max_tiles), dtype=torch.int64, device=dev)
+    counts = torch.empty(((4 if thin else 3) * len(layers),), dtype=torch.int32, device=dev)
     computed = torch.empty((len(layers), n_images, 2), dtype=torch.int32, device=dev) if want_computed else None
     T.embed_worklists(ext0, int(n_images), int(size), int(pool_mask), [v for l in layers for v in l], lists, counts, computed)
     return (lists, counts, computed) if want_computed else (lists, counts)
@@ -529,7 +531,7 @@
     return out
 
 
-def conv2d_list(x, pc, work, count, act=1, pool=False, mac=None, mac_off=0, store=True, units=None, strips=None, out=None):
+def conv2d_list(x, pc, work, count, act=1, pool=False, mac=None, mac_off=0, store=True, units=None, strips=None, out=None, thin=None):
     _need_cuda(x, work, count, mac)
     assert x.dtype == BF16 and pc.dtype == BF16 and x.is_contiguous() and x.dim() == 4
     assert pc.cin_pad % 64 == 0 and (pc.kh, pc.kw, pc.stride, pc.pad) == (3, 3, 1, 1) and pc.cout % 8 == 0 and pc.cout > 64
@@ -548,7 +550,11 @@
         wide = pc.cout <= 128
         tile_flops = 2.0 * 16 * (32 if wide else 16) * pc.cout * 9 * pc.cin
         tag = f'{pc.cin}->{pc.cout}@{h}' + ('mac' if mac is not None else '')
-        lunits = (units - 4 * strips[1]) if (units is not None and strips is not None) else units
+        lunits = units
+        if units is not None and strips is not None:
+            lunits = lunits - 4 * strips[1]
+        if units is not None and thin is not None:
+            lunits = lunits - 2 * thin[1]
         t.file('conv3x3_halo3_kernel' if wide else 'conv3x3_halo2_kernel', 2.0 * (n - 1) * h * w * pc.cout * 9 * pc.cin,
                extras=((lunits, tile_flops / 16) if units is not None else (count, tile_flops)) + (tag,))
     if strips is not None:
@@ -557,6 +563,12 @@
         if t is not None:
             t.stop()
             t.file('conv3x3_halo2_kernel[strips]', 0.0, extras=(strips[1], tile_flops / 4, tag))
+    if thin is not None:
+        assert pc.cout > 128
+        T.conv3x3_halo_strips2(x, pc.weight_halo, pc.bias, out, mac, int(mac_off), pc.cout, pc.k_pad, pc.cout_pad, int(act), int(pool and store), thin[0], thin[1])
+        if t is not None:
+            t.stop()
+            t.file('conv3x3_halo2_kernel[strips]', 0.0, extras=(thin[1], tile_flops / 8, tag))
     return out
 
 
diff --git a/cvpce_amd/torch_ops.py b/cvpce_amd/torch_ops.py
--- a/cvpce_amd/torch_ops.py
+++ b/cvpce_amd/torch_ops.py
@@ -249,8 +249,9 @@
 def _embed_worklists(ext0, n_images, size, pool_mask, layers, lists, counts, computed):
     nf = len(_lib.SkipLayer._fields_)
     nl = len(layers) // nf
-    if len(layers) != nl * nf or lists.dtype != torch.int64 or not lists.is_contiguous() or lists.shape[0] != 2 * nl or counts.dtype != torch.int32 \
-            or counts.numel() != 3 * nl or (ext0 is not None and (ext0.dtype != torch.int32 or not ext0.is_contiguous() or ext0.numel() < 2 * (n_images - 1))):
+    thin = any(int(layers[i * nf + nf - 1]) == 5 for i in range(nl))
+    if len(layers) != nl * nf or lists.dtype != torch.int64 or not lists.is_contiguous() or lists.shape[0] != (3 if thin else 2) * nl or counts.dtype != torch.int32 \
+            or counts.numel() != (4 if thin else 3) * nl or (ext0 is not None and (ext0.dtype != torch.int32 or not ext0.is_contiguous() or ext0.numel() < 2 * (n_images - 1))):
         raise RuntimeError('embed_worklists: bad argument shapes / types')
     arr = (_lib.SkipLayer * nl)(*[_lib.SkipLayer(*[int(v) for v in layers[i * nf:(i + 1) * nf]]) for i in range(nl)])
     if computed is not None and (computed.dtype != torch.int32 or not computed.is_contiguous() or computed.numel() < 2 * nl * n_images):
diff --git a/cvpce_amd/torch_ops_lists.py b/cvpce_amd/torch_ops_lists.py
--- /dev/null
+++ b/cvpce_amd/torch_ops_lists.py
@@ -0,0 +1,20 @@
+from ._lib import lib
+from .torch_ops import _L, _halo_list
+
+NAMES = []
+
+
+def _op(schema):
+    def deco(fn):
+        name = schema.split('(')[0]
+        _L.define(schema)
+        _L.impl(name, fn, 'CUDA')
+        NAMES.append(name)
+        return fn
+    return deco
+
+
+@_op('conv3x3_halo_strips2(Tensor x, Tensor weight, Tensor? bias, Tensor(a!)? out, Tensor(b!)? mac, int mac_off, int cout, int k_pad, '
+     'int cout_pad, int relu, int pool, Tensor work, Tensor count) -> ()')
+def _conv3x3_halo_strips2(x, weight, bias, out, mac, mac_off, cout, k_pad, cout_pad, relu, pool, work, count):
+    _halo_list(lib.cvpce_conv3x3_halo_strips2, 'cvpce_conv3x3_halo_strips2', x, weight, bias, out, mac, mac_off, cout, k_pad, cout_pad, relu, pool, work, count)
diff --git a/include/cvpce_amd_lists.h b/include/cvpce_amd_lists.h
--- /dev/null
+++ b/include/cvpce_amd_lists.h
@@ -0,0 +1,12 @@
+#pragma once
+#ifdef __cplusplus
+extern "C" {
+#endif
+
+int cvpce_conv3x3_halo_strips2(const void* in, const void* wgt, const float* bias, void* out, float* mac, int mac_stride,
+                               int mac_off, int N, int H, int W, int Cin, int Cout, int K_pad, int Cout_pad, int relu,
+                               int fuse_pool2, const unsigned long long* thin_list, const int* count_dev, void* stream);
+
+#ifdef __cplusplus
+}
+#endif
```

Measured after the change: 283.0 images/s, median of 6. 1.7% higher.
